# comprna/radian

Measured on AMD Instinct MI355X. Metric: signal samples/s basecalled (chunk=1024, beam=10), higher is better.
Workload: dtype f32

## Files before the change

include/radian_hip.h:

```cpp
#ifndef RADIAN_HIP_H
#define RADIAN_HIP_H

#include <stddef.h>
#include <stdint.h>

#ifdef __cplusplus
extern "C" {
#endif

#define RD_OK 0
#define RD_ERR_ARG (-1)
#define RD_ERR_HIP (-2)
#define RD_ERR_STATE (-3)
#define RD_ERR_NOMEM (-4)
#define RD_ERR_RCCL (-5)
#define RD_ERR_FORMAT (-6)
#define RD_ERR_IO (-7)
#define RD_LEN_MISSING_CONTEXT (-1)

typedef struct rd_ctx rd_ctx;

const char* rd_last_error(void);
int rd_version(void);
int rd_device_count(int* n);
int rd_decode_max_width(void);
int rd_decode_lane_width(void);

int rd_create(int device_id, rd_ctx** out);
int rd_destroy(rd_ctx* ctx);
int rd_sync(rd_ctx* ctx);
int rd_set_precision(rd_ctx* ctx, int mode);

typedef struct rd_weights_header {
    uint32_t magic;
    uint32_t version;
    uint32_t nb_filters;
    uint32_t kernel_size;
    uint32_t relu_units;
    uint32_t n_classes;
    uint32_t n_blocks;
    uint32_t dilations[16];
    uint32_t n_floats;
} rd_weights_header;
int rd_load_weights(rd_ctx* ctx, const void* blob, size_t nbytes);

int rd_load_lm(rd_ctx* ctx, const double* table, int k);
int rd_load_lm_absent(rd_ctx* ctx, int k);
int rd_load_lm_hashed(rd_ctx* ctx, const double* table, int table_order, int context_len);
int rd_set_logits(rd_ctx* ctx, int mode);
int rd_set_decode_partition(rd_ctx* ctx, int cus_per_xcd);
int rd_set_decode_math(rd_ctx* ctx, int mode);

int rd_forward(rd_ctx* ctx, const float* windows, int n_windows, int chunk_len, float* probs);

int rd_assemble(rd_ctx* ctx, const float* probs, int n_windows, int chunk_len, int pad, int step, double* out,
                int64_t out_cap, int64_t* n_rows, int* is_f64);

int rd_decode_batch(rd_ctx* ctx, const void* probs, int prob_is_f64, const int64_t* seq_off, const int32_t* seq_len,
                    int n_seq, int beam_width, int use_lm, double s_thr, double r_thr, uint8_t* labels_out,
                    const int64_t* label_off, int32_t* label_len, double* best_score);

int rd_basecall_chunk(rd_ctx* ctx, const float* windows, int n_windows, int chunk_len, const int32_t* valid_len,
                      int beam_width, uint8_t* labels_out, int32_t* label_len);

int rd_basecall_global(rd_ctx* ctx, const float* windows, int chunk_len, int step, const int32_t* read_win_off,
                       const int32_t* pad, int n_reads, int beam_width, int use_lm, double s_thr, double r_thr,
                       uint8_t* labels_out, const int64_t* label_off, int32_t* label_len);

int rd_count_windows(int64_t n_samples, int chunk_len, int step);
int rd_basecall_reads_chunk(rd_ctx* ctx, const float* signal, const int64_t* read_off, int n_reads, int chunk_len,
                            int step, int beam_width, uint8_t* labels_out, int32_t* label_len);
int rd_basecall_reads_global(rd_ctx* ctx, const float* signal, const int64_t* read_off, int n_reads, int chunk_len,
                             int step, int beam_width, int use_lm, double s_thr, double r_thr, uint8_t* labels_out,
                             const int64_t* label_off, int32_t* label_len);

int rd_normalise_reads(rd_ctx* ctx, const int16_t* raw, const int64_t* read_off, int n_reads, int outlier_clip,
                       float* norm_out , int32_t* status);
int rd_basecall_raw_chunk(rd_ctx* ctx, const int16_t* raw, const int64_t* read_off, int n_reads, int outlier_clip,
                          int chunk_len, int step, int beam_width, uint8_t* labels_out, int32_t* label_len, int32_t* status);
int rd_basecall_raw_global(rd_ctx* ctx, const int16_t* raw, const int64_t* read_off, int n_reads, int outlier_clip,
                           int chunk_len, int step, int beam_width, int use_lm, double s_thr, double r_thr,
                           uint8_t* labels_out, const int64_t* label_off, int32_t* label_len, int32_t* status);

int rd_dev_alloc(rd_ctx* ctx, size_t bytes, void** d_ptr);
int rd_dev_free(rd_ctx* ctx, void* d_ptr);
int rd_mem_info(rd_ctx* ctx, size_t* free_bytes, size_t* total_bytes);
int rd_memcpy_h2d(rd_ctx* ctx, void* d_dst, const void* src, size_t bytes);
int rd_memcpy_d2h(rd_ctx* ctx, void* dst, const void* d_src, size_t bytes);
int rd_forward_resident(rd_ctx* ctx, const float* d_windows, int n_windows, int chunk_len, float* d_probs);
int rd_forward_reads_resident(rd_ctx* ctx, const float* d_signal, const int64_t* read_off, int n_reads, int chunk_len,
                              int step, int decode_type, int lane, int64_t* total_rows);
int rd_forward_reads(rd_ctx* ctx, const float* signal, const int64_t* read_off, int n_reads, int chunk_len, int step,
                     float* probs_out, int64_t windows_cap, int64_t* n_windows);
int rd_basecall_chunk_resident(rd_ctx* ctx, const float* d_windows, int n_windows, int chunk_len,
                               const int32_t* valid_len, int beam_width, uint8_t* labels_out, int32_t* label_len);
int rd_decode_resident(rd_ctx* ctx, const float* d_probs, int n_windows, int chunk_len, const int32_t* valid_len,
                       int beam_width, uint8_t* labels_out, int32_t* label_len);

int rd_basecall_reads_chunk_resident(rd_ctx* ctx, const float* d_signal, const int64_t* read_off, int n_reads,
                                     int chunk_len, int step, int beam_width, uint8_t* labels_out, int32_t* label_len);
int rd_basecall_reads_global_resident(rd_ctx* ctx, const float* d_signal, const int64_t* read_off, int n_reads,
                                      int chunk_len, int step, int beam_width, int use_lm, double s_thr, double r_thr,
                                      uint8_t* labels_out, const int64_t* label_off, int32_t* label_len);

int rd_pipe_config(rd_ctx* ctx, int group_batches);
int rd_pipe_set_lanes(rd_ctx* ctx, int lanes);
int rd_pipe_submit(rd_ctx* ctx, const float* d_windows, int n_windows, int chunk_len, const int32_t* valid_len,
                   int beam_width, uint8_t* labels_out, int32_t* label_len);
int rd_pipe_submit_reads(rd_ctx* ctx, const float* d_signal, const int64_t* read_off, int n_reads, int chunk_len,
                         int step, int beam_width, uint8_t* labels_out, int32_t* label_len);
int rd_pipe_submit_reads_global(rd_ctx* ctx, const float* d_signal, const int64_t* read_off, int n_reads, int chunk_len,
                                int step, int beam_width, int use_lm, double s_thr, double r_thr, uint8_t* labels_out,
                                const int64_t* label_off, int32_t* label_len);
int rd_pipe_submit_raw_global(rd_ctx* ctx, const int16_t* raw, const int64_t* read_off, int n_reads, int outlier_clip,
                              int chunk_len, int step, int beam_width, int use_lm, double s_thr, double r_thr,
                              uint8_t* labels_out, const int64_t* label_off, int32_t* label_len, int32_t* status);
int rd_pipe_submit_raw_chunk(rd_ctx* ctx, const int16_t* raw, const int64_t* read_off, int n_reads, int outlier_clip,
                             int chunk_len, int step, int beam_width, uint8_t* labels_out, int32_t* label_len, int32_t* status);
int rd_pipe_progress(rd_ctx* ctx, int64_t wait_for, int64_t* delivered);
int rd_pipe_flush(rd_ctx* ctx);
int rd_pipe_submitted(rd_ctx* ctx, int64_t* submitted);

int rd_lm_json_probe(const char* buf, size_t n, int* k_out);
int rd_lm_json_fill(const char* buf, size_t n, int k, double* table, int64_t* n_entries, int64_t* n_contexts);
int rd_lm_json_write(const char* path, const double* table, int k, int64_t* n_rows, int64_t* n_bytes);

int rd_fasta_scan(const char* buf, size_t n, int field, const char* value, uint8_t* codes, int64_t* offsets, int64_t* counts);
int rd_lm_build(rd_ctx* ctx, const uint8_t* codes, const int64_t* offsets, int64_t n_records, int k, int as_written, int unseen, double alpha,
                double r_thr, int64_t cut, double* table_out, uint32_t* counts_out, int64_t* stats);
int rd_lm_score(rd_ctx* ctx, const uint8_t* codes, const int64_t* offsets, int64_t n_records, int as_written, double r_thr, int64_t cut,
                int64_t* stats, double* nll_sum);

typedef struct rd_fast5 rd_fast5;
int rd_fast5_open(const char* path, rd_fast5** out);
int rd_fast5_open_mem(const void* buf, size_t n, rd_fast5** out);
void rd_fast5_close(rd_fast5* f);
int rd_fast5_count(const rd_fast5* f, int64_t* n_reads);
int rd_fast5_lengths(rd_fast5* f, int64_t lo, int64_t hi, int64_t* n_samples);
int rd_fast5_read_batch(rd_fast5* f, int64_t lo, int64_t hi, int16_t* samples, int64_t cap, int64_t* offsets, char* ids, int id_stride);

int rd_stitch_chunk(const uint8_t* labels, const int32_t* label_len, int chunk_len, const int32_t* read_win_off, int n_reads,
                    uint8_t* seq_out, const int64_t* seq_off, int32_t* seq_len, int n_threads);

#define RD_ALIGN_OK 0
#define RD_ALIGN_CLIP_INDEX_ERROR 1
#define RD_ALIGN_EMPTY_AFTER_CLIP 2
#define RD_ALIGN_TOO_LARGE 3
int rd_align_batch(rd_ctx* ctx, const uint8_t* refs, const int64_t* ref_off, const uint8_t* reads, const int64_t* read_off, int n_pairs,
                   int match, int mismatch, int gap_open, int gap_extend, int64_t budget_bytes, int32_t* score, int32_t* counts,
                   int32_t* status, uint8_t* ops_out, const int64_t* ops_off, int32_t* ops_len);
int64_t rd_align_workspace_bytes(int64_t n, int64_t m);
int rd_align_clip_count(const uint8_t* ops, int64_t n_ops, const uint8_t* ref, const uint8_t* read, int32_t* counts, int32_t* status);

#define RD_CTCALIGN_OK 0
#define RD_CTCALIGN_NO_PATH 1
#define RD_CTCALIGN_TOO_LARGE 2
int rd_ctc_align_batch(rd_ctx* ctx, const void* probs, int prob_is_f64, const int64_t* seq_off, const int32_t* seq_len, int n_seq,
                       const uint8_t* labels, const int64_t* label_off, const int32_t* label_len, int64_t budget_bytes,
                       int32_t* first_step, int32_t* last_step, uint8_t* qual, double* score, int32_t* status);
int64_t rd_ctc_align_workspace_bytes(int64_t n_rows, int64_t n_labels);
int rd_basecall_raw_global_q(rd_ctx* ctx, const int16_t* raw, const int64_t* read_off, int n_reads, int outlier_clip, int chunk_len,
                             int step, int beam_width, int use_lm, double s_thr, double r_thr, uint8_t* labels_out,
                             const int64_t* label_off, int32_t* label_len, int32_t* status, int64_t budget_bytes, uint8_t* qual_out,
                             int32_t* first_step_out, int32_t* last_step_out, double* score_out, int32_t* align_status);

typedef struct rd_tfrecord rd_tfrecord;
int rd_tfrecord_open(const char* path, rd_tfrecord** out);
int rd_tfrecord_open_mem(const void* buf, size_t n, rd_tfrecord** out);
void rd_tfrecord_close(rd_tfrecord* f);
int rd_tfrecord_count(const rd_tfrecord* f, int64_t* n_records, int64_t* n_labels);
int rd_tfrecord_read(const rd_tfrecord* f, int64_t lo, int64_t hi, float* signals, int32_t* input_len, int64_t* label_off,
                     int32_t* label_len, uint8_t* labels, int64_t labels_cap);
uint32_t rd_crc32c(const void* buf, size_t n);
int rd_tfrecord_write(const char* path, const float* signals, const int32_t* input_len, const uint8_t* labels, const int64_t* label_off,
                      const int32_t* label_len, int64_t n, int append);

#define RD_FIT_OK 0
#define RD_FIT_EMPTY 1
#define RD_FIT_TOO_LARGE 2
int rd_fit_batch(rd_ctx* ctx, const uint8_t* refs, const int64_t* ref_off, int64_t n_refs, const uint8_t* queries, const int64_t* query_off,
                 const int32_t* query_ref, int64_t n_queries, int match, int mismatch, int gap_open, int gap_extend, int64_t budget_bytes,
                 int32_t* score, int32_t* ref_start, int32_t* ref_end, int32_t* counts, int32_t* status);

#define RD_MAP_HASH_C1 0x9E3779B1u
// ... 59 lines not shown
```

radian_amd/_lib.py:

```python
import ctypes
import os

HERE = os.path.dirname(os.path.abspath(__file__))
LIB_PATH = os.environ.get("RADIAN_HIP_LIB") or os.path.join(HERE, "libradian_hip.so")

c_i = ctypes.c_int
c_i32p = ctypes.POINTER(ctypes.c_int32)
c_i64 = ctypes.c_int64
c_i64p = ctypes.POINTER(ctypes.c_int64)
c_d = ctypes.c_double
c_dp = ctypes.POINTER(ctypes.c_double)
c_fp = ctypes.POINTER(ctypes.c_float)
c_u8p = ctypes.POINTER(ctypes.c_uint8)
c_vp = ctypes.c_void_p
c_sz = ctypes.c_size_t

SIGNATURES = {
    "rd_last_error": (ctypes.c_char_p, []),
    "rd_version": (c_i, []),
    "rd_device_count": (c_i, [ctypes.POINTER(c_i)]),
    "rd_decode_max_width": (c_i, []),
    "rd_decode_lane_width": (c_i, []),
    "rd_create": (c_i, [c_i, ctypes.POINTER(c_vp)]),
    "rd_destroy": (c_i, [c_vp]),
    "rd_sync": (c_i, [c_vp]),
    "rd_set_precision": (c_i, [c_vp, c_i]),
    "rd_load_weights": (c_i, [c_vp, c_vp, c_sz]),
    "rd_load_lm": (c_i, [c_vp, c_vp, c_i]),
    "rd_load_lm_absent": (c_i, [c_vp, c_i]),
    "rd_load_lm_hashed": (c_i, [c_vp, c_vp, c_i, c_i]),
    "rd_set_logits": (c_i, [c_vp, c_i]),
    "rd_set_decode_math": (c_i, [c_vp, c_i]),
    "rd_set_decode_partition": (c_i, [c_vp, c_i]),
    "rd_forward": (c_i, [c_vp, c_vp, c_i, c_i, c_vp]),
    "rd_assemble": (c_i, [c_vp, c_vp, c_i, c_i, c_i, c_i, c_vp, c_i64, c_i64p, ctypes.POINTER(c_i)]),
    "rd_decode_batch": (c_i, [c_vp, c_vp, c_i, c_vp, c_vp, c_i, c_i, c_i, c_d, c_d, c_vp, c_vp, c_vp, c_vp]),
    "rd_basecall_chunk": (c_i, [c_vp, c_vp, c_i, c_i, c_vp, c_i, c_vp, c_vp]),
    "rd_basecall_global": (c_i, [c_vp, c_vp, c_i, c_i, c_vp, c_vp, c_i, c_i, c_i, c_d, c_d, c_vp, c_vp, c_vp]),
    "rd_count_windows": (c_i, [c_i64, c_i, c_i]),
    "rd_basecall_reads_chunk": (c_i, [c_vp, c_vp, c_vp, c_i, c_i, c_i, c_i, c_vp, c_vp]),
    "rd_basecall_reads_global": (c_i, [c_vp, c_vp, c_vp, c_i, c_i, c_i, c_i, c_i, c_d, c_d, c_vp, c_vp, c_vp]),
    "rd_basecall_reads_chunk_resident": (c_i, [c_vp, c_vp, c_vp, c_i, c_i, c_i, c_i, c_vp, c_vp]),
    "rd_basecall_reads_global_resident": (c_i, [c_vp, c_vp, c_vp, c_i, c_i, c_i, c_i, c_i, c_d, c_d, c_vp, c_vp, c_vp]),
    "rd_pipe_submit_reads": (c_i, [c_vp, c_vp, c_vp, c_i, c_i, c_i, c_i, c_vp, c_vp]),
    "rd_pipe_submit_reads_global": (c_i, [c_vp, c_vp, c_vp, c_i, c_i, c_i, c_i, c_i, c_d, c_d, c_vp, c_vp, c_vp]),
    "rd_pipe_submit_raw_global": (c_i, [c_vp, c_vp, c_vp, c_i, c_i, c_i, c_i, c_i, c_i, c_d, c_d, c_vp, c_vp, c_vp, c_vp]),
    "rd_pipe_submit_raw_chunk": (c_i, [c_vp, c_vp, c_vp, c_i, c_i, c_i, c_i, c_i, c_vp, c_vp, c_vp]),
    "rd_pipe_progress": (c_i, [c_vp, c_i64, c_i64p]),
    "rd_pipe_submitted": (c_i, [c_vp, c_i64p]),
    "rd_normalise_reads": (c_i, [c_vp, c_vp, c_vp, c_i, c_i, c_vp, c_vp]),
    "rd_basecall_raw_chunk": (c_i, [c_vp, c_vp, c_vp, c_i, c_i, c_i, c_i, c_i, c_vp, c_vp, c_vp]),
    "rd_basecall_raw_global": (c_i, [c_vp, c_vp, c_vp, c_i, c_i, c_i, c_i, c_i, c_i, c_d, c_d, c_vp, c_vp, c_vp, c_vp]),
    "rd_stitch_chunk": (c_i, [c_vp, c_vp, c_i, c_vp, c_i, c_vp, c_vp, c_vp, c_i]),
    "rd_fast5_open": (c_i, [ctypes.c_char_p, ctypes.POINTER(c_vp)]),
    "rd_fast5_open_mem": (c_i, [c_vp, c_sz, ctypes.POINTER(c_vp)]),
    "rd_fast5_close": (None, [c_vp]),
    "rd_fast5_count": (c_i, [c_vp, c_i64p]),
    "rd_fast5_lengths": (c_i, [c_vp, c_i64, c_i64, c_vp]),
    "rd_fast5_read_batch": (c_i, [c_vp, c_i64, c_i64, c_vp, c_i64, c_vp, c_vp, c_i]),
    "rd_lm_json_probe": (c_i, [c_vp, ctypes.c_size_t, ctypes.POINTER(c_i)]),
    "rd_lm_json_fill": (c_i, [c_vp, ctypes.c_size_t, c_i, c_vp, ctypes.POINTER(ctypes.c_int64), ctypes.POINTER(ctypes.c_int64)]),
    "rd_lm_json_write": (c_i, [ctypes.c_char_p, c_vp, c_i, c_i64p, c_i64p]),
    "rd_fasta_scan": (c_i, [c_vp, c_sz, c_i, ctypes.c_char_p, c_vp, c_vp, c_vp]),
    "rd_lm_build": (c_i, [c_vp, c_vp, c_vp, c_i64, c_i, c_i, c_i, c_d, c_d, c_i64, c_vp, c_vp, c_vp]),
    "rd_lm_score": (c_i, [c_vp, c_vp, c_vp, c_i64, c_i, c_d, c_i64, c_vp, c_dp]),
    "rd_dev_alloc": (c_i, [c_vp, c_sz, ctypes.POINTER(c_vp)]),
    "rd_mem_info": (c_i, [c_vp, ctypes.POINTER(c_sz), ctypes.POINTER(c_sz)]),
    "rd_dev_free": (c_i, [c_vp, c_vp]),
    "rd_memcpy_h2d": (c_i, [c_vp, c_vp, c_vp, c_sz]),
    "rd_memcpy_d2h": (c_i, [c_vp, c_vp, c_vp, c_sz]),
    "rd_forward_resident": (c_i, [c_vp, c_vp, c_i, c_i, c_vp]),
    "rd_forward_reads_resident": (c_i, [c_vp, c_vp, c_vp, c_i, c_i, c_i, c_i, c_i, c_vp]),
    "rd_forward_reads": (c_i, [c_vp, c_vp, c_vp, c_i, c_i, c_i, c_vp, c_i64, c_vp]),
    "rd_basecall_chunk_resident": (c_i, [c_vp, c_vp, c_i, c_i, c_vp, c_i, c_vp, c_vp]),
    "rd_decode_resident": (c_i, [c_vp, c_vp, c_i, c_i, c_vp, c_i, c_vp, c_vp]),
    "rd_pipe_config": (c_i, [c_vp, c_i]),
    "rd_pipe_set_lanes": (c_i, [c_vp, c_i]),
    "rd_pipe_submit": (c_i, [c_vp, c_vp, c_i, c_i, c_vp, c_i, c_vp, c_vp]),
    "rd_pipe_flush": (c_i, [c_vp]),
    "rd_align_batch": (c_i, [c_vp, c_vp, c_vp, c_vp, c_vp, c_i, c_i, c_i, c_i, c_i, c_i64, c_vp, c_vp, c_vp, c_vp, c_vp, c_vp]),
    "rd_align_workspace_bytes": (c_i64, [c_i64, c_i64]),
    "rd_align_clip_count": (c_i, [c_vp, c_i64, c_vp, c_vp, c_vp, c_vp]),
    "rd_ctc_align_batch": (c_i, [c_vp, c_vp, c_i, c_vp, c_vp, c_i, c_vp, c_vp, c_vp, c_i64, c_vp, c_vp, c_vp, c_vp, c_vp]),
    "rd_ctc_align_workspace_bytes": (c_i64, [c_i64, c_i64]),
    "rd_basecall_raw_global_q": (c_i, [c_vp, c_vp, c_vp, c_i, c_i, c_i, c_i, c_i, c_i, c_d, c_d, c_vp, c_vp, c_vp, c_vp, c_i64, c_vp, c_vp, c_vp, c_vp, c_vp]),
    "rd_tfrecord_open": (c_i, [ctypes.c_char_p, ctypes.POINTER(c_vp)]),
    "rd_tfrecord_open_mem": (c_i, [c_vp, c_sz, ctypes.POINTER(c_vp)]),
    "rd_tfrecord_close": (None, [c_vp]),
    "rd_tfrecord_count": (c_i, [c_vp, c_i64p, c_i64p]),
    "rd_tfrecord_read": (c_i, [c_vp, c_i64, c_i64, c_vp, c_vp, c_vp, c_vp, c_vp, c_i64]),
    "rd_crc32c": (ctypes.c_uint32, [c_vp, c_sz]),
    "rd_tfrecord_write": (c_i, [ctypes.c_char_p, c_vp, c_vp, c_vp, c_vp, c_vp, c_i64, c_i]),
    "rd_fit_batch": (c_i, [c_vp, c_vp, c_vp, c_i64, c_vp, c_vp, c_vp, c_i64, c_i, c_i, c_i, c_i, c_i64, c_vp, c_vp, c_vp, c_vp, c_vp]),
    "rd_map_minimizers": (c_i, [c_vp, c_i64, c_i, c_i, c_vp, c_vp, c_i64, c_i64p]),
    "rd_map_index": (c_i, [c_vp, c_vp, c_vp, c_i64, c_i, c_i, c_i, c_vp]),
    "rd_map_batch": (c_i, [c_vp, c_vp, c_vp, c_i64, c_i, c_i, c_i, c_i, c_i64, c_vp, c_vp, c_vp]),
    "rd_ctc_eval": (c_i, [c_vp, c_vp, c_i, c_vp, c_vp, c_vp, c_vp, c_vp, c_vp, c_vp, c_vp, c_vp]),
    "rd_ctc_probs": (c_i, [c_vp, c_vp, c_i, c_vp, c_vp, c_vp, c_vp, c_vp, c_vp, c_vp, c_vp, c_vp]),
    "rd_ctc_probs_resident": (c_i, [c_vp, c_vp, c_i, c_vp, c_vp, c_vp, c_vp, c_vp, c_vp, c_vp, c_vp, c_vp]),
    "rd_train_grad": (c_i, [c_vp, c_vp, c_i, c_vp, c_vp, c_vp, c_vp, c_vp, c_vp, c_vp]),
    "rd_train_step": (c_i, [c_vp, c_vp, c_i, c_vp, c_vp, c_vp, c_vp, c_vp, c_vp, c_vp]),
    "rd_train_step_resident": (c_i, [c_vp, c_vp, c_i, c_vp, c_vp, c_vp, c_vp, c_vp, c_vp, c_vp]),
    "rd_train_reset": (c_i, [c_vp]),
    "rd_get_weights": (c_i, [c_vp, c_vp, c_sz]),
    "rd_model_params": (c_i, [c_vp, c_i64p]),
    "rd_train_ctc_grad": (c_i, [c_vp, c_vp, c_i, c_vp, c_vp, c_vp, c_vp, c_vp, c_vp, c_vp]),
    "rd_rccl_probe": (c_i, []),
    "rd_rccl_unique_id": (c_i, [c_vp]),
    "rd_rccl_init": (c_i, [c_vp, c_i, c_i, c_vp]),
    "rd_rccl_bcast_model": (c_i, [c_vp, c_i]),
    "rd_clone_artifacts": (c_i, [c_vp, c_vp]),
    "rd_rccl_allreduce_max": (c_i, [c_vp, c_vp, c_i]),
    "rd_rccl_barrier": (c_i, [c_vp]),
    "rd_rccl_comm_count": (c_i, [c_vp, ctypes.POINTER(c_i)]),
    "rd_rccl_finalize": (c_i, [c_vp]),
}

DIAG_SIGNATURES = {
    "rd_set_conv_fuse": (c_i, [c_vp, c_i]),
    "rd_set_conv_shape": (c_i, [c_vp, c_i]),
    "rd_split3": (c_i, [c_vp, c_vp, c_sz, c_vp]),
    "rd_set_decode_form": (c_i, [c_vp, c_i]),
    "rd_pipe_policy_read": (c_i, [c_vp, c_i, c_i, c_i, c_vp, c_vp, c_vp]),
    "rd_pipe_stats": (c_i, [c_vp, c_i64p, c_i]),
    "rd_set_trie_budget": (c_i, [c_vp, c_i64]),
    "rd_timer_enable": (c_i, [c_vp, c_i, c_i]),
    "rd_timer_read": (c_i, [c_vp, c_i, c_dp, ctypes.POINTER(c_i), c_dp, c_dp]),
    "rd_timer_read_launches": (c_i, [c_vp, c_i, c_i, c_vp, c_vp, c_vp, ctypes.POINTER(c_i)]),
}

_lib = None


def load():
    global _lib
    if _lib is not None:
        return _lib
    if not os.path.exists(LIB_PATH):
        raise RuntimeError(
            f"{LIB_PATH} is missing: build it with `python -m radian_amd.build` (hipcc --offload-arch=gfx950). "
            "radian_amd has no CPU fallback.")
    lib = ctypes.CDLL(LIB_PATH)
    for name, (res, args) in {**SIGNATURES, **DIAG_SIGNATURES}.items():
        fn = getattr(lib, name)
        fn.restype = res
        fn.argtypes = args
    _lib = lib
    return lib
```

radian_amd/backend.py:

```python
import ctypes

import numpy as np

from . import _lib
from .weights import pack_blob, DEFAULT_DILATIONS

RD_TIMER_CONV, RD_TIMER_DECODE, RD_TIMER_HEAD, RD_TIMER_IN = 0, 1, 2, 3


class RadianHipError(RuntimeError):
    pass


def lib_path():
    return _lib.LIB_PATH


def _p(a):
    return None if a is None else a.ctypes.data_as(ctypes.c_void_p)


MISSING_CONTEXT = -1


def _labels_of(labels, off, n):
    if n == MISSING_CONTEXT:
        return None
    return labels[off: off + n].copy()


def device_count():
    n = ctypes.c_int(0)
    L = _lib.load()
    if L.rd_device_count(ctypes.byref(n)) != 0:
        raise RadianHipError(L.rd_last_error().decode())
    return n.value


def device_for_rank(local_rank):
    n = device_count()
    if n < 1:
        raise RadianHipError("no HIP device is visible to this process")
    return local_rank if local_rank < n else local_rank % n


ALIGN_OK, ALIGN_CLIP_INDEX_ERROR, ALIGN_EMPTY_AFTER_CLIP, ALIGN_TOO_LARGE = 0, 1, 2, 3
ALIGN_SCORES = (2, -4, -4, -2)


CTCALIGN_OK, CTCALIGN_NO_PATH, CTCALIGN_TOO_LARGE = 0, 1, 2
CTCALIGN_STATUS_NAMES = ("ok", "no-path", "too-large")


def ctc_align_workspace_bytes(n_rows, n_labels):
    return int(_lib.load().rd_ctc_align_workspace_bytes(int(n_rows), int(n_labels)))


class CtcAlignResult:
    __slots__ = ("first_step", "last_step", "qual", "score", "status")

    def __init__(self, first_step, last_step, qual, score, status):
        self.first_step, self.last_step, self.qual, self.score, self.status = first_step, last_step, qual, score, status


FIT_OK, FIT_EMPTY, FIT_TOO_LARGE = 0, 1, 2


class FitResult:

    def __init__(self, score, ref_start, ref_end, counts, status):
        self.score, self.ref_start, self.ref_end, self.counts, self.status = score, ref_start, ref_end, counts, status


def _concat_codes(seqs):
    arrs = [np.ascontiguousarray(np.frombuffer(s, dtype=np.uint8) if isinstance(s, (bytes, bytearray)) else s, dtype=np.uint8).reshape(-1) for s in seqs]
    off = np.zeros(len(arrs) + 1, dtype=np.int64)
    np.cumsum([a.size for a in arrs], out=off[1:])
    buf = np.concatenate(arrs) if off[-1] else np.zeros(1, dtype=np.uint8)
    return np.ascontiguousarray(buf), off


MAP_OK, MAP_NO_SEED, MAP_NO_CHAIN, MAP_TOO_LARGE, MAP_EMPTY_SPAN = 0, 1, 2, 3, 4


class MapResult:

    FIELDS = ("t", "score", "score2", "n_anchors", "q0", "r0", "q1", "r1")

    def __init__(self, status, hits, stats=None):
        self.status, self.hits, self.stats = status, hits, stats
        for c, name in enumerate(self.FIELDS):
            setattr(self, name, hits[:, c])


def map_minimizers(codes, k, w):
    L = _lib.load()
    c = np.ascontiguousarray(codes, dtype=np.uint8).reshape(-1)
    n = c.size
    buf = c if n else np.zeros(1, dtype=np.uint8)
    pos = np.zeros(max(n, 1), dtype=np.int32)
    hs = np.zeros(max(n, 1), dtype=np.uint32)
    got = ctypes.c_int64(0)
    rc = L.rd_map_minimizers(_p(buf), n, int(k), int(w), _p(pos), _p(hs), pos.size, ctypes.byref(got))
    if rc != 0:
        raise RadianHipError(f"[rd error {rc}] " + L.rd_last_error().decode("utf-8", "replace"))
    return pos[: got.value].copy(), hs[: got.value].copy()


def tfrecord_write(path, signals, input_len, labels, label_len=None, append=False):
    L = _lib.load()
    sig = np.ascontiguousarray(signals, dtype=np.float32)
    n = len(input_len)
    if sig.size != n * CTC_T:
        raise ValueError(f"signals must be [{n}, {CTC_T}] float32")
    il = np.ascontiguousarray(input_len, dtype=np.int32).reshape(-1)
    buf, off, ll = _pack_labels(labels, label_len, n)
    rc = L.rd_tfrecord_write(str(path).encode(), _p(sig), _p(il), _p(buf), _p(off), _p(ll), n, 1 if append else 0)
    if rc == -7:
        raise OSError(L.rd_last_error().decode("utf-8", "replace"))
    if rc != 0:
        raise RadianHipError(f"[rd error {rc}] " + L.rd_last_error().decode("utf-8", "replace"))


def _as_bytes(s):
    return s.encode("latin-1") if isinstance(s, str) else bytes(s)


def _concat(seqs):
    bs = [_as_bytes(s) for s in seqs]
    off = np.zeros(len(bs) + 1, dtype=np.int64)
    np.cumsum([len(b) for b in bs], out=off[1:])
    buf = np.frombuffer(b"".join(bs), dtype=np.uint8) if off[-1] else np.zeros(1, dtype=np.uint8)
    return np.ascontiguousarray(buf), off


def align_workspace_bytes(n, m):
    return int(_lib.load().rd_align_workspace_bytes(int(n), int(m)))


def align_clip_count(ops, ref, read):
    L = _lib.load()
    o, r, q = (np.frombuffer(_as_bytes(x), dtype=np.uint8) if len(x) else np.zeros(1, dtype=np.uint8) for x in (ops, ref, read))
    cnt = np.zeros(4, dtype=np.int32)
    st = np.zeros(1, dtype=np.int32)
    rc = L.rd_align_clip_count(_p(o), len(ops), _p(r), _p(q), _p(cnt), _p(st))
    if rc != 0:
        raise RadianHipError(f"[rd error {rc}] " + L.rd_last_error().decode("utf-8", "replace"))
    return tuple(int(c) for c in cnt), int(st[0])


class AlignResult:

    def __init__(self, score, counts, status, ops):
        self.score, self.counts, self.status, self.ops = score, counts, status, ops


CTC_OK, CTC_INFEASIBLE = 0, 1
CTC_T, CTC_MAX_LABEL = 1024, 255


def _pack_labels(labels, label_len, n):
    if label_len is None:
        label_len = [len(l) for l in labels]
    ll = np.ascontiguousarray(label_len, dtype=np.int32).reshape(-1)
    if len(labels) != n or ll.size != n:
        raise ValueError(f"{len(labels)} label rows and {ll.size} lengths for {n} windows")
    rows = []
    for i in range(n):
        row = np.asarray(labels[i]).reshape(-1)
        if ll[i] < 0 or ll[i] > row.size:
            raise ValueError(f"window {i}: label_length {int(ll[i])} outside 0..{row.size}")
        r = row[: ll[i]]
        if r.size and (np.any(r != np.round(r)) or r.min() < 0 or r.max() > 3):
            raise ValueError(f"window {i}: labels must be 0..3")
        rows.append(r.astype(np.uint8))
    off = np.zeros(n + 1, dtype=np.int64)
    np.cumsum(ll, out=off[1:])
    buf = np.concatenate(rows) if off[-1] else np.zeros(1, dtype=np.uint8)
    return np.ascontiguousarray(buf), np.ascontiguousarray(off[:-1]), ll


class CtcResult:

    def __init__(self, loss, status, greedy_len, edit_distance, greedy):
        self.loss, self.status, self.greedy_len, self.edit_distance, self.greedy = loss, status, greedy_len, edit_distance, greedy


class PipeTicket:

    def __init__(self, be, decode_type, off, n):
        self.be, self.decode_type, self.off, self.n = be, decode_type, off, n
        self.status = np.zeros(n, dtype=np.int32)
        self.labels = self.lens = self.label_off = self.nw = None
        self.seq = 0

    def done(self):
        return self.be.pipe_progress(0) >= self.seq

    def wait(self):
        if self.be.pipe_progress(self.seq) < self.seq:
            raise RadianHipError("pipeline did not deliver the awaited batch")

    def result_raw(self):
        self.wait()
        return self.labels, self.lens, self.nw, self.status

    def result(self):
        self.wait()
        if self.decode_type == "global":
            return [_labels_of(self.labels, self.off[r], self.lens[r]) for r in range(self.n)], self.status
        out, w = [], 0
        for n in self.nw:
            out.append([self.labels[w + i, : self.lens[w + i]].copy() for i in range(n)])
            w += n
        return out, self.status


class Backend:

    def __init__(self, device_id=0):
        self._L = _lib.load()
        h = ctypes.c_void_p()
        self._h = None
        self._check(self._L.rd_create(int(device_id), ctypes.byref(h)))
        self._h = h
        self.device_id = device_id
        self.lm_k = None
        self._tickets = {}

    def _check(self, rc):
        if rc != 0:
            raise RadianHipError(f"[rd error {rc}] " + self._L.rd_last_error().decode("utf-8", "replace"))

    def close(self):
        if self._h is not None:
            self._L.rd_destroy(self._h)
            self._h = None
        self._tickets.clear()

    def __del__(self):
        try:
            self.close()
        except Exception:
            pass

    def __enter__(self):
        return self

    def __exit__(self, *exc):
        self.close()

    def sync(self):
        self._check(self._L.rd_sync(self._h))

    def set_precision(self, mode):
        code = {"fp32": 0, "f16x3": 1, "bf16x3": 2}[mode] if isinstance(mode, str) else int(mode)
        self._check(self._L.rd_set_precision(self._h, code))

    def set_conv_shape(self, shape):
        self._check(self._L.rd_set_conv_shape(self._h, int(shape)))

    def split3(self, values):
        v = np.ascontiguousarray(values, dtype=np.float32).ravel()
        out = np.zeros((3, v.size), dtype=np.uint16)
        self._check(self._L.rd_split3(self._h, _p(v), v.size, _p(out)))
        return out

    @property
    def max_beam_width(self):
        return self._L.rd_decode_max_width()

    def load_weights(self, flat, dilations=DEFAULT_DILATIONS):
        blob = pack_blob(flat, dilations)
        self.load_weights_blob(blob)

    def load_weights_blob(self, blob):
        buf = ctypes.create_string_buffer(blob, len(blob))
        self._check(self._L.rd_load_weights(self._h, ctypes.cast(buf, ctypes.c_void_p), len(blob)))

    def load_lm(self, table, k):
        if table is None:
            self._check(self._L.rd_load_lm(self._h, None, 0))
            self.lm_k = None
            return
        table = np.ascontiguousarray(table, dtype=np.float64)
        if table.shape != (4 ** k, 4):
            raise ValueError(f"LM table must be [4^{k},4], got {table.shape}")
        self._check(self._L.rd_load_lm(self._h, _p(table), int(k)))
        self.lm_k = k

    UNSEEN = {"backoff": 0, "uniform": 1, "absent": 2}

    @staticmethod
    def _records(codes, offsets):
        codes = np.ascontiguousarray(codes, dtype=np.uint8)
        offsets = np.ascontiguousarray(offsets, dtype=np.int64)
        if offsets.ndim != 1 or len(offsets) < 1 or codes.ndim != 1 or int(offsets[-1]) != len(codes):
            raise ValueError("offsets must be [records + 1] and end at len(codes)")
        return (codes if len(codes) else np.zeros(1, dtype=np.uint8)), offsets

    def build_lm(self, codes, offsets, k, as_written=False, unseen="backoff", pseudocount=0.0, r_threshold=0.5, cut=0,
                 want_table=True, want_counts=False):
        codes, offsets = self._records(codes, offsets)
        if unseen not in self.UNSEEN:
            raise ValueError(f"unseen must be one of {sorted(self.UNSEEN)}")
        big = 1 <= k <= 13
        table = np.empty((4 ** k, 4), dtype=np.float64) if want_table and big else None
        counts = np.empty((4 ** k, 4), dtype=np.uint32) if want_counts and big else None
        st = np.zeros(32, dtype=np.int64)
        self._check(self._L.rd_lm_build(self._h, _p(codes), _p(offsets), len(offsets) - 1, int(k), 1 if as_written else 0, self.UNSEEN[unseen],
                                        float(pseudocount), float(r_threshold), int(cut), _p(table), _p(counts), _p(st)))
        self.lm_k = k
        stats = {"windows": int(st[0]), "contexts": 4 ** k, "contexts_seen": int(st[1]), "gate_contexts": int(st[2]), "gate_windows": int(st[3]),
                 "absent_rows": int(st[4]), "uniform_rows": int(st[5]), "launches": int(st[6]),
                 "stage_us": {name: int(st[24 + i]) for i, name in enumerate(("staging", "upload", "count", "table", "download"))},
                 "rows_per_order": {j: int(st[8 + j]) for j in range(k, -1, -1) if st[8 + j]}}
        if counts is not None:
            stats["counts"] = counts
        return table, stats

    def score_lm(self, codes, offsets, as_written=False, r_threshold=0.5, cut=0):
        codes, offsets = self._records(codes, offsets)
        st = np.zeros(8, dtype=np.int64)
        total = ctypes.c_double(0.0)
        self._check(self._L.rd_lm_score(self._h, _p(codes), _p(offsets), len(offsets) - 1, 1 if as_written else 0, float(r_threshold), int(cut),
                                        _p(st), ctypes.byref(total)))
        n = int(st[1])
        return {"windows": int(st[0]), "scored": n, "zero": int(st[2]), "absent": int(st[3]), "gate_windows": int(st[4]),
                "nll_sum": total.value, "mean_nll": total.value / n if n else float("nan")}

    def load_lm_absent(self, k):
        self._check(self._L.rd_load_lm_absent(self._h, int(k)))
        self.lm_k = k

    def load_lm_hashed(self, table, table_order, context_len):
        table = np.ascontiguousarray(table, dtype=np.float64)
        if table.shape != (4 ** table_order, 4):
            raise ValueError(f"LM table must be [4^{table_order},4], got {table.shape}")
        self._check(self._L.rd_load_lm_hashed(self._h, _p(table), int(table_order), int(context_len)))
        self.lm_k = context_len

    def set_logits(self, mode):
        self._check(self._L.rd_set_logits(self._h, {"f32": 0, "f16": 1}[mode] if isinstance(mode, str) else int(mode)))

    def set_trie_budget(self, nbytes):
        self._check(self._L.rd_set_trie_budget(self._h, int(nbytes)))

    def set_conv_fuse(self, on):
        self._check(self._L.rd_set_conv_fuse(self._h, 1 if on else 0))

    def set_decode_form(self, form):
        self._check(self._L.rd_set_decode_form(self._h, {"auto": 0, "waves": 1, "lanes": 2, "two": 3, "one": 4, "queue": 5}[form] if isinstance(form, str) else int(form)))

    def set_decode_partition(self, cus_per_xcd):
        self._check(self._L.rd_set_decode_partition(self._h, int(cus_per_xcd)))

    def set_decode_math(self, mode):
        self._check(self._L.rd_set_decode_math(self._h, {"fast": 0, "glibc": 1}[mode] if isinstance(mode, str) else int(mode)))

    def forward(self, windows):
        windows = np.ascontiguousarray(windows, dtype=np.float32)
        if windows.ndim != 2:
            raise ValueError("windows must be [n_windows, chunk_len]")
        n, T = windows.shape
        probs = np.empty((n, T, 5), dtype=np.float32)
        self._check(self._L.rd_forward(self._h, _p(windows), n, T, _p(probs)))
        return probs

    def assemble(self, probs, pad, step):
        probs = np.ascontiguousarray(probs, dtype=np.float32)
        nW, T, _ = probs.shape
        cap = (nW - 1) * step + T
        out = np.empty((max(cap, 1), 5), dtype=np.float64)
        n_rows = ctypes.c_int64(0)
        is64 = ctypes.c_int(0)
        self._check(self._L.rd_assemble(self._h, _p(probs), nW, T, int(pad), int(step), _p(out), out.shape[0],
                                        ctypes.byref(n_rows), ctypes.byref(is64)))
        out = out[: n_rows.value]
        return out if is64.value else out.astype(np.float32)

    def forward_reads(self, signals, chunk_len, step):
        sigs = [np.ascontiguousarray(s_, dtype=np.float32) for s_ in signals]
        off = np.zeros(len(sigs) + 1, dtype=np.int64)
        off[1:] = np.cumsum([s_.shape[0] for s_ in sigs])
        nws = [self.count_windows(int(s_.shape[0]), chunk_len, step) for s_ in sigs]
        tot = int(sum(nws))
        flat = np.concatenate(sigs) if sigs else np.zeros(0, dtype=np.float32)
        out = np.zeros((tot, chunk_len, 5), dtype=np.float32)
        n = ctypes.c_int64(0)
        self._check(self._L.rd_forward_reads(self._h, _p(flat), _p(off), len(sigs), int(chunk_len), int(step), _p(out), tot, ctypes.byref(n)))
        assert n.value == tot
        res, w = [], 0
        for k in nws:
            res.append(out[w:w + k])
            w += k
        return res

    def decode_batch(self, mats, seq_off, seq_len, beam_width, use_lm=False, s_threshold=0.0, r_threshold=0.0,
                     with_scores=False):
        mats = np.ascontiguousarray(mats)
        if mats.dtype not in (np.float32, np.float64):
            raise TypeError("probabilities must be float32 or float64")
        seq_off = np.ascontiguousarray(seq_off, dtype=np.int64)
        seq_len = np.ascontiguousarray(seq_len, dtype=np.int32)
        n = int(seq_len.shape[0])
        label_off = np.zeros(n, dtype=np.int64)
        if n:
            label_off[1:] = np.cumsum(seq_len[:-1].astype(np.int64))
        labels = np.zeros(int(seq_len.astype(np.int64).sum()) + 1, dtype=np.uint8)
        lens = np.zeros(n, dtype=np.int32)
# ... 528 lines not shown
```

radian_amd/csrc/api.hip:

```cpp
#include "common.h"
#include "plan.h"
#include "../../include/radian_hip.h"

#include <math.h>
#include <string.h>

using namespace rdi;

namespace {

struct SeqMeta {
    int64_t *d_seq_off, *d_seq_off2, *d_node_off, *d_label_off;
    int32_t *d_seq_len, *d_split, *d_label_len;
    double* d_score;
    int64_t total_labels;
    std::vector<TrieRun> runs;
};

int prepare_seq_meta(rd_ctx* ctx, const int64_t* seq_off, const int64_t* seq_off2, const int32_t* split, const int32_t* seq_len,
                     int n_seq, int W, SeqMeta& sm, std::vector<int64_t>& label_off_used)
{
    std::vector<int64_t> node_off(n_seq), lab_off(n_seq);
    int64_t labs = 0;
    for (int i = 0; i < n_seq; i++) {
// ... 194 lines not shown
    }
    return decode_and_fetch(ctx, d_probs, 0, seq_off.data(), valid_len, n_windows, beam_width, 0, 0.0, 0.0, labels_out, lab_off.data(),
                            label_len, nullptr);
}

extern "C" int rd_basecall_chunk_resident(rd_ctx* ctx, const float* d_windows, int n_windows, int chunk_len,
                                          const int32_t* valid_len, int beam_width, uint8_t* labels_out, int32_t* label_len)
{
    RD_REQUIRE(ctx && d_windows && valid_len && labels_out && label_len, "rd_basecall_chunk_resident: null argument");
    RD_REQUIRE(n_windows >= 1 && chunk_len >= 1, "rd_basecall_chunk_resident: bad shape");
    RD_REQUIRE(beam_width >= 1 && beam_width <= rd_decode_max_width(), "beam_width %d out of range", beam_width);
    RD_HIP(hipSetDevice(ctx->device));
    const size_t n = (size_t)n_windows * chunk_len;
    if (ctx->ws_probs.reserve(n * 20)) return RD_ERR_NOMEM;
    int rc = rd_forward_dev(ctx, d_windows, n_windows, chunk_len, ctx->ws_probs.as<float>());
    if (rc) return rc;
    return chunk_decode_from_probs(ctx, ctx->ws_probs.as<float>(), n_windows, chunk_len, valid_len, beam_width, labels_out, label_len);
}

extern "C" int rd_basecall_chunk(rd_ctx* ctx, const float* windows, int n_windows, int chunk_len, const int32_t* valid_len,
                                 int beam_width, uint8_t* labels_out, int32_t* label_len)
{
    RD_REQUIRE(ctx && windows, "rd_basecall_chunk: null argument");
    RD_REQUIRE(n_windows >= 1 && chunk_len >= 1, "rd_basecall_chunk: bad shape");
    RD_HIP(hipSetDevice(ctx->device));
    const size_t n = (size_t)n_windows * chunk_len;
    if (ctx->ws_in.reserve(n * 4)) return RD_ERR_NOMEM;
    RD_HIP(hipMemcpyAsync(ctx->ws_in.p, windows, n * 4, hipMemcpyHostToDevice, ctx->stream));
    return rd_basecall_chunk_resident(ctx, ctx->ws_in.as<float>(), n_windows, chunk_len, valid_len, beam_width, labels_out, label_len);
}

extern "C" int rd_decode_resident(rd_ctx* ctx, const float* d_probs, int n_windows, int chunk_len, const int32_t* valid_len,
                                  int beam_width, uint8_t* labels_out, int32_t* label_len)
{
    RD_REQUIRE(ctx && d_probs && valid_len && labels_out && label_len, "rd_decode_resident: null argument");
    RD_REQUIRE(beam_width >= 1 && beam_width <= rd_decode_max_width(), "beam_width %d out of range", beam_width);
    RD_HIP(hipSetDevice(ctx->device));
    return chunk_decode_from_probs(ctx, d_probs, n_windows, chunk_len, valid_len, beam_width, labels_out, label_len);
}

extern "C" int rd_forward_resident(rd_ctx* ctx, const float* d_windows, int n_windows, int chunk_len, float* d_probs)
{
    RD_REQUIRE(ctx && d_windows, "rd_forward_resident: null argument");
    RD_HIP(hipSetDevice(ctx->device));
    if (!d_probs) {
        if (ctx->ws_probs.reserve((size_t)n_windows * chunk_len * 20)) return RD_ERR_NOMEM;
        d_probs = ctx->ws_probs.as<float>();
    }
    return rd_forward_dev(ctx, d_windows, n_windows, chunk_len, d_probs);
}

static int global_finish(rd_ctx* ctx, const void* d_probs, int f16, bool streamed, const int32_t* win_off, const int32_t* pad, const int64_t* src_row,
                         const int64_t* read_off, int n_reads, int chunk_len, int step, int beam_width, int use_lm, double s_thr, double r_thr,
                         uint8_t* labels_out, const int64_t* label_off, int32_t* label_len, AlignOut* ao = nullptr )
{
    std::vector<ReadRows> rr;
    const int64_t rows64 = classify_reads(win_off, pad, n_reads, chunk_len, step, 0, rr);
    for (int r = 0; read_off && r < n_reads; r++)
        RD_REQUIRE(rr[r].N == read_off[r + 1] - read_off[r], "internal: assembled length mismatch for read %d", r);
    if (ctx->ws_mat.reserve((size_t)(rows64 + 1) * 40)) return RD_ERR_NOMEM;
    int rc;
    for (int r = 0; r < n_reads; r++) {
        if (!rr[r].is64) continue;
        rc = rd_assemble_dev(ctx, (const char*)d_probs + (size_t)src_row[r] * 5 * (f16 ? 2 : 4), win_off[r + 1] - win_off[r], chunk_len, pad[r], step,
                             ctx->ws_mat.as<double>() + rr[r].row64 * 5, rr[r].N, streamed ? 1 : 0, f16);
        if (rc) return rc;
    }
    for (int pass = 0; pass < 2; pass++) {
        std::vector<int64_t> so, lo;
        std::vector<int32_t> sl;
        std::vector<int> idx;
        for (int r = 0; r < n_reads; r++)
            if (rr[r].is64 == (pass == 0)) {
                so.push_back(pass == 0 ? rr[r].row64 : src_row[r]);
                sl.push_back((int32_t)rr[r].N);
                lo.push_back(label_off[r]);
                idx.push_back(r);
            }
        if (idx.empty()) continue;
        std::vector<int32_t> ll(idx.size()), ast(idx.size());
        std::vector<double> asc(idx.size());
        AlignOut pa;
        if (ao) {
            pa = *ao;
            pa.score = asc.data();
            pa.status = ast.data();
        }
        rc = decode_and_fetch(ctx, pass == 0 ? (const void*)ctx->ws_mat.p : d_probs, pass == 0 ? 1 : (f16 ? 2 : 0), so.data(), sl.data(),
                              (int)idx.size(), beam_width, use_lm, s_thr, r_thr, labels_out, lo.data(), ll.data(), nullptr, nullptr, nullptr,
                              ao ? &pa : nullptr);
        if (rc) return rc;
        for (size_t i = 0; i < idx.size(); i++) {
            label_len[idx[i]] = ll[i];
            if (ao) {
                ao->score[idx[i]] = asc[i];
                ao->status[idx[i]] = ast[i];
                ao->too_large |= pa.too_large;
            }
        }
    }
    return RD_OK;
}

extern "C" int rd_basecall_global(rd_ctx* ctx, const float* windows, int chunk_len, int step, const int32_t* read_win_off,
                                  const int32_t* pad, int n_reads, int beam_width, int use_lm, double s_thr, double r_thr,
                                  uint8_t* labels_out, const int64_t* label_off, int32_t* label_len)
{
    RD_REQUIRE(ctx && windows && read_win_off && pad && labels_out && label_off && label_len, "rd_basecall_global: null argument");
    RD_REQUIRE(n_reads >= 1 && chunk_len >= 1, "rd_basecall_global: bad shape");
    RD_REQUIRE(step >= 1 && step <= chunk_len, "rd_basecall_global: step %d must be in [1, chunk_len]", step);
    RD_REQUIRE(beam_width >= 1 && beam_width <= rd_decode_max_width(), "beam_width %d out of range", beam_width);
    RD_REQUIRE_WIDTH_LM(ctx, beam_width, use_lm);
    RD_HIP(hipSetDevice(ctx->device));
    const int nW = read_win_off[n_reads];
    RD_REQUIRE(nW >= n_reads, "rd_basecall_global: every read needs at least one window");
    const size_t n = (size_t)nW * chunk_len;
    if (ctx->ws_in.reserve(n * 4) || ctx->ws_probs.reserve(n * 20)) return RD_ERR_NOMEM;
    RD_HIP(hipMemcpyAsync(ctx->ws_in.p, windows, n * 4, hipMemcpyHostToDevice, ctx->stream));
    int rc = rd_forward_dev(ctx, ctx->ws_in.as<float>(), nW, chunk_len, ctx->ws_probs.as<float>());
    if (rc) return rc;
    std::vector<int64_t> src_row(n_reads);
    for (int r = 0; r < n_reads; r++) {
        RD_REQUIRE(read_win_off[r + 1] > read_win_off[r], "rd_basecall_global: read %d has no windows", r);
        RD_REQUIRE(pad[r] >= 0 && pad[r] <= chunk_len, "rd_basecall_global: pad[%d] out of range", r);
        src_row[r] = (int64_t)read_win_off[r] * chunk_len;
    }
    return global_finish(ctx, ctx->ws_probs.p, 0, false, read_win_off, pad, src_row.data(), nullptr, n_reads, chunk_len, step, beam_width, use_lm,
                         s_thr, r_thr, labels_out, label_off, label_len);
}

extern "C" int rd_count_windows(int64_t n_samples, int chunk_len, int step)
{
    if (n_samples < 0 || chunk_len < 1 || step < 1 || step > chunk_len) return -1;
    return count_windows(n_samples, chunk_len, step);
}

namespace {
struct PlanCache {
    PlanKey key;
    ReadsPlan plan;
    bool streamed = false;
    DevBuf d_tiles;
    TileLists lists;
};

int get_plan(rd_ctx* ctx, const int64_t* read_off, int n_reads, int chunk, int step, int mode, const ReadsPlan** out,
             const TileLists** lists, bool* streamed)
{
    PlanCache* pc = (PlanCache*)ctx->plan_cache[mode];
    if (!pc) {
        pc = new PlanCache();
        ctx->plan_cache[mode] = pc;
    }
    const int halo = rd_model_halo(ctx);
    if (!(pc->d_tiles.p && pc->key.matches(ctx->model, read_off, n_reads, chunk, step, mode, halo))) {
        RD_REQUIRE(read_off[0] == 0, "read_off[0] must be 0");
        size_t total = 0;
        int rc = pc->key.rebuild(ctx->model, read_off, n_reads, chunk, step, mode, halo, pc->plan, &pc->streamed, &total);
        if (rc) return rc;
        if (pc->d_tiles.reserve(total * sizeof(TileDesc) + 16)) return RD_ERR_NOMEM;
        if ((rc = rd_sync_lanes(ctx))) return rc;
        std::vector<TileDesc> host(total);
        plan_fill_lists(pc->plan, pc->d_tiles.as<TileDesc>(), host.data(), pc->lists);
        if (total) RD_HIP(hipMemcpy(pc->d_tiles.p, host.data(), total * sizeof(TileDesc), hipMemcpyHostToDevice));
        pc->key.valid = true;
    }
    *out = &pc->plan;
    *lists = &pc->lists;
    if (streamed) *streamed = pc->streamed;
    return RD_OK;
}

}

int rdi::rd_check_reads_args(rd_ctx* ctx, const void* signal, const int64_t* read_off, int n_reads, int chunk_len, int step, int W)
{
    RD_REQUIRE(ctx && signal && read_off, "null argument");
    RD_REQUIRE(n_reads >= 1 && chunk_len >= 1, "bad shape");
    RD_REQUIRE(step >= 1 && step <= chunk_len, "step %d must be in [1, chunk_len]", step);
    RD_REQUIRE(W >= 1 && W <= rd_decode_max_width(), "beam_width %d out of range", W);
    if (!ctx->model.loaded) {
        rd_set_error("no weights loaded (rd_load_weights)");
        return RD_ERR_STATE;
    }
    return RD_OK;
}

void rd_plan_cache_destroy_internal(rd_ctx* ctx)
{
    for (int m = 0; m < 2; m++) {
        PlanCache* pc = (PlanCache*)ctx->plan_cache[m];
        if (pc) {
            pc->d_tiles.release();
            delete pc;
        }
        ctx->plan_cache[m] = nullptr;
    }
}

extern "C" int rd_basecall_reads_chunk_resident(rd_ctx* ctx, const float* d_signal, const int64_t* read_off, int n_reads,
                                                int chunk_len, int step, int beam_width, uint8_t* labels_out,
                                                int32_t* label_len)
{
    int rc = rd_check_reads_args(ctx, d_signal, read_off, n_reads, chunk_len, step, beam_width);
    if (rc) return rc;
    RD_REQUIRE(labels_out && label_len, "rd_basecall_reads_chunk: null output");
    RD_HIP(hipSetDevice(ctx->device));
    const ReadsPlan* P = nullptr;
    const TileLists* tl = nullptr;
    if ((rc = get_plan(ctx, read_off, n_reads, chunk_len, step, 0, &P, &tl, nullptr))) return rc;
    if (ctx->ws_probs.reserve((size_t)P->total_rows * 20)) return RD_ERR_NOMEM;
    const int f16 = ctx->logits_f16;
    rc = rd_forward_tiles_dev(ctx, d_signal, *tl, P->total_rows, ctx->ws_probs.p, 0, f16);
    if (rc) return rc;
    std::vector<int64_t> lab_off(P->n_windows);
    for (int w = 0; w < P->n_windows; w++) lab_off[w] = (int64_t)w * chunk_len;
    return decode_and_fetch(ctx, ctx->ws_probs.p, f16 ? 2 : 0, P->off1.data(), P->valid.data(), P->n_windows, beam_width, 0, 0.0, 0.0,
                            labels_out, lab_off.data(), label_len, nullptr, P->off2.data(), P->split.data());
}

extern "C" int rd_forward_reads_resident(rd_ctx* ctx, const float* d_signal, const int64_t* read_off, int n_reads, int chunk_len,
                                         int step, int decode_type, int lane, int64_t* total_rows)
{
    int rc = rd_check_reads_args(ctx, d_signal, read_off, n_reads, chunk_len, step, 1);
    if (rc) return rc;
    RD_REQUIRE(decode_type == 0 || decode_type == 1, "rd_forward_reads_resident: decode_type %d (0 = chunk plan, 1 = global plan)", decode_type);
    RD_REQUIRE(lane >= 0 && lane < RD_MAX_LANES, "rd_forward_reads_resident: lane %d out of range [0,%d)", lane, RD_MAX_LANES);
    RD_HIP(hipSetDevice(ctx->device));
    const ReadsPlan* P = nullptr;
    const TileLists* tl = nullptr;
    if ((rc = get_plan(ctx, read_off, n_reads, chunk_len, step, decode_type, &P, &tl, nullptr))) return rc;
    if (ctx->ws_probs.reserve((size_t)P->total_rows * 20)) return RD_ERR_NOMEM;
    if (total_rows) *total_rows = P->total_rows;
    return rd_forward_tiles_dev(ctx, d_signal, *tl, P->total_rows, ctx->ws_probs.p, lane, ctx->logits_f16);
}

extern "C" int rd_forward_reads(rd_ctx* ctx, const float* signal, const int64_t* read_off, int n_reads, int chunk_len, int step,
                                float* probs_out, int64_t windows_cap, int64_t* n_windows)
{
    int rc = rd_check_reads_args(ctx, signal, read_off, n_reads, chunk_len, step, 1);
    if (rc) return rc;
    RD_REQUIRE(probs_out && n_windows, "rd_forward_reads: null output");
    RD_REQUIRE(!ctx->logits_f16, "rd_forward_reads: float32 rows only (rd_set_logits 0)");
    RD_HIP(hipSetDevice(ctx->device));
    const size_t n = (size_t)read_off[n_reads];
    if (ctx->ws_in.reserve(n * 4 + 16)) return RD_ERR_NOMEM;
    RD_HIP(hipMemcpyAsync(ctx->ws_in.p, signal, n * 4, hipMemcpyHostToDevice, ctx->stream));
    const ReadsPlan* P = nullptr;
    const TileLists* tl = nullptr;
    if ((rc = get_plan(ctx, read_off, n_reads, chunk_len, step, 0, &P, &tl, nullptr))) return rc;
    *n_windows = P->n_windows;
    RD_REQUIRE(P->n_windows <= windows_cap, "rd_forward_reads: %d windows, room for %lld", P->n_windows, (long long)windows_cap);
    if (ctx->ws_probs.reserve((size_t)P->total_rows * 20)) return RD_ERR_NOMEM;
    if ((rc = rd_forward_tiles_dev(ctx, ctx->ws_in.as<float>(), *tl, P->total_rows, ctx->ws_probs.p, 0, 0))) return rc;
    const size_t nw = (size_t)P->n_windows, a8 = align_up(nw * 8, 256), a4 = align_up(nw * 4, 256);
    const size_t out_bytes = nw * chunk_len * 20;
    if (ctx->ws_misc.reserve(2 * a8 + 2 * a4) || ctx->ws_mat.reserve(out_bytes + 16)) return RD_ERR_NOMEM;
    char* dm = (char*)ctx->ws_misc.p;
    RD_HIP(hipMemcpyAsync(dm, P->off1.data(), nw * 8, hipMemcpyHostToDevice, ctx->stream));
    RD_HIP(hipMemcpyAsync(dm + a8, P->off2.data(), nw * 8, hipMemcpyHostToDevice, ctx->stream));
    RD_HIP(hipMemcpyAsync(dm + 2 * a8, P->split.data(), nw * 4, hipMemcpyHostToDevice, ctx->stream));
    RD_HIP(hipMemcpyAsync(dm + 2 * a8 + a4, P->valid.data(), nw * 4, hipMemcpyHostToDevice, ctx->stream));
    if ((rc = rd_gather_windows_dev(ctx->stream, ctx->ws_probs.as<float>(), (const int64_t*)dm, (const int64_t*)(dm + a8), (const int32_t*)(dm + 2 * a8),
                                    (const int32_t*)(dm + 2 * a8 + a4), P->n_windows, chunk_len, (float*)ctx->ws_mat.p)))
        return rc;
    RD_HIP(hipMemcpyAsync(probs_out, ctx->ws_mat.p, out_bytes, hipMemcpyDeviceToHost, ctx->stream));
    RD_HIP(hipStreamSynchronize(ctx->stream));
    return RD_OK;
}

extern "C" int rd_basecall_reads_chunk(rd_ctx* ctx, const float* signal, const int64_t* read_off, int n_reads, int chunk_len,
                                       int step, int beam_width, uint8_t* labels_out, int32_t* label_len)
{
    int rc = rd_check_reads_args(ctx, signal, read_off, n_reads, chunk_len, step, beam_width);
    if (rc) return rc;
    RD_HIP(hipSetDevice(ctx->device));
    const size_t n = (size_t)read_off[n_reads];
    if (ctx->ws_in.reserve(n * 4 + 16)) return RD_ERR_NOMEM;
    RD_HIP(hipMemcpyAsync(ctx->ws_in.p, signal, n * 4, hipMemcpyHostToDevice, ctx->stream));
    return rd_basecall_reads_chunk_resident(ctx, ctx->ws_in.as<float>(), read_off, n_reads, chunk_len, step, beam_width, labels_out,
                                            label_len);
}

static int reads_global_resident(rd_ctx* ctx, const float* d_signal, const int64_t* read_off, int n_reads, int chunk_len, int step, int beam_width,
                                 int use_lm, double s_thr, double r_thr, uint8_t* labels_out, const int64_t* label_off, int32_t* label_len,
                                 AlignOut* ao)
{
    int rc = rd_check_reads_args(ctx, d_signal, read_off, n_reads, chunk_len, step, beam_width);
    if (rc) return rc;
    RD_REQUIRE(labels_out && label_off && label_len, "rd_basecall_reads_global: null output");
    RD_REQUIRE_WIDTH_LM(ctx, beam_width, use_lm);
    RD_HIP(hipSetDevice(ctx->device));
    const ReadsPlan* P = nullptr;
    const TileLists* tl = nullptr;
    bool streamed = false;
    if ((rc = get_plan(ctx, read_off, n_reads, chunk_len, step, 1, &P, &tl, &streamed))) return rc;
    if (ctx->ws_probs.reserve((size_t)P->total_rows * 20)) return RD_ERR_NOMEM;
    const int f16 = ctx->logits_f16;
    rc = rd_forward_tiles_dev(ctx, d_signal, *tl, P->total_rows, ctx->ws_probs.p, 0, f16);
    if (rc) return rc;
    return global_finish(ctx, ctx->ws_probs.p, f16, streamed, P->read_win_off.data(), P->valid.data(), P->read_row.data(), read_off, n_reads, chunk_len,
                         step, beam_width, use_lm, s_thr, r_thr, labels_out, label_off, label_len, ao);
}

extern "C" int rd_basecall_reads_global_resident(rd_ctx* ctx, const float* d_signal, const int64_t* read_off, int n_reads,
                                                 int chunk_len, int step, int beam_width, int use_lm, double s_thr, double r_thr,
                                                 uint8_t* labels_out, const int64_t* label_off, int32_t* label_len)
{
    return reads_global_resident(ctx, d_signal, read_off, n_reads, chunk_len, step, beam_width, use_lm, s_thr, r_thr, labels_out, label_off, label_len,
                                 nullptr);
}
// ... 94 lines not shown
```

radian_amd/csrc/common.h:

```cpp
#pragma once
#include <hip/hip_runtime.h>
#include <stdint.h>
#include <stddef.h>
#include <string>
#include <vector>

#define RD_OK 0
#define RD_ERR_ARG (-1)
#define RD_ERR_HIP (-2)
#define RD_ERR_STATE (-3)
#define RD_ERR_NOMEM (-4)
#define RD_ERR_RCCL (-5)

void rd_set_error(const char* fmt, ...);

#define RD_HIP(expr)                                                                                   \
    do {                                                                                               \
        hipError_t _e = (expr);                                                                        \
        if (_e != hipSuccess) {                                                                        \
            rd_set_error("%s:%d: %s failed: %s", __FILE__, __LINE__, #expr, hipGetErrorString(_e));   \
            return RD_ERR_HIP;                                                                         \
        }                                                                                              \
    } while (0)

#define RD_REQUIRE(cond, ...)                                                                          \
    do {                                                                                               \
        if (!(cond)) {                                                                                 \
            rd_set_error(__VA_ARGS__);                                                                 \
            return RD_ERR_ARG;                                                                         \
        }                                                                                              \
    } while (0)

struct DevBuf {
    void* p = nullptr;
    size_t cap = 0;
    int reserve(size_t bytes);
    void release();
    template <typename T> T* as() const { return (T*)p; }
};

constexpr int RD_C = 256;
constexpr int RD_K = 3;
constexpr int RD_H = 128;
constexpr int RD_NCLS = 5;
constexpr int RD_MAX_BLOCKS = 16;

struct Model {
    bool loaded = false;
    int nblocks = 0;
    int dil[RD_MAX_BLOCKS] = {0};
    float* sink = nullptr;
    float* w_in = nullptr;
    float* b_in = nullptr;
    float* w_match = nullptr;
    float* b_match = nullptr;
    float* w_conv[2 * RD_MAX_BLOCKS] = {nullptr};
    float* b_conv[2 * RD_MAX_BLOCKS] = {nullptr};
    float* w_d1 = nullptr;
    float* b_d1 = nullptr;
    void* ws_conv[2 * RD_MAX_BLOCKS] = {nullptr};
    float inv_scale[2 * RD_MAX_BLOCKS] = {0};
    void* ws_d1 = nullptr;
    float inv_scale_d1 = 0.f;
    void* w3_conv[2 * RD_MAX_BLOCKS] = {nullptr};
    void* w3_d1 = nullptr;
    float* w_d2 = nullptr;
    float* b_d2 = nullptr;
    DevBuf storage;
    bool split_stale = false;
};

struct LM {
    bool loaded = false;
    int k = 0;
    int table_order = 0;
    int hashed = 0;
    double* table = nullptr;
    double* d_entropy = nullptr;
    int sparse = 0;
    uint32_t* d_missing = nullptr;
    uint32_t* gate_bits = nullptr;
    double gate_r_thr = 0.0;
    bool gate_valid = false;
    DevBuf storage, gate_storage;
};

struct TileDesc {
    int64_t seg_row;
    int64_t src_row;
    int64_t alt_row;
    int32_t t0;
    int32_t seg_len;
    int32_t in_len;
    int32_t alt_in;
    int32_t alt_res;
    int32_t pad_;
};

constexpr int RD_MAX_LAYERS = 2 * 16 + 1;
struct TileLists {
    const TileDesc* d[RD_MAX_LAYERS];
    int n[RD_MAX_LAYERS];
    int64_t rows[RD_MAX_LAYERS];
};

struct KernelTimer {
    bool enabled = false;
    std::vector<hipEvent_t> starts, stops;
    size_t used = 0;
    double flops = 0.0;
    double bytes = 0.0;
    std::vector<double> each_flops;
    std::vector<int> each_tag;
};

constexpr int RD_MAX_LANES = 4;
struct FwdLane {
    hipStream_t st = nullptr;
    DevBuf act[3];
    hipEvent_t done = nullptr;
};

struct rd_ctx {
    int device = 0;
    int n_cu = 256;
    int precision = 0;
    int decode_form = 0;
    int decode_math = 1;
    int conv_fuse = 1;
    int conv_shape = 0;
    int logits_f16 = 0;
    hipStream_t stream = nullptr;
    hipStream_t stream_hi = nullptr;
    hipEvent_t ev_chain = nullptr;
    Model model;
    LM lm;
    DevBuf ws_tiles, ws_raw;
    int tiles_nW = -1, tiles_T = -1;
    FwdLane lanes[2 * RD_MAX_LANES];
    int part_mode = -1;
    int part_cus = 0;
    DevBuf ws_in, ws_probs, ws_mat, ws_seq, ws_nodes_child, ws_nodes_back, ws_labels, ws_misc;
    DevBuf ws_queue;
    DevBuf ws_wide, ws_wide_slot;
    DevBuf ws_align;
    DevBuf ws_ctc;
    DevBuf ws_calign;
    int64_t trie_budget = (int64_t)24 << 30;
    void* h_stage = nullptr;
    size_t h_stage_cap = 0;
    bool h_stage_busy = false;
    KernelTimer timer_conv, timer_decode, timer_head, timer_in;
    void* rccl = nullptr;
    void* rpipe = nullptr;
    int pipe_group = 4;
    int pipe_lanes = 2;
    void* plan_cache[2] = {nullptr, nullptr};
    void* train = nullptr;
    void* map = nullptr;
};

size_t rd_model_image_floats(int nblocks);
void rd_model_bind(Model& m);
int rd_model_refresh_split(rd_ctx* ctx);
int rd_model_halo(const rd_ctx* ctx);
size_t rd_lm_image_doubles(int table_order);
void rd_lm_bind(LM& lm);
int rd_lm_finish_device(rd_ctx* ctx, int table_order, int context_len, int hashed);
int rd_forward_dev(rd_ctx* ctx, const float* d_windows, int nW, int T, float* d_probs, int lane = 0);
int rd_forward_tiles_dev(rd_ctx* ctx, const float* d_signal, const TileLists& tiles, int64_t total_rows, void* d_probs, int lane = 0,
                         int probs_f16 = 0 );
int rd_lane_get(rd_ctx* ctx, int lane, FwdLane** out);
constexpr int RD_XCDS = 8;
int rd_part_set(rd_ctx* ctx, int cus_per_xcd);
int rd_masked_stream_acquire(int device, int cus_per_xcd, bool complement, hipStream_t* out);
void rd_masked_stream_release(hipStream_t st);
int rd_sync_lanes(rd_ctx* ctx);
int rd_split3_dev(rd_ctx* ctx, const float* d_in, size_t n, uint16_t* d_out);
int rd_decode_dev(rd_ctx* ctx, const void* d_probs, int ptype , const int64_t* d_seq_off, const int32_t* d_seq_len,
                  const int64_t* d_node_off, const int64_t* d_label_off, int n_seq, int64_t total_nodes, int W, int use_lm,
                  double s_thr, double r_thr, uint8_t* d_labels, int32_t* d_label_len, double* d_best_score,
                  hipStream_t stream = nullptr , const int64_t* d_seq_off2 = nullptr,
                  const int32_t* d_seq_split = nullptr, int n_cu_avail = 0 ,
                  int queue_wave_slots = 0 );
int rd_normalise_dev(rd_ctx* ctx, const int16_t* d_raw, const int64_t* d_read_off, int n_reads, int clip, float* d_out,
                     int32_t* d_status, hipStream_t stream = nullptr );
struct AsmRead {
    int64_t src_row, out_row;
    int32_t N, nW, pad, pad_;
};
int rd_assemble_batch_dev(hipStream_t st, const void* d_probs, const AsmRead* d_reads, int n_reads, int64_t max_n, int T, int step,
                          double* d_out, int streamed, int in_f16);
int rd_gather_windows_dev(hipStream_t st, const float* d_rows, const int64_t* d_off1, const int64_t* d_off2, const int32_t* d_split,
                          const int32_t* d_valid, int n_windows, int T, float* d_out);
int rd_assemble_dev(rd_ctx* ctx, const void* d_probs, int nW, int T, int pad, int step, double* d_out, int64_t N,
                    int streamed = 0 ,
                    int in_f16 = 0 );

int rd_ctc_align_dev(rd_ctx* ctx, hipStream_t st, const void* d_probs, int ptype, const int64_t* seq_off, const int32_t* seq_len, int n_seq,
                     const uint8_t* d_labels, const int64_t* dlab_off, const int32_t* label_len, int64_t budget_bytes, int32_t* first_step,
                     int32_t* last_step, uint8_t* qual, const int64_t* out_off, double* score, int32_t* status);
void rd_train_invalidate(rd_ctx* ctx);
void rd_train_destroy(rd_ctx* ctx);
int rd_train_weights_host(rd_ctx* ctx, std::vector<float>& flat);
void rd_map_destroy(rd_ctx* ctx);
void rd_plan_cache_destroy_internal(rd_ctx* ctx);

bool rd_rpipe_idle(const rd_ctx* ctx);
int rd_rpipe_drain_decode(rd_ctx* ctx);
void rd_rpipe_destroy(rd_ctx* ctx);

inline bool rd_decode_len_ok(int W, int64_t rows) { return 1 + (int64_t)W * rows < ((int64_t)1 << 29); }

extern "C" int rd_decode_max_width(void);
constexpr int RD_LANE_MAX_W = 256;
constexpr int RD_HASHED_MAX_W = 64;
constexpr int RD_WIDE_MAX_W = 1024;
int rd_decode_wide_launch(rd_ctx* ctx, hipStream_t st, const void* decode_args, int ptype, int n_seq, int64_t total_nodes, bool lm);

static inline size_t align_up(size_t x, size_t a) { return (x + a - 1) / a * a; }

inline size_t rd_wide_scratch_bytes(int W)
{
    const size_t b = (size_t)2 * W * 48 + (size_t)3 * 5 * W * 8 + (size_t)2 * 5 * W * 4 + (size_t)W * 4;
    return (b + 255) & ~(size_t)255;
}

struct TrieRun {
    int k0, k1;
    int64_t nodes;
};
template <typename LenOf>
inline void rd_plan_trie_runs(const rd_ctx* ctx, int W, int k_begin, int k_end, LenOf len_of, int64_t* node_off, std::vector<TrieRun>& runs)
{
    const int64_t per_node = W > RD_LANE_MAX_W ? 24 : 20;
    const int64_t per_seq = W > RD_LANE_MAX_W ? (int64_t)rd_wide_scratch_bytes(W) : 0;
    int64_t nodes = 0, bytes = 0;
    int k0 = k_begin;
    for (int k = k_begin; k < k_end; k++) {
        const int64_t nk = 1 + (int64_t)W * len_of(k), bk = nk * per_node + per_seq;
        if (k > k0 && bytes + bk > ctx->trie_budget) {
            runs.push_back({k0, k, nodes});
            k0 = k;
            nodes = bytes = 0;
        }
        node_off[k] = nodes;
        nodes += nk;
        bytes += bk;
    }
    if (k_end > k0) runs.push_back({k0, k_end, nodes});
}

#define RD_REQUIRE_WIDTH_LM(ctx, W, use_lm)                                                                                     \
    RD_REQUIRE(!((use_lm) && (ctx)->lm.loaded && (ctx)->lm.hashed && (W) > RD_HASHED_MAX_W),                                     \
               "beam width %d with a hashed long-context RNA model (rd_load_lm_hashed): hashed contexts exist for widths up to 64", (W))
```

radian_amd/csrc/context.hip:

```cpp
#include "common.h"
#include "../../include/radian_hip.h"
#include "../../include/radian_hip_diag.h"

#include <algorithm>
#include <stdarg.h>
#include <stdio.h>
#include <string.h>

static thread_local char g_err[1024] = "";

void rd_set_error(const char* fmt, ...)
{
    va_list ap;
    va_start(ap, fmt);
    vsnprintf(g_err, sizeof(g_err), fmt, ap);
    va_end(ap);
}

extern "C" const char* rd_last_error(void) { return g_err; }
extern "C" int rd_version(void) { return 1; }

int DevBuf::reserve(size_t bytes)
{
    if (bytes <= cap) return 0;
// ... 41 lines not shown
        return RD_ERR_HIP;
    }
    *n = c;
    return RD_OK;
}


extern "C" int rd_create(int device_id, rd_ctx** out)
{
    RD_REQUIRE(out != nullptr, "rd_create: null out pointer");
    *out = nullptr;
    int n = 0;
    hipError_t e = hipGetDeviceCount(&n);
    if (e != hipSuccess || n <= 0) {
        rd_set_error("rd_create: no HIP device available (%s); this backend has no CPU fallback",
                     e != hipSuccess ? hipGetErrorString(e) : "device count is 0");
        return RD_ERR_HIP;
    }
    RD_REQUIRE(device_id >= 0 && device_id < n, "rd_create: device_id %d out of range [0,%d)", device_id, n);
    RD_HIP(hipSetDevice(device_id));
    hipDeviceProp_t prop;
    RD_HIP(hipGetDeviceProperties(&prop, device_id));
    if (strncmp(prop.gcnArchName, "gfx950", 6) != 0) {
        rd_set_error("rd_create: device %d is %s; libradian_hip is built for gfx950 (MI355X) only", device_id, prop.gcnArchName);
        return RD_ERR_HIP;
    }
    rd_ctx* ctx = new rd_ctx();
    ctx->device = device_id;
    ctx->n_cu = prop.multiProcessorCount > 0 ? prop.multiProcessorCount : 256;
    e = hipStreamCreateWithFlags(&ctx->stream, hipStreamNonBlocking);
    if (e == hipSuccess) {
        int lo = 0, hi = 0;
        e = hipDeviceGetStreamPriorityRange(&lo, &hi);
        if (e == hipSuccess) e = hipStreamCreateWithPriority(&ctx->stream_hi, hipStreamNonBlocking, hi);
        if (e == hipSuccess) e = hipEventCreateWithFlags(&ctx->ev_chain, hipEventDisableTiming);
    }
    if (e != hipSuccess) {
        rd_set_error("hipStreamCreate failed: %s", hipGetErrorString(e));
        if (ctx->stream) (void)hipStreamDestroy(ctx->stream);
        if (ctx->stream_hi) (void)hipStreamDestroy(ctx->stream_hi);
        delete ctx;
        return RD_ERR_HIP;
    }
    *out = ctx;
    return RD_OK;
}

static void timer_free(KernelTimer& t)
{
    for (auto ev : t.starts) (void)hipEventDestroy(ev);
    for (auto ev : t.stops) (void)hipEventDestroy(ev);
    t.starts.clear();
    t.stops.clear();
    t.each_flops.clear();
    t.each_tag.clear();
    t.used = 0;
    t.enabled = false;
}

extern "C" int rd_destroy(rd_ctx* ctx)
{
    if (!ctx) return RD_OK;
    (void)hipSetDevice(ctx->device);
    if (ctx->stream) (void)hipStreamSynchronize(ctx->stream);
    rd_rccl_finalize(ctx);
    rd_rpipe_destroy(ctx);
    rd_plan_cache_destroy_internal(ctx);
    rd_train_destroy(ctx);
    rd_map_destroy(ctx);
    timer_free(ctx->timer_conv);
    timer_free(ctx->timer_decode);
    timer_free(ctx->timer_head);
    timer_free(ctx->timer_in);
    for (int i = 0; i < 2 * RD_MAX_LANES; i++) {
        FwdLane& L = ctx->lanes[i];
        if (i > 0 && L.st) {
            (void)hipStreamSynchronize(L.st);
            if (i >= RD_MAX_LANES) rd_masked_stream_release(L.st);
            else (void)hipStreamDestroy(L.st);
        }
        if (L.done) (void)hipEventDestroy(L.done);
        for (DevBuf& b : L.act) b.release();
    }
    DevBuf* bufs[] = {&ctx->ws_tiles, &ctx->ws_raw, &ctx->ws_in, &ctx->ws_probs, &ctx->ws_mat, &ctx->ws_seq,
                      &ctx->ws_nodes_child, &ctx->ws_nodes_back, &ctx->ws_wide, &ctx->ws_wide_slot, &ctx->ws_align, &ctx->ws_ctc, &ctx->ws_calign, &ctx->ws_queue, &ctx->ws_labels, &ctx->ws_misc, &ctx->model.storage,
                      &ctx->lm.storage, &ctx->lm.gate_storage};
    for (DevBuf* b : bufs) b->release();
    if (ctx->h_stage) (void)hipHostFree(ctx->h_stage);
    if (ctx->stream_hi) {
        (void)hipStreamSynchronize(ctx->stream_hi);
        (void)hipStreamDestroy(ctx->stream_hi);
    }
    if (ctx->ev_chain) (void)hipEventDestroy(ctx->ev_chain);
    if (ctx->stream) (void)hipStreamDestroy(ctx->stream);
    delete ctx;
    return RD_OK;
}

extern "C" int rd_set_precision(rd_ctx* ctx, int mode)
{
    RD_REQUIRE(ctx, "rd_set_precision: null context");
    RD_REQUIRE(mode >= 0 && mode <= 2, "rd_set_precision: mode %d (0 = fp32 MFMA, 1 = split-f16 f16x3, 2 = three-term bf16x3)", mode);
    ctx->precision = mode;
    return RD_OK;
}

extern "C" int rd_sync(rd_ctx* ctx)
{
    RD_REQUIRE(ctx, "rd_sync: null context");
    return rd_sync_lanes(ctx);
}

extern "C" int rd_set_logits(rd_ctx* ctx, int mode)
{
    RD_REQUIRE(ctx, "rd_set_logits: null context");
    RD_REQUIRE(mode == 0 || mode == 1, "rd_set_logits: mode %d (0 = float32 rows, 1 = float16 rows)", mode);
    ctx->logits_f16 = mode;
    return RD_OK;
}

extern "C" int rd_set_decode_form(rd_ctx* ctx, int form)
{
    RD_REQUIRE(ctx, "rd_set_decode_form: null context");
    RD_REQUIRE(form >= 0 && form <= 5, "rd_set_decode_form: form %d (0 = per launch, 1 = waves per sequence, 2 = candidates per lane, 3 = W <= 12: two sequences per "
               "wave, 4 = one, 5 = work queue)", form);
    ctx->decode_form = form;
    return RD_OK;
}

extern "C" int rd_set_trie_budget(rd_ctx* ctx, int64_t bytes)
{
    RD_REQUIRE(ctx, "rd_set_trie_budget: null context");
    RD_REQUIRE(bytes >= 0, "rd_set_trie_budget: negative budget");
    ctx->trie_budget = bytes ? bytes : (int64_t)24 << 30;
    return RD_OK;
}

extern "C" int rd_set_conv_shape(rd_ctx* ctx, int shape)
{
    RD_REQUIRE(ctx, "rd_set_conv_shape: null context");
    RD_REQUIRE(shape == 0 || shape == 1, "rd_set_conv_shape: shape %d (0 = 128-row tiles, two workgroups per CU; 1 = 256-row tiles, one workgroup per CU)", shape);
    ctx->conv_shape = shape;
    return RD_OK;
}

extern "C" int rd_set_conv_fuse(rd_ctx* ctx, int on)
{
    RD_REQUIRE(ctx, "rd_set_conv_fuse: null context");
    RD_REQUIRE(on == 0 || on == 1, "rd_set_conv_fuse: %d (1 = block 0's first conv inside its second, 0 = its own kernel)", on);
    ctx->conv_fuse = on;
    return RD_OK;
}

extern "C" int rd_set_decode_partition(rd_ctx* ctx, int cus_per_xcd)
{
    RD_REQUIRE(ctx, "rd_set_decode_partition: null context");
    RD_REQUIRE(cus_per_xcd >= -1 && cus_per_xcd <= 16, "rd_set_decode_partition: %d CUs per XCD (-1 = by beam width, 0 = off, 1..16)", cus_per_xcd);
    RD_REQUIRE(rd_rpipe_idle(ctx), "rd_set_decode_partition: pipeline not empty (call rd_pipe_flush first)");
    ctx->part_mode = cus_per_xcd;
    return RD_OK;
}

extern "C" int rd_set_decode_math(rd_ctx* ctx, int mode)
{
    RD_REQUIRE(ctx, "rd_set_decode_math: null context");
    RD_REQUIRE(mode == 0 || mode == 1, "rd_set_decode_math: mode %d (0 = library routines, 1 = glibc's operation sequence)", mode);
    ctx->decode_math = mode;
    return RD_OK;
}

extern "C" int rd_dev_alloc(rd_ctx* ctx, size_t bytes, void** d_ptr)
{
    RD_REQUIRE(ctx && d_ptr, "rd_dev_alloc: null argument");
    RD_HIP(hipSetDevice(ctx->device));
    RD_HIP(hipMalloc(d_ptr, bytes ? bytes : 1));
    return RD_OK;
}
extern "C" int rd_mem_info(rd_ctx* ctx, size_t* free_bytes, size_t* total_bytes)
{
    RD_REQUIRE(ctx && free_bytes && total_bytes, "rd_mem_info: null argument");
    RD_HIP(hipSetDevice(ctx->device));
    RD_HIP(hipMemGetInfo(free_bytes, total_bytes));
    return RD_OK;
}
extern "C" int rd_dev_free(rd_ctx* ctx, void* d_ptr)
{
    RD_REQUIRE(ctx, "rd_dev_free: null context");
    if (d_ptr) RD_HIP(hipFree(d_ptr));
    return RD_OK;
}
extern "C" int rd_memcpy_h2d(rd_ctx* ctx, void* d_dst, const void* src, size_t bytes)
{
    RD_REQUIRE(ctx && d_dst && src, "rd_memcpy_h2d: null argument");
    RD_HIP(hipMemcpyAsync(d_dst, src, bytes, hipMemcpyHostToDevice, ctx->stream));
    RD_HIP(hipStreamSynchronize(ctx->stream));
    return RD_OK;
}
extern "C" int rd_memcpy_d2h(rd_ctx* ctx, void* dst, const void* d_src, size_t bytes)
{
    RD_REQUIRE(ctx && dst && d_src, "rd_memcpy_d2h: null argument");
    RD_HIP(hipMemcpyAsync(dst, d_src, bytes, hipMemcpyDeviceToHost, ctx->stream));
    RD_HIP(hipStreamSynchronize(ctx->stream));
    return RD_OK;
}

extern "C" int rd_split3(rd_ctx* ctx, const float* values, size_t n, uint16_t* terms_out)
{
    RD_REQUIRE(ctx && values && terms_out, "rd_split3: null argument");
    RD_HIP(hipSetDevice(ctx->device));
    if (n == 0) return RD_OK;
    if (ctx->ws_in.reserve(n * 4) || ctx->ws_misc.reserve(n * 6)) return RD_ERR_NOMEM;
    RD_HIP(hipMemcpyAsync(ctx->ws_in.p, values, n * 4, hipMemcpyHostToDevice, ctx->stream));
    int rc = rd_split3_dev(ctx, ctx->ws_in.as<float>(), n, ctx->ws_misc.as<uint16_t>());
    if (rc) return rc;
    RD_HIP(hipMemcpyAsync(terms_out, ctx->ws_misc.p, n * 6, hipMemcpyDeviceToHost, ctx->stream));
    RD_HIP(hipStreamSynchronize(ctx->stream));
    return RD_OK;
}

static KernelTimer* timer_of(rd_ctx* ctx, int which)
{
    switch (which) {
        case RD_TIMER_CONV: return &ctx->timer_conv;
        case RD_TIMER_DECODE: return &ctx->timer_decode;
        case RD_TIMER_HEAD: return &ctx->timer_head;
        case RD_TIMER_IN: return &ctx->timer_in;
    }
    return nullptr;
}

extern "C" int rd_timer_enable(rd_ctx* ctx, int which, int max_launches)
{
    RD_REQUIRE(ctx, "rd_timer_enable: null context");
    KernelTimer* t = timer_of(ctx, which);
    RD_REQUIRE(t, "rd_timer_enable: unknown timer %d", which);
    RD_HIP(hipSetDevice(ctx->device));
    RD_HIP(hipStreamSynchronize(ctx->stream));
    timer_free(*t);
    t->flops = t->bytes = 0.0;
    if (max_launches <= 0) return RD_OK;
    t->starts.resize(max_launches);
    t->stops.resize(max_launches);
    for (int i = 0; i < max_launches; i++) {
        RD_HIP(hipEventCreate(&t->starts[i]));
        RD_HIP(hipEventCreate(&t->stops[i]));
    }
    t->enabled = true;
    return RD_OK;
}

extern "C" int rd_timer_read(rd_ctx* ctx, int which, double* total_ms, int* launches, double* flops, double* bytes)
{
    RD_REQUIRE(ctx, "rd_timer_read: null context");
    KernelTimer* t = timer_of(ctx, which);
    RD_REQUIRE(t, "rd_timer_read: unknown timer %d", which);
    RD_HIP(hipStreamSynchronize(ctx->stream));
    double ms = 0.0;
    for (size_t i = 0; i < t->used; i++) {
        float f = 0.f;
        RD_HIP(hipEventElapsedTime(&f, t->starts[i], t->stops[i]));
        ms += f;
    }
    if (total_ms) *total_ms = ms;
    if (launches) *launches = (int)t->used;
    if (flops) *flops = t->flops;
    if (bytes) *bytes = t->bytes;
    return RD_OK;
}

extern "C" int rd_timer_read_launches(rd_ctx* ctx, int which, int cap, float* ms_out, double* flops_out, int32_t* tag_out, int* n_out)
{
    RD_REQUIRE(ctx && n_out, "rd_timer_read_launches: null argument");
    KernelTimer* t = timer_of(ctx, which);
    RD_REQUIRE(t, "rd_timer_read_launches: unknown timer %d", which);
    RD_HIP(hipStreamSynchronize(ctx->stream));
    const size_t n = std::min(t->used, (size_t)std::max(0, cap));
    for (size_t i = 0; i < n; i++) {
        float f = 0.f;
        RD_HIP(hipEventElapsedTime(&f, t->starts[i], t->stops[i]));
        if (ms_out) ms_out[i] = f;
        if (flops_out) flops_out[i] = i < t->each_flops.size() ? t->each_flops[i] : 0.0;
        if (tag_out) tag_out[i] = i < t->each_tag.size() ? t->each_tag[i] : 0;
    }
    *n_out = (int)n;
    return RD_OK;
}
```

radian_amd/csrc/forward.hip:

```cpp
#include "common.h"

#include <algorithm>
#include <vector>
#include <mutex>

#include <stdint.h>
#include <stdlib.h>
#include <type_traits>

namespace {

typedef float f32x16 __attribute__((ext_vector_type(16)));

constexpr int BM = 128;
constexpr int BK = 16;

enum { EPI_RELU = 0, EPI_RES_IDENT = 1, EPI_RES_MATCH = 2, EPI_HEAD = 3 };

struct ZeroRows {
    uint4* row[3];
    int n16;
};
__device__ __forceinline__ void clear_zero_rows(const ZeroRows& z)
{
    if (blockIdx.x != 0) return;
    for (int r = 0; r < 3; r++)
        for (int i = threadIdx.x; i < z.n16; i += blockDim.x) z.row[r][i] = make_uint4(0u, 0u, 0u, 0u);
}

struct ConvArgs {
    const float* in;
    float* out;
    const float* wpk;
    const float* bias;
    const float* resid;
    const float* x;
    const float* wmatch;
    const float* bmatch;
    const float* w2;
    const float* b2;
    float* probs;
    int probs_f16;
    int zero_row;
    float* sink;
    const TileDesc* tiles;
    int dil;
    const float* w_in;
    const float* b_in;
    ZeroRows zr;
};

__device__ __forceinline__ float conv_in_value(float b, float w0, float w1, float w2, float x0, float x1, float x2)
{
    const float v = __builtin_fmaf(x2, w2, __builtin_fmaf(x1, w1, __builtin_fmaf(x0, w0, b)));
    return v > 0.f ? v : 0.f;
}

__device__ __forceinline__ void glds16_uncounted(const float* src, float* lds_dst)
{
    unsigned keep;
    const unsigned dst = (unsigned)(uintptr_t)(__attribute__((address_space(3))) void*)lds_dst;
    asm volatile("s_mov_b32 %0, m0\n\ts_mov_b32 m0, %2\n\ts_nop 0\n\tglobal_load_lds_dwordx4 %1, off\n\ts_mov_b32 m0, %0"
                 : "=&s"(keep)
                 : "v"(src), "s"(dst)
                 : "memory");
}
template <int OFFSET>
__device__ __forceinline__ void glds16_uncounted_saddr(unsigned lane_off, const void* sbase, float* lds_dst)
{
    unsigned keep;
    const unsigned dst = (unsigned)(uintptr_t)(__attribute__((address_space(3))) void*)lds_dst;
    asm volatile("s_mov_b32 %0, m0\n\ts_mov_b32 m0, %3\n\ts_nop 0\n\tglobal_load_lds_dwordx4 %1, %2 offset:%4\n\ts_mov_b32 m0, %0"
                 : "=&s"(keep)
                 : "v"(lane_off), "s"(sbase), "s"(dst), "n"(OFFSET)
                 : "memory");
}
template <int LEAVE, bool LGKM = false>
__device__ __forceinline__ void wait_dma_and_barrier()
{
    if constexpr (LGKM) asm volatile("s_waitcnt vmcnt(%0) lgkmcnt(0)\n\ts_barrier" ::"n"(LEAVE) : "memory");
    else asm volatile("s_waitcnt vmcnt(%0)\n\ts_barrier" ::"n"(LEAVE) : "memory");
}

__device__ __forceinline__ float relu_raw(float v)
{
    float r;
    asm("v_max_f32 %0, 0, %1" : "=v"(r) : "v"(v));
    return r;
}

typedef float f32x4 __attribute__((ext_vector_type(4)));
__device__ __forceinline__ __attribute__((address_space(1))) char* sgpr_base(const void* p)
{
    const uint32_t lo = __builtin_amdgcn_readfirstlane((uint32_t)(uint64_t)p), hi = __builtin_amdgcn_readfirstlane((uint32_t)((uint64_t)p >> 32));
    uint64_t u = (uint64_t)hi << 32 | lo;
    asm("" : "+s"(u));
    return (__attribute__((address_space(1))) char*)u;
}
__device__ __forceinline__ float4 gload16(const void* sbase, unsigned byte_off)
{
    asm("" : "+v"(byte_off));
    const f32x4 v = *(const __attribute__((address_space(1))) f32x4*)(sgpr_base(sbase) + byte_off);
    return make_float4(v.x, v.y, v.z, v.w);
}
__device__ __forceinline__ void gstore16(void* sbase, unsigned byte_off, float4 v)
{
    asm("" : "+v"(byte_off));
    *(__attribute__((address_space(1))) f32x4*)(sgpr_base(sbase) + byte_off) = f32x4{v.x, v.y, v.z, v.w};
}

template <int ROWS, typename Args>
__device__ __forceinline__ void head_dense5_softmax(const float* hs, const float* w2s, float* part, const TileDesc* __restrict__ tds,
                                                    const Args& a, int tid)
{
    constexpr int LDH = RD_H + 1;
    const int hrow = tid < ROWS ? tid : tid - ROWS;
    const int j0 = tid < ROWS ? 0 : RD_H / 2;
    float lg[5];
#pragma unroll
    for (int o = 0; o < 5; o++) lg[o] = tid < ROWS ? w2s[RD_H * 5 + o] : 0.f;
    for (int j = j0; j < j0 + RD_H / 2; j++) {
        const float h = hs[hrow * LDH + j];
#pragma unroll
        for (int o = 0; o < 5; o++) lg[o] += h * w2s[j * 5 + o];
    }
    if (tid >= ROWS) {
#pragma unroll
        for (int o = 0; o < 5; o++) part[hrow * 5 + o] = lg[o];
    }
    __syncthreads();
    if (tid < ROWS) {
        const TileDesc sd = tds[tid >> 5];
        const int t = sd.t0 + (tid & 31);
        const int64_t seg_row = sd.seg_row;
        if (t < sd.seg_len) {
#pragma unroll
            for (int o = 0; o < 5; o++) lg[o] += part[tid * 5 + o];
            float mx = lg[0];
#pragma unroll
            for (int o = 1; o < 5; o++) mx = lg[o] > mx ? lg[o] : mx;
            float e[5], sum = 0.f;
#pragma unroll
            for (int o = 0; o < 5; o++) {
                e[o] = expf(lg[o] - mx);
                sum += e[o];
            }
            if (a.probs_f16) {
                _Float16* pr = (_Float16*)a.probs + ((size_t)seg_row + t) * 5;
#pragma unroll
                for (int o = 0; o < 5; o++) pr[o] = (_Float16)(e[o] / sum);
            } else {
                float* pr = a.probs + ((size_t)seg_row + t) * 5;
#pragma unroll
                for (int o = 0; o < 5; o++) pr[o] = e[o] / sum;
            }
        }
    }
}

constexpr int FIN_DMAX = 2;
template <int NT, int TAPS, int EPI, int WM = 2, bool FIN = false>
__global__ __launch_bounds__(128 * WM, WM == 2 ? 2 : 1) void tcn_gemm_kernel(ConvArgs a)
{
    static_assert(!FIN || (EPI == EPI_RES_MATCH && WM == 2 && TAPS == 3 && NT == 4), "FIN: block 0's second conv, product shape");
    constexpr int BM = 64 * WM;
    constexpr int NWAVE = 2 * WM;
    constexpr int BN = 2 * NT * 32;
    constexpr int NCHUNK = TAPS * (RD_C / BK);
    constexpr int A_FLOATS = FIN ? 0 : BM * BK;
    constexpr int STAGE_FLOATS = A_FLOATS + BN * BK;
    constexpr int HEAD_FLOATS = BM * (RD_H + 1) + RD_H * 5 + 8 + BM * 5;
    constexpr int NSTAGE = 3;
    constexpr int MIDROWS = 4 * (32 + 2 * FIN_DMAX);
    constexpr int FIN_FLOATS = FIN ? 2 * MIDROWS * BK + 4 * RD_C : 0;
    constexpr int SMEM_FLOATS = (EPI == EPI_HEAD && HEAD_FLOATS > NSTAGE * STAGE_FLOATS) ? HEAD_FLOATS : NSTAGE * STAGE_FLOATS + FIN_FLOATS;

    __shared__ __attribute__((aligned(1024))) float smem[SMEM_FLOATS];

    if constexpr (FIN) clear_zero_rows(a.zr);
    const int tid = threadIdx.x;
    const int lane = tid & 63;
    const int wave = __builtin_amdgcn_readfirstlane(tid >> 6);
    const int wm = wave >> 1;
    const int wn = wave & 1;
    const TileDesc* __restrict__ tds = a.tiles + (size_t)blockIdx.x * NWAVE;
    const TileDesc sdm[2] = {tds[wm * 2], tds[wm * 2 + 1]};
    const bool mval[2] = {sdm[0].seg_len > sdm[0].t0, sdm[1].seg_len > sdm[1].t0};

    const int dma_r = lane >> 2;
    const int dma_ps = lane & 3;
    const TileDesc sst = tds[wave];
    const int64_t d_seg = sst.seg_row, d_alt = sst.alt_row;
    const int d_t0 = sst.t0, d_ain = sst.alt_in;
    const int d_len = sst.seg_len > sst.t0 ? sst.in_len : 0;
    const int lane_slot = (dma_ps ^ ((dma_r >> 2) & 3)) * 4;
    int arow[TAPS][2];
#pragma unroll
    for (int tap = 0; tap < TAPS; tap++)
#pragma unroll
        for (int pc = 0; pc < 2; pc++) {
            const int t = d_t0 + pc * 16 + dma_r - (TAPS - 1 - tap) * a.dil;
            arow[tap][pc] = (t >= 0 && t < d_len) ? (int)((t < d_ain ? d_seg : d_alt) + t) : a.zero_row;
        }
    const char* lanebase = (const char*)(a.in + lane_slot);
    const unsigned lane_off = lane * 16;

    constexpr int PB = BN / (16 * NWAVE);
    constexpr int NA = FIN ? 0 : 2;
    constexpr int NPIECE = NA + PB;
    auto stage_piece = [&](int chunk, int tap, float* st, int pc) {
        if (pc < NA) {
            const int cc = chunk / TAPS;
            const char* src = lanebase + (size_t)cc * (BK * 4) + (uint64_t)(unsigned)arow[tap][pc] * (RD_C * 4);
            glds16_uncounted((const float*)src, st + (wave * 2 + pc) * 256);
        } else {
            const float* wb = a.wpk + (size_t)chunk * BN * BK + wave * PB * 256;
            float* dst = st + A_FLOATS + wave * PB * 256;
            const int pb = pc - NA;
            if (pb == 0) glds16_uncounted_saddr<0>(lane_off, wb, dst);
            else if (pb == 1) glds16_uncounted_saddr<1024>(lane_off, wb, dst);
            else if (pb == 2) glds16_uncounted_saddr<2048>(lane_off, wb, dst);
            else glds16_uncounted_saddr<3072>(lane_off, wb, dst);
        }
    };
    auto stage = [&](int chunk, int tap, float* st) {
#pragma unroll
        for (int pc = 0; pc < NPIECE; pc++) stage_piece(chunk, tap, st, pc);
    };

    float* const midb = smem + NSTAGE * STAGE_FLOATS;
    float* const wins = midb + 2 * MIDROWS * BK;
    const int RS = 32 + 2 * a.dil;
    float xs[3][3] = {{0.f, 0.f, 0.f}, {0.f, 0.f, 0.f}, {0.f, 0.f, 0.f}};
    bool rowv[3] = {false, false, false};
    if constexpr (FIN) {
        *(float4*)(wins + tid * 4) = tid < 192 ? *(const float4*)(a.w_in + tid * 4) : *(const float4*)(a.b_in + (tid - 192) * 4);
        const float* __restrict__ xw = a.x + sst.src_row;
#pragma unroll
        for (int p = 0; p < 3; p++) {
            const int i = dma_r + 16 * p;
            const int t = d_t0 - 2 * a.dil + i;
            rowv[p] = i < RS && t >= 0 && t < d_len;
#pragma unroll
            for (int j = 0; j < 3; j++) {
                const int u = t - (2 - j) * a.dil;
                xs[p][j] = (rowv[p] && u >= 0) ? xw[u] : 0.f;
            }
        }
        __syncthreads();
    }
    auto fin_pass = [&](int cc, int p) {
        const int i = dma_r + 16 * p;
        if (i < RS) {
            const int c0 = cc * BK + dma_ps * 4;
            const float4 w0 = *(const float4*)(wins + c0), w1 = *(const float4*)(wins + RD_C + c0), w2 = *(const float4*)(wins + 2 * RD_C + c0),
                         bb = *(const float4*)(wins + 3 * RD_C + c0);
            float4 v = make_float4(0.f, 0.f, 0.f, 0.f);
            if (rowv[p]) {
                v.x = conv_in_value(bb.x, w0.x, w1.x, w2.x, xs[p][0], xs[p][1], xs[p][2]);
                v.y = conv_in_value(bb.y, w0.y, w1.y, w2.y, xs[p][0], xs[p][1], xs[p][2]);
                v.z = conv_in_value(bb.z, w0.z, w1.z, w2.z, xs[p][0], xs[p][1], xs[p][2]);
                v.w = conv_in_value(bb.w, w0.w, w1.w, w2.w, xs[p][0], xs[p][1], xs[p][2]);
            }
            const int rho = wave * RS + i;
            *(float4*)(midb + (cc & 1) * (MIDROWS * BK) + rho * BK + ((dma_ps ^ ((rho >> 2) & 3)) * 4)) = v;
        }
    };
    if constexpr (FIN) {
#pragma unroll
        for (int p = 0; p < 3; p++) fin_pass(0, p);
    }

    const int fr = lane & 31;
    const int fh = lane >> 5;
    f32x16 acc[2][NT];
#pragma unroll
    for (int n = 0; n < NT; n++) {
        const float bias = a.bias[wn * NT * 32 + n * 32 + fr];
#pragma unroll
        for (int m = 0; m < 2; m++)
#pragma unroll
            for (int e = 0; e < 16; e++) acc[m][n][e] = bias;
    }

    const int swz = (fr >> 2) & 3;
    int koff[BK / 8];
#pragma unroll
    for (int g = 0; g < BK / 8; g++) koff[g] = ((2 * g + fh) ^ swz) * 4;
    const int a_off = (wm * 64 + fr) * BK;
    const int b_off = A_FLOATS + (wn * NT * 32 + fr) * BK;

    const bool work = mval[0] || mval[1];
    int frow[3][2] = {{0, 0}, {0, 0}, {0, 0}}, fswz[3][2] = {{0, 0}, {0, 0}, {0, 0}};
    if constexpr (FIN) {
#pragma unroll
        for (int tap = 0; tap < 3; tap++)
#pragma unroll
            for (int m = 0; m < 2; m++) {
                const int rho = (wm * 2 + m) * RS + fr + tap * a.dil;
                frow[tap][m] = rho * BK;
                fswz[tap][m] = (rho >> 2) & 3;
            }
    }
    auto chunk_step = [&](const float* st, int cur, int cur_tap, int next, int next_tap, float* nst) {
        const float* Ab = st + a_off;
        const float* Bb = st + b_off;
        const float* Mb = midb + ((cur / TAPS) & 1) * (MIDROWS * BK);
        constexpr int NSTEP = (BK / 8) * NT;
        float4 af[2][2], bq[2];
        auto rdA = [&](int g) {
#pragma unroll
            for (int m = 0; m < 2; m++) {
                if constexpr (FIN) af[g & 1][m] = *(const float4*)(Mb + frow[cur_tap][m] + (((2 * g + fh) ^ fswz[cur_tap][m]) * 4));
                else af[g & 1][m] = *(const float4*)(Ab + m * 32 * BK + koff[g]);
            }
        };
        auto rdB = [&](int sidx) { bq[sidx & 1] = *(const float4*)(Bb + (sidx % NT) * 32 * BK + koff[sidx / NT]); };
        const bool st_ok = next < NCHUNK;
        if (work) {
            rdA(0);
            rdB(0);
        }
#pragma unroll
        for (int sidx = 0; sidx < NSTEP; sidx++) {
            const int g = sidx / NT, n = sidx % NT;
            if (work) {
                if (sidx + 1 < NSTEP) rdB(sidx + 1);
                if (n == NT - 1 && g + 1 < BK / 8) rdA(g + 1);
#pragma unroll
                for (int kr = 0; kr < 4; kr++) {
                    const float bv = kr == 0 ? bq[sidx & 1].x : kr == 1 ? bq[sidx & 1].y : kr == 2 ? bq[sidx & 1].z : bq[sidx & 1].w;
#pragma unroll
                    for (int m = 0; m < 2; m++) {
                        const float4 aq = af[g & 1][m];
                        const float av = kr == 0 ? aq.x : kr == 1 ? aq.y : kr == 2 ? aq.z : aq.w;
                        acc[m][n] = __builtin_amdgcn_mfma_f32_32x32x2f32(av, bv, acc[m][n], 0, 0, 0);
                    }
                }
                __builtin_amdgcn_sched_group_barrier(0x100, 3, 0);
                __builtin_amdgcn_sched_group_barrier(0x008, 8, 0);
            }
            __builtin_amdgcn_sched_barrier(0);
            if (st_ok && sidx < NPIECE) stage_piece(next, next_tap, nst, sidx);
            if constexpr (FIN) {
                if (sidx == NPIECE && cur / TAPS + 1 < RD_C / BK) fin_pass(cur / TAPS + 1, cur_tap);
            }
            __builtin_amdgcn_sched_barrier(0);
        }
    };

    static_assert(NPIECE <= (BK / 8) * NT, "one DMA piece per MFMA step");
    float* st0 = smem;
    float* st1 = smem + STAGE_FLOATS;
    float* st2 = smem + 2 * STAGE_FLOATS;
    constexpr bool T3 = TAPS == 3;
    static_assert(TAPS == 3 || TAPS == 1, "tap of a chunk is a literal in the unrolled loop");
    stage(0, 0, st0);
    stage(1, T3 ? 1 : 0, st1);
    auto step = [&](int c, int tap, const float* st, int tap2, float* nst) {
        if (c + 1 < NCHUNK) wait_dma_and_barrier<NPIECE, FIN>(); else wait_dma_and_barrier<0, FIN>();
        chunk_step(st, c, tap, c + 2, tap2, nst);
    };
    for (int chunk = 0; chunk < NCHUNK; chunk += 3) {
        step(chunk, 0, st0, T3 ? 2 : 0, st2);
        if (chunk + 1 < NCHUNK) step(chunk + 1, T3 ? 1 : 0, st1, 0, st0);
        if (chunk + 2 < NCHUNK) step(chunk + 2, T3 ? 2 : 0, st2, T3 ? 1 : 0, st1);
    }
    __syncthreads();

    if constexpr (EPI != EPI_HEAD) {
        constexpr int TSTR = 64;
        float* ts = smem + wave * (32 * TSTR);
        float4* sink4 = (float4*)a.sink + (threadIdx.x & 255);
        const int rrow = lane >> 4;
        const int c4 = (lane & 15) * 4;
#pragma unroll
        for (int m = 0; m < 2; m++) {
            if (!mval[m]) continue;
            const TileDesc sd = sdm[m];
            const int T = sd.seg_len;
            float* __restrict__ outw = a.out + (size_t)sd.seg_row * RD_C;
            const float* __restrict__ resw = a.resid + (size_t)sd.seg_row * RD_C;
            const float* __restrict__ resalt = a.resid + (size_t)sd.alt_row * RD_C;
            const bool interior = sd.t0 + 32 <= T;
            auto to_patch = [&](int np) {
#pragma unroll
                for (int j = 0; j < 2; j++) {
                    const int n = 2 * np + j;
#pragma unroll
                    for (int e = 0; e < 16; e++) {
                        const int rl = (e & 3) + 8 * (e >> 2) + 4 * fh;
                        ts[rl * TSTR + j * 32 + fr] = relu_raw(acc[m][n][e]);
                    }
                }
                __builtin_amdgcn_fence(__ATOMIC_RELEASE, "wavefront");
                __builtin_amdgcn_wave_barrier();
            };
            const bool res_one = EPI != EPI_RES_IDENT || sd.t0 + 32 <= sd.alt_res || sd.t0 >= sd.alt_res;
            if (EPI != EPI_RES_MATCH && interior && res_one) {
                const unsigned lbyte = (rrow * RD_C + c4) * 4;
                float* __restrict__ ob = outw + (size_t)sd.t0 * RD_C + wn * (NT * 32);
                const float* __restrict__ rb = (sd.t0 < sd.alt_res ? resw : resalt) + (size_t)sd.t0 * RD_C + wn * (NT * 32);
#pragma unroll
                for (int np = 0; np < NT / 2; np++) {
                    to_patch(np);
#pragma unroll
                    for (int ih = 0; ih < 8; ih += 4) {
                        float4 rv[4];
                        if constexpr (EPI == EPI_RES_IDENT) {
#pragma unroll
                            for (int i = 0; i < 4; i++) rv[i] = gload16(rb + np * 64 + (ih + i) * 4 * RD_C, lbyte);
                        }
#pragma unroll
                        for (int i = 0; i < 4; i++) {
                            float4 v = *(const float4*)(ts + ((ih + i) * 4 + rrow) * TSTR + c4);
                            if constexpr (EPI == EPI_RES_IDENT) {
                                v.x += rv[i].x; v.y += rv[i].y; v.z += rv[i].z; v.w += rv[i].w;
                            }
                            gstore16(ob + np * 64 + (ih + i) * 4 * RD_C, lbyte, v);
                        }
                    }
                    __builtin_amdgcn_fence(__ATOMIC_RELEASE, "wavefront");
                    __builtin_amdgcn_wave_barrier();
                }
                continue;
            }
#pragma unroll
            for (int np = 0; np < NT / 2; np++) {
                to_patch(np);
                const int ch = wn * NT * 32 + np * 64 + c4;
                float4 wm4 = make_float4(0.f, 0.f, 0.f, 0.f), bm4 = wm4;
                if constexpr (EPI == EPI_RES_MATCH) {
                    wm4 = *(const float4*)(a.wmatch + ch);
                    bm4 = *(const float4*)(a.bmatch + ch);
                }
#pragma unroll
                for (int ih = 0; ih < 8; ih += 4) {
                    float4 rv[4];
                    int tt[4];
#pragma unroll
                    for (int i = 0; i < 4; i++) {
                        const int t = sd.t0 + (ih + i) * 4 + rrow;
                        tt[i] = t;
                        if constexpr (EPI == EPI_RES_IDENT) {
                            const int tc = (interior || t < T) ? t : T - 1;
                            rv[i] = *(const float4*)((tc < sd.alt_res ? resw : resalt) + (size_t)tc * RD_C + ch);
                        }
                    }
#pragma unroll
                    for (int i = 0; i < 4; i++) {
                        float4 v = *(const float4*)(ts + ((ih + i) * 4 + rrow) * TSTR + c4);
                        const int t = tt[i];
                        const bool inb = interior || t < T;
                        if constexpr (EPI == EPI_RES_IDENT) {
                            v.x += rv[i].x; v.y += rv[i].y; v.z += rv[i].z; v.w += rv[i].w;
                        } else if constexpr (EPI == EPI_RES_MATCH) {
                            const float xv = a.x[(size_t)sd.src_row + (inb ? t : T - 1)];
                            v.x = (bm4.x + xv * wm4.x) + v.x; v.y = (bm4.y + xv * wm4.y) + v.y;
                            v.z = (bm4.z + xv * wm4.z) + v.z; v.w = (bm4.w + xv * wm4.w) + v.w;
                            v.x = v.x > 0.f ? v.x : 0.f; v.y = v.y > 0.f ? v.y : 0.f;
                            v.z = v.z > 0.f ? v.z : 0.f; v.w = v.w > 0.f ? v.w : 0.f;
                        }
                        float4* dst = inb ? (float4*)(outw + (size_t)t * RD_C + ch) : sink4;
                        *dst = v;
                    }
                }
                __builtin_amdgcn_fence(__ATOMIC_RELEASE, "wavefront");
                __builtin_amdgcn_wave_barrier();
            }
        }
    } else {
        constexpr int LDH = RD_H + 1;
        float* hs = smem;
#pragma unroll
        for (int n = 0; n < NT; n++) {
            const int hcol = wn * NT * 32 + n * 32 + fr;
#pragma unroll
            for (int m = 0; m < 2; m++)
#pragma unroll
                for (int e = 0; e < 16; e++) {
                    const int row = wm * 64 + m * 32 + (e & 3) + 8 * (e >> 2) + 4 * fh;
                    const float v = acc[m][n][e];
                    hs[row * LDH + hcol] = v > 0.f ? v : 0.f;
                }
        }
        float* w2s = smem + BM * LDH;
        for (int i = tid; i < RD_H * 5; i += 64 * NWAVE) w2s[i] = a.w2[i];
        if (tid < 5) w2s[RD_H * 5 + tid] = a.b2[tid];
        __syncthreads();
        static_assert(64 * NWAVE == 2 * BM, "head epilogue: two threads per row");
        head_dense5_softmax<BM>(hs, w2s, w2s + RD_H * 5 + 8, tds, a, tid);
    }
}

__global__ __launch_bounds__(256) void tcn_in_kernel(const float* __restrict__ x, const float* __restrict__ w ,
                                                      const float* __restrict__ b, float* __restrict__ out,
                                                      const TileDesc* __restrict__ tiles, int dil, ZeroRows zr)
{
    clear_zero_rows(zr);
    const TileDesc td = tiles[(size_t)blockIdx.x * 4 + (threadIdx.x >> 6)];
    const int c4 = (threadIdx.x & 63) * 4;
    const float4 w0 = *(const float4*)(w + c4), w1 = *(const float4*)(w + 256 + c4), w2 = *(const float4*)(w + 512 + c4);
    const float4 bb = *(const float4*)(b + c4);
    const float* xw = x + td.src_row;
    float* ow = out + (size_t)td.seg_row * RD_C;
    const int tend = td.t0 + 32 < td.seg_len ? td.t0 + 32 : td.seg_len;
    for (int t = td.t0; t < tend; t++) {
        const float x2 = xw[t];
        const float x1 = t - dil >= 0 ? xw[t - dil] : 0.f;
        const float x0 = t - 2 * dil >= 0 ? xw[t - 2 * dil] : 0.f;
        float4 v;
        v.x = conv_in_value(bb.x, w0.x, w1.x, w2.x, x0, x1, x2);
        v.y = conv_in_value(bb.y, w0.y, w1.y, w2.y, x0, x1, x2);
        v.z = conv_in_value(bb.z, w0.z, w1.z, w2.z, x0, x1, x2);
        v.w = conv_in_value(bb.w, w0.w, w1.w, w2.w, x0, x1, x2);
        *(float4*)(ow + (size_t)t * RD_C + c4) = v;
    }
}

typedef _Float16 f16x8 __attribute__((ext_vector_type(8)));
typedef _Float16 f16x4 __attribute__((ext_vector_type(4)));
constexpr int ROWH = 2 * RD_C;

struct SplitArgs {
    const _Float16* in;
    _Float16* out;
    const _Float16* wpk;
    const float* bias;
    float inv_scale;
    const _Float16* resid;
    const float* x;
    const float* wmatch;
    const float* bmatch;
    const float* w2;
    const float* b2;
    float* probs;
    int probs_f16;
    int zero_row;
    float* sink;
    const TileDesc* tiles;
    int dil;
};

template <int NT, int TAPS, int EPI>
__global__ __launch_bounds__(256, 2) void tcn_gemm_split_kernel(SplitArgs a)
{
    constexpr int BN = 2 * NT * 32;
    constexpr int BKC = 16;
    constexpr int NCHUNK = TAPS * (RD_C / BKC);
    constexpr int STAGE_FLOATS = (BM + BN) * 16;
    constexpr int NSTAGE = 3;
    constexpr int HEAD_FLOATS = BM * (RD_H + 1) + RD_H * 5 + 8 + BM * 5;
    constexpr int SMEM_FLOATS = (EPI == EPI_HEAD && HEAD_FLOATS > NSTAGE * STAGE_FLOATS) ? HEAD_FLOATS : NSTAGE * STAGE_FLOATS;

    __shared__ __attribute__((aligned(1024))) float smem[SMEM_FLOATS];

    const int tid = threadIdx.x;
    const int lane = tid & 63;
    const int wave = __builtin_amdgcn_readfirstlane(tid >> 6);
    const int wm = wave >> 1;
    const int wn = wave & 1;
    const TileDesc* __restrict__ tds = a.tiles + (size_t)blockIdx.x * 4;
    const TileDesc sdm[2] = {tds[wm * 2], tds[wm * 2 + 1]};
    const bool mval[2] = {sdm[0].seg_len > sdm[0].t0, sdm[1].seg_len > sdm[1].t0};

    const int dma_r = lane >> 2;
    const int dma_ps = lane & 3;
    const TileDesc sst = tds[wave];
    const int64_t d_seg = sst.seg_row, d_alt = sst.alt_row;
    const int d_t0 = sst.t0, d_ain = sst.alt_in;
    const int d_len = sst.seg_len > sst.t0 ? sst.in_len : 0;
    const int lslot = dma_ps ^ ((dma_r >> 2) & 3);
    const int lane_half = (lslot & 1) * 8 + (lslot >> 1) * 32;
    int arow[TAPS][2];
#pragma unroll
    for (int tap = 0; tap < TAPS; tap++)
#pragma unroll
        for (int pc = 0; pc < 2; pc++) {
            const int t = d_t0 + pc * 16 + dma_r - (TAPS - 1 - tap) * a.dil;
            arow[tap][pc] = (t >= 0 && t < d_len) ? (int)((t < d_ain ? d_seg : d_alt) + t) : a.zero_row;
        }
    const char* lanebase = (const char*)(a.in + lane_half);
    const unsigned lane_off = lane * 16;

    constexpr int PB = BN / 64;
    constexpr int NPIECE = 2 + PB;
    auto stage_piece = [&](int chunk, int tap, float* st, int pc) {
        if (pc < 2) {
            const int cc = chunk / TAPS;
            const char* src = lanebase + (size_t)((cc >> 1) * 128 + (cc & 1) * 32) + (uint64_t)(unsigned)arow[tap][pc] * (ROWH * 2);
            glds16_uncounted((const float*)src, st + (wave * 2 + pc) * 256);
        } else {
            const float* wb = (const float*)(a.wpk + (size_t)chunk * BN * 32) + wave * PB * 256;
            float* dst = st + BM * 16 + wave * PB * 256;
            if (pc == 2) glds16_uncounted_saddr<0>(lane_off, wb, dst);
            else if (pc == 3) glds16_uncounted_saddr<1024>(lane_off, wb, dst);
            else if (pc == 4) glds16_uncounted_saddr<2048>(lane_off, wb, dst);
            else glds16_uncounted_saddr<3072>(lane_off, wb, dst);
        }
    };
    auto stage = [&](int chunk, int tap, float* st) {
#pragma unroll
        for (int pc = 0; pc < NPIECE; pc++) stage_piece(chunk, tap, st, pc);
    };

    const int fr = lane & 31;
    const int fh = lane >> 5;
    f32x16 acc[2][NT];
#pragma unroll
    for (int n = 0; n < NT; n++) {
// ... 445 lines not shown
                }
                bf16x4 r3[8][3];
                int tt[8];
#pragma unroll
                for (int i = 0; i < 8; i++) {
                    const int t = sd.t0 + i * 4 + rrow;
                    tt[i] = t;
                    if constexpr (EPI == EPI_RES_IDENT) {
                        const int tc = (interior || t < T) ? t : T - 1;
                        const __bf16* rb = (tc < sd.alt_res ? resw : resalt) + (size_t)tc * ROW3 + hoff;
#pragma unroll
                        for (int q = 0; q < 3; q++) r3[i][q] = *(const bf16x4*)(rb + 16 * q);
                    }
                }
#pragma unroll
                for (int i = 0; i < 8; i++) {
                    const float4 p = *(const float4*)(ts + (i * 4 + rrow) * TSTR + c4);
                    float v[4] = {p.x, p.y, p.z, p.w};
                    const int t = tt[i];
                    const bool inb = interior || t < T;
                    if constexpr (EPI == EPI_RES_IDENT) {
#pragma unroll
                        for (int q = 0; q < 4; q++) {
                            v[q] += (float)r3[i][0][q] + ((float)r3[i][1][q] + (float)r3[i][2][q]);
                            v[q] = v[q] > 0.f ? v[q] : 0.f;
                        }
                    } else if constexpr (EPI == EPI_RES_MATCH) {
                        const float xv = a.x[(size_t)sd.src_row + (inb ? t : T - 1)];
                        const float wq[4] = {wm4.x, wm4.y, wm4.z, wm4.w}, bq[4] = {bm4.x, bm4.y, bm4.z, bm4.w};
#pragma unroll
                        for (int q = 0; q < 4; q++) {
                            v[q] = (bq[q] + xv * wq[q]) + v[q];
                            v[q] = v[q] > 0.f ? v[q] : 0.f;
                        }
                    }
                    bf16x4 o3[3];
#pragma unroll
                    for (int q = 0; q < 4; q++) {
                        __bf16 h, md, l;
                        split3(v[q], h, md, l);
                        o3[0][q] = h;
                        o3[1][q] = md;
                        o3[2][q] = l;
                    }
                    __bf16* ob = outw + (size_t)t * ROW3 + hoff;
#pragma unroll
                    for (int q = 0; q < 3; q++) {
                        bf16x4* d = inb ? (bf16x4*)(ob + 16 * q) : sinkh;
                        *d = o3[q];
                    }
                }
                __builtin_amdgcn_fence(__ATOMIC_RELEASE, "wavefront");
                __builtin_amdgcn_wave_barrier();
            }
        }
    } else {
        constexpr int LDH = RD_H + 1;
        float* hs = smem;
#pragma unroll
        for (int n = 0; n < NT; n++) {
            const int hcol = wn * NT * 32 + n * 32 + fr;
#pragma unroll
            for (int m = 0; m < 2; m++)
#pragma unroll
                for (int e = 0; e < 16; e++) {
                    const int row = wm * 64 + m * 32 + (e & 3) + 8 * (e >> 2) + 4 * fh;
                    const float v = acc[m][n][e];
                    hs[row * LDH + hcol] = v > 0.f ? v : 0.f;
                }
        }
        float* w2s = smem + BM3 * LDH;
        for (int i = tid; i < RD_H * 5; i += 512) w2s[i] = a.w2[i];
        if (tid < 5) w2s[RD_H * 5 + tid] = a.b2[tid];
        __syncthreads();
        head_dense5_softmax<BM3>(hs, w2s, w2s + RD_H * 5 + 8, tds, a, tid);
    }
}

__global__ __launch_bounds__(256) void tcn_in_bf3_kernel(const float* __restrict__ x, const float* __restrict__ w, const float* __restrict__ b,
                                                          __bf16* __restrict__ out, const TileDesc* __restrict__ tiles, int dil, ZeroRows zr)
{
    clear_zero_rows(zr);
    const TileDesc td = tiles[(size_t)blockIdx.x * 4 + (threadIdx.x >> 6)];
    const int c4 = (threadIdx.x & 63) * 4;
    const float4 w0 = *(const float4*)(w + c4), w1 = *(const float4*)(w + 256 + c4), w2 = *(const float4*)(w + 512 + c4);
    const float4 bb = *(const float4*)(b + c4);
    const float* xw = x + td.src_row;
    __bf16* ow = out + (size_t)td.seg_row * ROW3;
    const int hoff = (c4 >> 4) * 48 + (c4 & 15);
    const int tend = td.t0 + 32 < td.seg_len ? td.t0 + 32 : td.seg_len;
    for (int t = td.t0; t < tend; t++) {
        const float x2 = xw[t];
        const float x1 = t - dil >= 0 ? xw[t - dil] : 0.f;
        const float x0 = t - 2 * dil >= 0 ? xw[t - 2 * dil] : 0.f;
        float v[4];
        v[0] = bb.x + x0 * w0.x + x1 * w1.x + x2 * w2.x;
        v[1] = bb.y + x0 * w0.y + x1 * w1.y + x2 * w2.y;
        v[2] = bb.z + x0 * w0.z + x1 * w1.z + x2 * w2.z;
        v[3] = bb.w + x0 * w0.w + x1 * w1.w + x2 * w2.w;
        bf16x4 o3[3];
#pragma unroll
        for (int q = 0; q < 4; q++) {
            const float r = v[q] > 0.f ? v[q] : 0.f;
            __bf16 h, md, l;
            split3(r, h, md, l);
            o3[0][q] = h;
            o3[1][q] = md;
            o3[2][q] = l;
        }
#pragma unroll
        for (int q = 0; q < 3; q++) *(bf16x4*)(ow + (size_t)t * ROW3 + hoff + 16 * q) = o3[q];
    }
}

__global__ void split3_kernel(const float* __restrict__ v, uint16_t* __restrict__ out, size_t n)
{
    const size_t i = (size_t)blockIdx.x * blockDim.x + threadIdx.x;
    if (i >= n) return;
    __bf16 h, m, l;
    split3(v[i], h, m, l);
    out[i] = *(const uint16_t*)&h;
    out[n + i] = *(const uint16_t*)&m;
    out[2 * n + i] = *(const uint16_t*)&l;
}

int timer_begin(hipStream_t st, KernelTimer& tm)
{
    if (tm.enabled && tm.used < tm.starts.size()) RD_HIP(hipEventRecord(tm.starts[tm.used], st));
    return RD_OK;
}
int timer_end(hipStream_t st, KernelTimer& tm, double flops, double bytes, int tag = 0)
{
    if (tm.enabled && tm.used < tm.starts.size()) {
        RD_HIP(hipEventRecord(tm.stops[tm.used], st));
        tm.used++;
        tm.flops += flops;
        tm.bytes += bytes;
        tm.each_flops.push_back(flops);
        tm.each_tag.push_back(tag);
    }
    return RD_OK;
}

}

namespace {

bool fuse_first_conv(const rd_ctx* ctx)
{
    return ctx->conv_fuse && ctx->precision == 0 && ctx->conv_shape == 0 && ctx->model.nblocks >= 1 && ctx->model.dil[0] >= 1 &&
           ctx->model.dil[0] <= FIN_DMAX;
}

int launch_layer(rd_ctx* ctx, hipStream_t st, int b, int kind , const TileDesc* tiles, int n,
                double rows, int zero_row, const float* d_signal, float* Xin, float* Xout, float* MID, float* d_probs, int probs_f16)
{
    if (n <= 0) return RD_OK;
    Model& m = ctx->model;
    const bool split = ctx->precision == 1;
    const bool bf3 = ctx->precision == 2;
    if (kind != 0 && (bf3 || (!split && ctx->conv_shape == 1)))
        RD_REQUIRE(n % 2 == 0, "internal: %d tiles in a layer of 256-row workgroups (lists are padded to pairs)", n);
    int rc;
    ZeroRows zr = {};
    const bool fin = kind == 2 && b == 0 && fuse_first_conv(ctx);
    if (kind == 0 || fin) {
        const size_t row_bytes = (size_t)RD_C * (bf3 ? 6 : 4);
        zr.n16 = (int)(row_bytes / 16);
        zr.row[0] = (uint4*)((char*)Xin + (size_t)zero_row * row_bytes);
        zr.row[1] = (uint4*)((char*)Xout + (size_t)zero_row * row_bytes);
        zr.row[2] = (uint4*)((char*)MID + (size_t)zero_row * row_bytes);
    }
    if (kind == 0 && fuse_first_conv(ctx)) return RD_OK;
    if (bf3) {
        Bf3Args h = {};
        h.zero_row = zero_row;
        h.sink = m.sink;
        h.tiles = tiles;
        if (kind == 0) {
            if ((rc = timer_begin(st, ctx->timer_in))) return rc;
            hipLaunchKernelGGL(tcn_in_bf3_kernel, dim3(n), dim3(256), 0, st, d_signal, m.w_in, m.b_in, (__bf16*)MID, tiles, m.dil[0], zr);
            RD_HIP(hipGetLastError());
            return timer_end(st, ctx->timer_in, 2.0 * rows * RD_C * RD_K, rows * (RD_C * 6.0 + 4.0));
        }
        if (kind == 3) {
            if ((rc = timer_begin(st, ctx->timer_head))) return rc;
            h.in = (const __bf16*)Xin;
            h.wpk = (const __bf16*)m.w3_d1;
            h.bias = m.b_d1;
            h.w2 = m.w_d2;
            h.b2 = m.b_d2;
            h.probs = d_probs;
            h.probs_f16 = probs_f16;
            hipLaunchKernelGGL((tcn_gemm_bf3_kernel<2, 1, EPI_HEAD>), dim3(n / 2), dim3(512), 0, st, h);
            RD_HIP(hipGetLastError());
            return timer_end(st, ctx->timer_head, 2.0 * rows * (RD_C * RD_H + RD_H * 5), rows * (RD_C * 6.0 + 20.0));
        }
        const int wi = 2 * b + (kind == 2 ? 1 : 0);
        h.dil = m.dil[b];
        h.wpk = (const __bf16*)m.w3_conv[wi];
        h.bias = m.b_conv[wi];
        if (kind == 1) {
            h.in = (const __bf16*)Xin;
            h.out = (__bf16*)MID;
        } else {
            h.in = (const __bf16*)MID;
            h.out = (__bf16*)Xout;
            h.resid = (const __bf16*)Xin;
            h.x = d_signal;
            h.wmatch = m.w_match;
            h.bmatch = m.b_match;
        }
        if ((rc = timer_begin(st, ctx->timer_conv))) return rc;
        if (kind == 1) hipLaunchKernelGGL((tcn_gemm_bf3_kernel<4, 3, EPI_RELU>), dim3(n / 2), dim3(512), 0, st, h);
        else if (b == 0) hipLaunchKernelGGL((tcn_gemm_bf3_kernel<4, 3, EPI_RES_MATCH>), dim3(n / 2), dim3(512), 0, st, h);
        else hipLaunchKernelGGL((tcn_gemm_bf3_kernel<4, 3, EPI_RES_IDENT>), dim3(n / 2), dim3(512), 0, st, h);
        RD_HIP(hipGetLastError());
        return timer_end(st, ctx->timer_conv, 2.0 * rows * RD_C * RD_C * RD_K, (kind == 2 && b > 0 ? 3.0 : 2.0) * rows * RD_C * 6.0, kind == 1 ? 0 : b == 0 ? 2 : 1);
    }
    if (kind == 0) {
        if ((rc = timer_begin(st, ctx->timer_in))) return rc;
        if (split)
            hipLaunchKernelGGL(tcn_in_split_kernel, dim3(n), dim3(256), 0, st, d_signal, m.w_in, m.b_in, (_Float16*)MID, tiles, m.dil[0], zr);
        else
            hipLaunchKernelGGL(tcn_in_kernel, dim3(n), dim3(256), 0, st, d_signal, m.w_in, m.b_in, MID, tiles, m.dil[0], zr);
        RD_HIP(hipGetLastError());
        return timer_end(st, ctx->timer_in, 2.0 * rows * RD_C * RD_K, rows * (RD_C * 4.0 + 4.0));
    }
    if (kind == 3) {
        if ((rc = timer_begin(st, ctx->timer_head))) return rc;
        if (split) {
            SplitArgs h = {};
            h.zero_row = zero_row;
            h.sink = m.sink;
            h.tiles = tiles;
            h.in = (const _Float16*)Xin;
            h.wpk = (const _Float16*)m.ws_d1;
            h.inv_scale = m.inv_scale_d1;
            h.bias = m.b_d1;
            h.w2 = m.w_d2;
            h.b2 = m.b_d2;
            h.probs = d_probs;
            h.probs_f16 = probs_f16;
            hipLaunchKernelGGL((tcn_gemm_split_kernel<2, 1, EPI_HEAD>), dim3(n), dim3(256), 0, st, h);
        } else {
            ConvArgs h = {};
            h.zero_row = zero_row;
            h.sink = m.sink;
            h.tiles = tiles;
            h.in = Xin;
            h.wpk = m.w_d1;
            h.bias = m.b_d1;
            h.w2 = m.w_d2;
            h.b2 = m.b_d2;
            h.probs = d_probs;
            h.probs_f16 = probs_f16;
            if (ctx->conv_shape == 1) hipLaunchKernelGGL((tcn_gemm_kernel<2, 1, EPI_HEAD, 4>), dim3(n / 2), dim3(512), 0, st, h);
            else hipLaunchKernelGGL((tcn_gemm_kernel<2, 1, EPI_HEAD>), dim3(n), dim3(256), 0, st, h);
        }
        RD_HIP(hipGetLastError());
        return timer_end(st, ctx->timer_head, 2.0 * rows * (RD_C * RD_H + RD_H * 5), rows * (RD_C * 4.0 + 20.0));
    }
    const int wi = 2 * b + (kind == 2 ? 1 : 0);
    ConvArgs a = {};
    a.zero_row = zero_row;
    a.sink = m.sink;
    a.dil = m.dil[b];
    a.tiles = tiles;
    a.wpk = m.w_conv[wi];
    a.bias = m.b_conv[wi];
    SplitArgs sa = {};
    sa.zero_row = zero_row;
    sa.sink = m.sink;
    sa.dil = m.dil[b];
    sa.tiles = tiles;
    sa.wpk = (const _Float16*)m.ws_conv[wi];
    sa.inv_scale = m.inv_scale[wi];
    sa.bias = m.b_conv[wi];
    if (kind == 1) {
        a.in = Xin;
        a.out = MID;
        sa.in = (const _Float16*)Xin;
        sa.out = (_Float16*)MID;
    } else {
        a.in = MID;
        a.out = Xout;
        a.resid = Xin;
        a.x = d_signal;
        a.wmatch = m.w_match;
        a.bmatch = m.b_match;
        sa.in = (const _Float16*)MID;
        sa.out = (_Float16*)Xout;
        sa.resid = (const _Float16*)Xin;
        sa.x = d_signal;
        sa.wmatch = m.w_match;
        sa.bmatch = m.b_match;
    }
    if ((rc = timer_begin(st, ctx->timer_conv))) return rc;
    if (kind == 1) {
        if (split) hipLaunchKernelGGL((tcn_gemm_split_kernel<4, 3, EPI_RELU>), dim3(n), dim3(256), 0, st, sa);
        else if (ctx->conv_shape == 1) hipLaunchKernelGGL((tcn_gemm_kernel<4, 3, EPI_RELU, 4>), dim3(n / 2), dim3(512), 0, st, a);
        else hipLaunchKernelGGL((tcn_gemm_kernel<4, 3, EPI_RELU>), dim3(n), dim3(256), 0, st, a);
    } else if (b == 0) {
        if (fin) {
            a.w_in = m.w_in;
            a.b_in = m.b_in;
            a.zr = zr;
            a.in = nullptr;
        }
        if (split) hipLaunchKernelGGL((tcn_gemm_split_kernel<4, 3, EPI_RES_MATCH>), dim3(n), dim3(256), 0, st, sa);
        else if (ctx->conv_shape == 1) hipLaunchKernelGGL((tcn_gemm_kernel<4, 3, EPI_RES_MATCH, 4>), dim3(n / 2), dim3(512), 0, st, a);
        else if (fin) hipLaunchKernelGGL((tcn_gemm_kernel<4, 3, EPI_RES_MATCH, 2, true>), dim3(n), dim3(256), 0, st, a);
        else hipLaunchKernelGGL((tcn_gemm_kernel<4, 3, EPI_RES_MATCH>), dim3(n), dim3(256), 0, st, a);
    } else {
        if (split) hipLaunchKernelGGL((tcn_gemm_split_kernel<4, 3, EPI_RES_IDENT>), dim3(n), dim3(256), 0, st, sa);
        else if (ctx->conv_shape == 1) hipLaunchKernelGGL((tcn_gemm_kernel<4, 3, EPI_RES_IDENT, 4>), dim3(n / 2), dim3(512), 0, st, a);
        else hipLaunchKernelGGL((tcn_gemm_kernel<4, 3, EPI_RES_IDENT>), dim3(n), dim3(256), 0, st, a);
    }
    RD_HIP(hipGetLastError());
    return timer_end(st, ctx->timer_conv, 2.0 * rows * RD_C * RD_C * RD_K, (kind == 2 && b > 0 ? 3.0 : 2.0) * rows * RD_C * 4.0, kind == 1 ? 0 : b == 0 ? 2 : 1);
}

}

int rd_split3_dev(rd_ctx* ctx, const float* d_in, size_t n, uint16_t* d_out)
{
    if (n == 0) return RD_OK;
    hipLaunchKernelGGL(split3_kernel, dim3((unsigned)((n + 255) / 256)), dim3(256), 0, ctx->stream, d_in, d_out, n);
    RD_HIP(hipGetLastError());
    return RD_OK;
}

namespace {
struct MaskedStream {
    int device, cus;
    bool complement, in_use;
    hipStream_t st;
};
std::vector<MaskedStream> g_masked;
std::mutex g_masked_mu;
}

int rd_masked_stream_acquire(int device, int cus_per_xcd, bool complement, hipStream_t* out)
{
    std::lock_guard<std::mutex> lk(g_masked_mu);
    for (MaskedStream& m : g_masked)
        if (!m.in_use && m.device == device && m.cus == cus_per_xcd && m.complement == complement) {
            m.in_use = true;
            *out = m.st;
            return RD_OK;
        }
    uint32_t mask[RD_XCDS] = {0};
    const int nbits = RD_XCDS * 32, k = RD_XCDS * cus_per_xcd;
    for (int i = 0; i < nbits; i++)
        if ((i < k) != complement) mask[i / 32] |= 1u << (i % 32);
    hipStream_t st = nullptr;
    RD_HIP(hipExtStreamCreateWithCUMask(&st, RD_XCDS, mask));
    g_masked.push_back({device, cus_per_xcd, complement, true, st});
    *out = st;
    return RD_OK;
}

void rd_masked_stream_release(hipStream_t st)
{
    if (!st) return;
    (void)hipStreamSynchronize(st);
    std::lock_guard<std::mutex> lk(g_masked_mu);
    for (MaskedStream& m : g_masked)
        if (m.st == st) m.in_use = false;
}

int rd_lane_get(rd_ctx* ctx, int lane, FwdLane** out)
{
    if (lane < 0 || lane >= 2 * RD_MAX_LANES) {
        rd_set_error("forward lane %d out of range", lane);
        return RD_ERR_ARG;
    }
    FwdLane& L = ctx->lanes[lane];
    if (!L.st) {
        if (lane == 0) L.st = ctx->stream;
        else if (lane < RD_MAX_LANES) {
            RD_HIP(hipStreamCreateWithFlags(&L.st, hipStreamNonBlocking));
        }
        else {
            if (ctx->part_cus < 1 || ctx->part_cus > 31) {
                rd_set_error("internal: partitioned lane %d without a decode partition", lane);
                return RD_ERR_STATE;
            }
            int rc = rd_masked_stream_acquire(ctx->device, ctx->part_cus, true, &L.st);
            if (rc) return rc;
        }
    }
    if (!L.done) RD_HIP(hipEventCreateWithFlags(&L.done, hipEventDisableTiming));
    *out = &L;
    return RD_OK;
}

int rd_part_set(rd_ctx* ctx, int cus_per_xcd)
{
    if (ctx->part_cus == cus_per_xcd) return RD_OK;
    for (int i = RD_MAX_LANES; i < 2 * RD_MAX_LANES; i++) {
        FwdLane& L = ctx->lanes[i];
        if (L.st) {
            rd_masked_stream_release(L.st);
            L.st = nullptr;
        }
    }
    ctx->part_cus = cus_per_xcd;
    return RD_OK;
}

int rd_sync_lanes(rd_ctx* ctx)
{
    RD_HIP(hipStreamSynchronize(ctx->stream));
    for (int i = 1; i < 2 * RD_MAX_LANES; i++)
        if (ctx->lanes[i].st) RD_HIP(hipStreamSynchronize(ctx->lanes[i].st));
    return RD_OK;
}

int rd_forward_tiles_dev(rd_ctx* ctx, const float* d_signal, const TileLists& tl, int64_t total_rows, void* d_probs, int lane, int probs_f16)
{
    Model& m = ctx->model;
    if (!m.loaded) {
        rd_set_error("rd_forward: no weights loaded (rd_load_weights)");
        return RD_ERR_STATE;
    }
    if (total_rows == 0) return RD_OK;
    int rc = RD_OK;
    if (m.split_stale && ctx->precision != 0 && (rc = rd_model_refresh_split(ctx))) return rc;
    FwdLane* L = nullptr;
    if ((rc = rd_lane_get(ctx, lane, &L))) return rc;
    if (total_rows >= INT32_MAX) {
        rd_set_error("rd_forward: %lld rows in one batch (the kernels index rows with 32 bits)", (long long)total_rows);
        return RD_ERR_ARG;
    }
    const size_t row_bytes = (size_t)RD_C * (ctx->precision == 2 ? 6 : 4);
    const size_t act_bytes = (size_t)(total_rows + 1) * row_bytes;
    if (L->act[0].reserve(act_bytes) || L->act[1].reserve(act_bytes) || L->act[2].reserve(act_bytes)) return RD_ERR_NOMEM;
    float* Xin = L->act[0].as<float>();
    float* Xout = L->act[1].as<float>();
    float* MID = L->act[2].as<float>();
    const int zero_row = (int)total_rows;
    const int nl = 2 * m.nblocks + 1;
    for (int li = 0; li < nl; li++) {
        const int b = li == nl - 1 ? m.nblocks : li / 2;
        const int kind = li == nl - 1 ? 3 : (li == 0 ? 0 : (li & 1 ? 2 : 1));
        if ((rc = launch_layer(ctx, L->st, b, kind, tl.d[li], tl.n[li], (double)tl.rows[li], zero_row, d_signal, Xin, Xout, MID, (float*)d_probs, probs_f16))) return rc;
        if (kind == 2) {
            float* t = Xin;
            Xin = Xout;
            Xout = t;
        }
    }
    RD_HIP(hipEventRecord(L->done, L->st));
    return RD_OK;
}

int rd_uniform_tiles(rd_ctx* ctx, int nW, int T, TileLists* out)
{
    const int subs = (T + 31) / 32;
    const size_t nsub = (size_t)nW * subs;
    const size_t n = (nsub + 7) / 8 * 2;
    if (ctx->tiles_nW != nW || ctx->tiles_T != T) {
        std::vector<TileDesc> h(n * 4);
        for (size_t i = 0; i < n * 4; i++) {
            TileDesc& td = h[i];
            const size_t w = i / subs;
            const int k = (int)(i % subs);
            const bool real = i < nsub;
            td.seg_row = real ? (int64_t)w * T : 0;
            td.src_row = td.seg_row;
            td.alt_row = td.seg_row;
            td.t0 = real ? k * 32 : 0;
            td.seg_len = real ? T : 0;
            td.in_len = td.seg_len;
            td.alt_in = INT32_MAX;
            td.alt_res = INT32_MAX;
            td.pad_ = 0;
        }
        if (ctx->ws_tiles.reserve(h.size() * sizeof(TileDesc))) return RD_ERR_NOMEM;
        if (int rcs = rd_sync_lanes(ctx)) return rcs;
        RD_HIP(hipMemcpy(ctx->ws_tiles.p, h.data(), h.size() * sizeof(TileDesc), hipMemcpyHostToDevice));
        ctx->tiles_nW = nW;
        ctx->tiles_T = T;
    }
    const int nl = 2 * ctx->model.nblocks + 1;
    for (int li = 0; li < RD_MAX_LAYERS; li++) {
        out->d[li] = li < nl ? ctx->ws_tiles.as<TileDesc>() : nullptr;
        out->n[li] = li < nl ? (int)n : 0;
        out->rows[li] = li < nl ? (int64_t)nW * T : 0;
    }
    return RD_OK;
}

int rd_forward_dev(rd_ctx* ctx, const float* d_windows, int nW, int T, float* d_probs, int lane)
{
    RD_REQUIRE(nW >= 0 && T >= 1, "rd_forward: bad shape nW=%d T=%d", nW, T);
    if (nW == 0) return RD_OK;
    if (!ctx->model.loaded) {
        rd_set_error("rd_forward: no weights loaded (rd_load_weights)");
        return RD_ERR_STATE;
    }
    TileLists tl;
    int rc = rd_uniform_tiles(ctx, nW, T, &tl);
    if (rc) return rc;
    return rd_forward_tiles_dev(ctx, d_windows, tl, (int64_t)nW * T, d_probs, lane);
}
```

radian_amd/csrc/pipe_reads.hip:

```cpp
#include "common.h"
#include "plan.h"
#include "../../include/radian_hip.h"
#include "../../include/radian_hip_diag.h"

#include <stdio.h>
#include <time.h>
#include <stdlib.h>
#include <string.h>

using namespace rdi;

namespace {

__global__ void copy_bytes_kernel(char* __restrict__ dst, const char* __restrict__ src, size_t n)
{
    const size_t i0 = ((size_t)blockIdx.x * blockDim.x + threadIdx.x) * 16;
    const size_t stride = (size_t)gridDim.x * blockDim.x * 16;
    if ((((uintptr_t)dst | (uintptr_t)src) & 15) == 0) {
        for (size_t i = i0; i + 16 <= n; i += stride) *(uint4*)(dst + i) = *(const uint4*)(src + i);
        const size_t tail = n & ~(size_t)15;
        if (blockIdx.x == 0 && threadIdx.x < (n & 15)) dst[tail + threadIdx.x] = src[tail + threadIdx.x];
    } else {
        for (size_t i = i0; i < n; i += stride)
            for (size_t k = i; k < n && k < i + 16; k++) dst[k] = src[k];
// ... 309 lines not shown
    p->delivered += (int64_t)s.subs.size();
    slot_reset(s);
    return rc;
}

int slot_launch_decode(rd_ctx* ctx, ReadsPipe* p, RSlot& s)
{
    if (s.seqs.empty() || s.busy) return RD_OK;
    int rc;
    const size_t n = s.seqs.size();
    s.order.clear();
    for (size_t i = 0; i < n; i++)
        if (s.seqs[i].is64) s.order.push_back((int)i);
    s.n64 = (int)s.order.size();
    for (size_t i = 0; i < n; i++)
        if (!s.seqs[i].is64) s.order.push_back((int)i);
    auto by_len = [&](int x, int y) { return s.seqs[x].len != s.seqs[y].len ? s.seqs[x].len > s.seqs[y].len : x < y; };
    std::sort(s.order.begin(), s.order.begin() + s.n64, by_len);
    std::sort(s.order.begin() + s.n64, s.order.end(), by_len);
    const size_t a8 = align_up(n * 8, 256), a4 = align_up(n * 4, 256);
    const size_t o_off2 = a8, o_node = 2 * a8, o_lab = 3 * a8, o_len = 4 * a8, o_split = o_len + a4, o_llen = o_split + a4;
    const size_t meta_bytes = o_llen + a4;
    if ((rc = pinned_reserve(&s.h_meta, &s.h_meta_cap, meta_bytes))) return rc;
    if (s.meta.reserve(meta_bytes)) return RD_ERR_NOMEM;
    char* hm = (char*)s.h_meta;
    int64_t *h1 = (int64_t*)hm, *h2 = (int64_t*)(hm + o_off2), *hn = (int64_t*)(hm + o_node), *hl = (int64_t*)(hm + o_lab);
    int32_t *hlen = (int32_t*)(hm + o_len), *hsp = (int32_t*)(hm + o_split);
    for (size_t k = 0; k < n; k++) {
        const RSeq& q = s.seqs[s.order[k]];
        h1[k] = q.off1;
        h2[k] = q.off2;
        hsp[k] = q.split;
        hlen[k] = q.len;
        hl[k] = q.label_off;
    }
    std::vector<TrieRun> runs[2];
    rd_plan_trie_runs(ctx, s.W, 0, s.n64, [&](int k) { return (int64_t)hlen[k]; }, hn, runs[0]);
    rd_plan_trie_runs(ctx, s.W, s.n64, (int)n, [&](int k) { return (int64_t)hlen[k]; }, hn, runs[1]);
    if (s.labels.reserve((size_t)s.labels_total + 16)) return RD_ERR_NOMEM;
    const size_t ho_len = align_up((size_t)s.labels_total + 16, 256);
    s.status_off = ho_len + align_up(n * 4, 256);
    if ((rc = pinned_reserve(&s.h_out, &s.h_out_cap, s.status_off + (size_t)s.n_reads * 4 + 16))) return rc;
    const bool on_part = s.part && ((int)n <= part_seq_limit(s.part, s.W) || s.oversub);
    hipStream_t ds = on_part ? p->s_part : p->s_dec;
    if (p->last_dec && p->last_dec != ds) {
        RD_HIP(hipEventRecord(p->ev_switch, p->last_dec));
        RD_HIP(hipStreamWaitEvent(ds, p->ev_switch, 0));
    }
    p->last_dec = ds;
    s.dec_stream = ds;
    for (int l = 0; l < 2 * RD_MAX_LANES; l++)
        if (s.lane_mask & (1u << l)) RD_HIP(hipStreamWaitEvent(ds, ctx->lanes[l].done, 0));
    const bool kc = s.mode == 1;
    if ((rc = copy_on_stream(s.meta.p, s.h_meta, o_llen, ds, kc))) return rc;
    char* dm = (char*)s.meta.p;
    Calib::Dec* cd = nullptr;
    const bool q_launch = on_part && (int)n > part_seq_limit(s.part, s.W);
    if (s.mode == 1 && s.longest > 0 && (!q_launch || s.steps_total / queue_resident_seqs(s.part, s.W) <= s.longest * 4 / 5)) {
        calib_harvest(p->calib);
        Calib::Dec& d = p->calib.d[p->calib.d_next % Calib::ND];
        if (!d.pending) {
            cd = &d;
            p->calib.d_next++;
            d.longest = s.longest;
            d.key = Calib::key_of(s.W, on_part ? std::min(3, part_waves_per_simd(s.part, s.W, (int64_t)n)) : 0, ctx->decode_math, ctx->precision, s.use_lm);
            RD_HIP(hipEventRecord(d.e0, ds));
        }
    }
    for (int pass = 0; pass < 2; pass++)
    for (const TrieRun& run : runs[pass]) {
        const int k0 = run.k0, k1 = run.k1;
        const bool chunk = s.mode == 0;
        const void* src = pass == 0 ? s.mat.p : s.probs.p;
        const int ptype = pass == 0 ? 1 : (s.f16 ? 2 : 0);
        rc = rd_decode_dev(ctx, src, ptype, (const int64_t*)dm + k0, (const int32_t*)(dm + o_len) + k0, (const int64_t*)(dm + o_node) + k0,
                           (const int64_t*)(dm + o_lab) + k0, k1 - k0, run.nodes, s.W, s.use_lm, s.s_thr, s.r_thr, s.labels.as<uint8_t>(),
                           (int32_t*)(dm + o_llen) + k0, nullptr, ds, chunk ? (const int64_t*)(dm + o_off2) + k0 : nullptr,
                           chunk ? (const int32_t*)(dm + o_split) + k0 : nullptr, on_part ? RD_XCDS * s.part : 0,
                           on_part && (int)n > part_seq_limit(s.part, s.W) ? RD_XCDS * s.part * 4 * 3 : 0);
        if (rc) return rc;
    }
    if (cd) {
        RD_HIP(hipEventRecord(cd->e1, ds));
        cd->pending = true;
    }
    if ((rc = copy_on_stream(s.h_out, s.labels.p, (size_t)s.labels_total, ds, kc))) return rc;
    if ((rc = copy_on_stream((char*)s.h_out + ho_len, dm + o_llen, n * 4, ds, kc))) return rc;
    if (s.n_reads && s.status.p)
        if ((rc = copy_on_stream((char*)s.h_out + s.status_off, s.status.p, (size_t)s.n_reads * 4, ds, kc))) return rc;
    RD_HIP(hipEventRecord(s.dec_done, ds));
    s.busy = true;
    s.launch_seq = ++p->launches;
    if (s.mode == 1 && s.part && s.oversub && (int)s.seqs.size() > part_seq_limit(s.part, s.W)) p->queue_launches++;
    return RD_OK;
}

int close_group(rd_ctx* ctx, ReadsPipe* p)
{
    int rc = slot_launch_decode(ctx, p, p->slot[p->cur]);
    if (rc) return rc;
    p->cur = (p->cur + 1) % ReadsPipe::NSLOT;
    return RD_OK;
}

int flush_groups(rd_ctx* ctx, ReadsPipe* p)
{
    int rc;
    if ((rc = slot_launch_decode(ctx, p, p->slot[p->cur]))) return rc;
    for (;;) {
        RSlot* first = nullptr;
        for (RSlot& s : p->slot)
            if (s.busy && (!first || s.launch_seq < first->launch_seq)) first = &s;
        if (!first) return RD_OK;
        if ((rc = slot_collect(p, *first))) return rc;
    }
}

int open_slot(rd_ctx* ctx, ReadsPipe* p, int mode, int W, int f16, int use_lm, double s_thr, double r_thr, int part, int64_t rows,
              int64_t expect_rows, RSlot** out)
{
    int rc;
    RSlot* s = &p->slot[p->cur];
    if (s->busy && (rc = slot_collect(p, *s))) return rc;
    const bool same = s->mode == mode && s->W == W && s->f16 == f16 && s->use_lm == use_lm && s->s_thr == s_thr && s->r_thr == r_thr && s->part == part;
    if (!s->seqs.empty() && (!same || s->rows + rows > s->cap_rows)) {
        if (same) s->grow_hint = 2 * (s->rows + rows);
        if ((rc = close_group(ctx, p))) return rc;
        s = &p->slot[p->cur];
    }
    if (s->busy && (rc = slot_collect(p, *s))) return rc;
    if (s->seqs.empty()) {
        int64_t want = rows > s->grow_hint ? rows : s->grow_hint;
        if (expect_rows > want) want = expect_rows;
        if (want > s->cap_rows) {
            const int64_t cap = want + want / 4;
            if (s->probs.reserve((size_t)cap * 20)) return RD_ERR_NOMEM;
            s->cap_rows = cap;
        }
        if (mode == 1 && s->mat.reserve((size_t)(s->cap_rows + 1) * 40)) return RD_ERR_NOMEM;
    }
    s->mode = mode;
    s->part = part;
    s->W = W;
    s->f16 = f16;
    s->use_lm = use_lm;
    s->s_thr = s_thr;
    s->r_thr = r_thr;
    *out = s;
    return RD_OK;
}

int lane_plan_build(rd_ctx* ctx, RLane& R, const int64_t* read_off, int n_reads, int chunk, int step, int mode, bool* miss, size_t* n_desc)
{
    const int halo = rd_model_halo(ctx);
    *miss = !R.key.matches(ctx->model, read_off, n_reads, chunk, step, mode, halo);
    int rc = *miss ? R.key.rebuild(ctx->model, read_off, n_reads, chunk, step, mode, halo, R.plan, &R.streamed, &R.n_desc) : RD_OK;
    *n_desc = R.n_desc;
    return rc;
}

int lane_plan_upload(FwdLane* L, RLane& R, char* hs)
{
    ReadsPlan& P = R.plan;
    const size_t off = plan_fill_lists(P, R.tiles.as<TileDesc>(), (TileDesc*)hs, R.lists);
    if (off) {
        int rc_ = copy_on_stream(R.tiles.p, hs, off * sizeof(TileDesc), L->st);
        if (rc_) return rc_;
    }
    for (int li = 0; li < RD_MAX_LAYERS; li++) std::vector<TileDesc>().swap(P.tiles[li]);
    R.key.valid = true;
    return RD_OK;
}

int check_args(rd_ctx* ctx, const void* signal, const int64_t* read_off, int n_reads, int chunk_len, int step, int W, bool window_bound = false)
{
    const int rc = rd_check_reads_args(ctx, signal, read_off, n_reads, chunk_len, step, W);
    if (rc == RD_ERR_ARG) return rc;
    RD_REQUIRE(!window_bound || rd_decode_len_ok(W, chunk_len), "chunk_len %d too long for beam width %d (1 + W * rows < 2^29)", chunk_len, W);
    RD_REQUIRE(read_off[0] == 0, "read_off[0] must be 0");
    for (int r = 0; r < n_reads; r++) {
        RD_REQUIRE(read_off[r + 1] > read_off[r], "read %d is empty (the caller skips empty reads, basecall.py:77-82)", r);
        RD_REQUIRE(window_bound || rd_decode_len_ok(W, read_off[r + 1] - read_off[r]), "read %d has %lld samples; beam width %d supports at most %lld (1 + W * rows < 2^29)", r,
                   (long long)(read_off[r + 1] - read_off[r]), W, (long long)((((int64_t)1 << 29) - 2) / W));
    }
    return rc;
}

int join_group(rd_ctx* ctx, ReadsPipe* p, RSlot* s, RSub&& sb, const std::vector<RSeq>& seqs, int64_t rows, int64_t rows64, int64_t labels_total,
               int64_t longest, int64_t steps, int plane)
{
    s->seqs.insert(s->seqs.end(), seqs.begin(), seqs.end());
    s->rows64 = rows64;
    s->labels_total = labels_total;
    s->lane_mask |= 1u << plane;
    s->n_reads += sb.n_reads;
    s->rows += rows;
    if (longest > s->longest) s->longest = longest;
    s->steps_total += steps;
    s->subs.push_back(std::move(sb));
    p->next_lane = (plane % RD_MAX_LANES + 1) % ctx->pipe_lanes;
    p->submitted++;
    const int W = s->W, part = s->part, use_lm = s->use_lm;
    bool close;
    if (s->mode == 1) {
        const int limit = part ? part_seq_limit(part, W) : 0;
        const bool few = part && ((int)s->seqs.size() <= limit || s->oversub);
        const int m = few ? std::min(3, part_waves_per_simd(part, W, (int64_t)s->seqs.size())) : 0;
        int64_t need = chain_rows(ctx, p->calib, W, m, use_lm) * s->longest;
        const int resident = part ? queue_resident_seqs(part, W) : 1;
        const int64_t need_chain = need;
        if (s->oversub) need = std::max(need, chain_rows(ctx, p->calib, W, 3, use_lm) * 5 / 6 * s->steps_total / resident);
        close = s->rows >= need || s->rows >= kGroupRowsCap || (s->oversub && s->rows >= need_chain && (int)s->seqs.size() >= 3 * resident);
        close = close || p->launches == 0;
    } else {
        close = (int)s->subs.size() >= ctx->pipe_group;
    }
    if (close) return close_group(ctx, p);
    return RD_OK;
}

int submit(rd_ctx* ctx, int mode, const float* d_signal, const int16_t* raw, int clip, const int64_t* read_off, int n_reads, int chunk_len,
           int step, int W, int use_lm, double s_thr, double r_thr, uint8_t* labels_out, const int64_t* label_off, int32_t* label_len,
           int32_t* status)
{
    int rc;
    RD_REQUIRE_WIDTH_LM(ctx, W, use_lm && mode == 1);
    RD_HIP(hipSetDevice(ctx->device));
    ReadsPipe* p = nullptr;
    if ((rc = rpipe_get(ctx, &p))) return rc;
    const int part_cus = mode == 1 && ctx->n_cu == RD_XCDS * 32 ? (ctx->part_mode < 0 ? auto_part_cus(W) : ctx->part_mode) : 0;
    const int part = part_cus && n_reads <= part_seq_limit(part_cus, W) / 2 ? part_cus : 0;
    if (part && part != p->part_cus) {
        if ((rc = flush_groups(ctx, p))) return rc;
        if (p->s_part) {
            rd_masked_stream_release(p->s_part);
            p->s_part = nullptr;
            if (p->last_dec != p->s_dec) p->last_dec = nullptr;
        }
        if ((rc = rd_part_set(ctx, part))) return rc;
        if ((rc = rd_masked_stream_acquire(ctx->device, part, false, &p->s_part))) return rc;
        p->part_cus = part;
    }
    const int lane = p->next_lane % ctx->pipe_lanes;
    const int plane = lane + (part ? RD_MAX_LANES : 0);
    FwdLane* L = nullptr;
    if ((rc = rd_lane_get(ctx, plane, &L))) return rc;
    RLane& R = p->lane[plane];
    const size_t n_samples = (size_t)read_off[n_reads];
    const int f16 = ctx->logits_f16;

    if (!R.staged) RD_HIP(hipEventCreateWithFlags(&R.staged, hipEventDisableTiming));
    bool miss = false;
    size_t n_desc = 0;
    if ((rc = lane_plan_build(ctx, R, read_off, n_reads, chunk_len, step, mode, &miss, &n_desc))) return rc;
    const ReadsPlan& P = R.plan;
    const bool stages = raw || miss || mode == 1;
    const size_t st_off = align_up((size_t)(n_reads + 1) * 8, 256);
    const size_t st_raw = raw ? align_up(n_samples * 2 + 16, 256) : 0;
    const size_t st_desc = miss ? align_up(n_desc * sizeof(TileDesc), 256) : 0;
    const size_t st_asm = mode == 1 ? align_up((size_t)n_reads * sizeof(AsmRead), 256) : 0;
    const size_t o_raw = st_off, o_desc = raw ? st_off + st_raw : 0, o_asm = o_desc + st_desc;
    if (stages && R.staged_pending) {
        RD_HIP(hipEventSynchronize(R.staged));
        R.staged_pending = false;
    }
    if (stages && (rc = pinned_reserve(&R.h_stage, &R.h_stage_cap, o_asm + st_asm + 256))) return rc;
    char* hs = (char*)R.h_stage;
    const size_t d_asm = align_up(n_desc * sizeof(TileDesc), 256);
    if (d_asm + st_asm + 256 > R.tiles.cap) {
        RD_HIP(hipStreamSynchronize(L->st));
        if (!miss) {
            rd_set_error("internal: descriptor buffer too small on a plan hit");
            return RD_ERR_STATE;
        }
        if (R.tiles.reserve(d_asm + st_asm + (d_asm + st_asm) / 4 + 256)) {
            R.key.invalidate();
            return RD_ERR_NOMEM;
        }
    }
    const size_t d_st = st_off, d_raw = st_off + align_up((size_t)n_reads * 4, 256);
    if (raw && (d_raw + st_raw > R.raw.cap || n_samples * 4 + 16 > R.sig.cap)) {
        RD_HIP(hipStreamSynchronize(L->st));
        if (R.raw.reserve(d_raw + st_raw + (d_raw + st_raw) / 4) || R.sig.reserve(n_samples * 4 + n_samples + 16)) return RD_ERR_NOMEM;
    }

    RSlot* s = nullptr;
    int64_t expect_rows = ctx->pipe_group * P.total_rows;
    int64_t longest_b = 0;
    if (mode == 1) {
        for (int r = 0; r < n_reads; r++) longest_b = std::max<int64_t>(longest_b, read_off[r + 1] - read_off[r]);
        calib_harvest(p->calib);
        expect_rows = std::min<int64_t>(kGroupRowsCap, chain_rows(ctx, p->calib, W, part ? 2 : 0, use_lm) * longest_b + 2 * P.total_rows);
    }
    if (mode == 1 && part) {
        RSlot& g = p->slot[p->cur];
        const int limit = part_seq_limit(part, W);
        if (!g.busy && !g.seqs.empty() && g.mode == 1 && g.part == part && g.W == W && !g.oversub && (int)g.seqs.size() <= limit &&
            (int)g.seqs.size() + n_reads > limit) {
            const double ns = p->calib.ns_row[ctx->precision] > 0.0 ? p->calib.ns_row[ctx->precision] : kDefaultNsPerRow;
            const double* us3 = p->calib.find(Calib::key_of(W, 3, ctx->decode_math, ctx->precision, use_lm));
            const double pace3 = us3 ? *us3 : (double)chain_rows_default(W, true) * kDefaultNsPerRow * 1e-3;
            const double work_ms = (double)(g.steps_total + (int64_t)n_samples) * pace3 * 1e-3 / (double)queue_resident_seqs(part, W);
            const double fwd_ms = (double)(g.rows + P.total_rows) * ns * 1e-6;
            const int64_t chain_need = chain_rows(ctx, p->calib, W, 3, use_lm) * std::max<int64_t>(g.longest, longest_b);
            const bool uncovered = g.rows + P.total_rows < chain_need;
            if ((work_ms <= 1.25 * fwd_ms || uncovered) && W <= RD_LANE_MAX_W  && !(use_lm && ctx->lm.hashed)) g.oversub = true;
            else {
                p->limit_closes++;
                if ((rc = close_group(ctx, p))) return rc;
            }
        }
    }
    if ((rc = open_slot(ctx, p, mode, W, f16, use_lm, s_thr, r_thr, part, P.total_rows, expect_rows, &s))) return rc;

    RSub sb;
    sb.seq0 = (int)s->seqs.size();
    sb.read0 = s->n_reads;
    sb.n_reads = n_reads;
    sb.user_labels = labels_out;
    sb.user_lens = label_len;
    sb.user_status = raw ? status : nullptr;
    std::vector<RSeq> seqs;
// ... 355 lines not shown
```

radian_amd/csrc/plan.h:

```cpp
#pragma once
#include "common.h"

namespace rdi {

int64_t assembled_rows(int nW, int T, int pad, int step);
int assembled_is_f64(int nW, int T, int pad, int step);

struct ReadRows {
    int64_t N, row64;
    int is64;
};
int64_t classify_reads(const int32_t* win_off, const int32_t* pad, int n_reads, int T, int step, int64_t rows64, std::vector<ReadRows>& out);

inline int count_windows(int64_t N, int chunk, int step) { return (N < chunk ? 0 : (int)((N - chunk) / step) + 1) + 1; }

struct WindowGeom {
    int nW, pad;
};
inline WindowGeom window_geom(int64_t N, int chunk, int step)
{
    WindowGeom g;
    g.nW = count_windows(N, chunk, step);
    const int64_t last_start = (int64_t)(g.nW - 1) * step;
    g.pad = (int)(chunk - (N - last_start));
    return g;
}

struct ReadsPlan {
    int n_layers = 0;
    bool per_layer = false;
    std::vector<TileDesc> tiles[RD_MAX_LAYERS];
    int64_t rows[RD_MAX_LAYERS] = {0};
    std::vector<int64_t> off1, off2;
    std::vector<int32_t> split, valid;
    std::vector<int32_t> read_win_off;
    std::vector<int64_t> read_row;
    int64_t total_rows = 0;
    int n_windows = 0;
};

int plan_reads_chunk(const Model& m, const int64_t* read_off, int n_reads, int chunk, int step, int halo, ReadsPlan& P);
int plan_reads_global(const Model& m, const int64_t* read_off, int n_reads, int chunk, int step, int halo, ReadsPlan& P, bool* streamed);
size_t plan_pad_tiles(ReadsPlan& P);

struct PlanKey {
    bool valid = false;
    int chunk = -1, step = -1, mode = -1, halo = -1, nblocks = -1;
    int dil[RD_MAX_BLOCKS] = {0};
    std::vector<int64_t> lens;
    bool matches(const Model& m, const int64_t* read_off, int n_reads, int chunk_, int step_, int mode_, int halo_) const;
    void invalidate() { valid = false; }
    int rebuild(const Model& m, const int64_t* read_off, int n_reads, int chunk_, int step_, int mode_, int halo_, ReadsPlan& P, bool* streamed,
                size_t* n_desc);
};
size_t plan_fill_lists(const ReadsPlan& P, const TileDesc* d_base, TileDesc* h_dst, TileLists& lists);

int rd_check_reads_args(rd_ctx* ctx, const void* signal, const int64_t* read_off, int n_reads, int chunk_len, int step, int W);

int pinned_reserve(void** p, size_t* cap, size_t bytes);

}
```

radian_amd/csrc/plan.hip:

```cpp
#include "plan.h"

#include <string.h>

namespace rdi {

int64_t assembled_rows(int nW, int T, int pad, int step)
{
    int64_t N = 0;
    for (int i = 0; i < nW; i++) {
        int rows = (i == nW - 1) ? T - pad : T;
        int64_t end = (int64_t)i * step + rows;
        if (rows > 0 && end > N) N = end;
    }
    return N;
}

int assembled_is_f64(int nW, int T, int pad, int step)
{
    if (step >= T) return 0;
    if (nW >= 3) return 1;
    if (nW == 2 && T - pad > 0) return 1;
    return 0;
}

int64_t classify_reads(const int32_t* win_off, const int32_t* pad, int n_reads, int T, int step, int64_t rows64, std::vector<ReadRows>& out)
{
    out.resize(n_reads);
    for (int r = 0; r < n_reads; r++) {
        const int nW = win_off[r + 1] - win_off[r];
        out[r].N = assembled_rows(nW, T, pad[r], step);
        out[r].is64 = assembled_is_f64(nW, T, pad[r], step);
        out[r].row64 = rows64;
        if (out[r].is64) rows64 += out[r].N;
    }
    return rows64;
}

void add_segment(std::vector<TileDesc>& list, int64_t& rows, int64_t seg_row, int64_t src_row, int len, int in_len,
                 int64_t alt_row = 0, int alt_in = INT32_MAX, int alt_res = INT32_MAX)
{
    for (int t0 = 0; t0 < len; t0 += 32) {
        TileDesc td;
        td.seg_row = seg_row;
        td.src_row = src_row;
        td.alt_row = alt_row;
        td.t0 = t0;
        td.seg_len = len;
        td.in_len = in_len;
        td.alt_in = alt_in;
        td.alt_res = alt_res;
        td.pad_ = 0;
        list.push_back(td);
    }
    rows += len;
}

struct LayerHalo {
    int h_in, h_res, h_out;
};
void layer_halos(const Model& m, LayerHalo* lh)
{
    int H = 0;
    for (int b = 0; b < m.nblocks; b++) {
        const int d = m.dil[b];
        lh[2 * b] = {H, H, H + 2 * d};
        lh[2 * b + 1] = {H + 2 * d, H, H + 4 * d};
        H += 4 * d;
    }
    lh[2 * m.nblocks] = {H, H, H};
}

int plan_reads_chunk(const Model& m, const int64_t* read_off, int n_reads, int chunk, int step, int halo, ReadsPlan& P)
{
    LayerHalo lh[RD_MAX_LAYERS];
    layer_halos(m, lh);
    P.n_layers = 2 * m.nblocks + 1;
    P.per_layer = true;
    int64_t row = 0;
    P.read_win_off.assign(1, 0);
    std::vector<TileDesc> heads[RD_MAX_LAYERS];
    for (int r = 0; r < n_reads; r++) {
        const int64_t N = read_off[r + 1] - read_off[r];
        RD_REQUIRE(N >= 1, "read %d is empty", r);
        RD_REQUIRE(N < INT32_MAX, "read %d too long", r);
        const WindowGeom g = window_geom(N, chunk, step);
        const int64_t stream_row = row;
        P.read_row.push_back(stream_row);
        for (int li = 0; li < P.n_layers; li++) add_segment(P.tiles[li], P.rows[li], stream_row, read_off[r], (int)N, (int)N);
        row += N;
        for (int i = 0; i < g.nW; i++) {
            const int valid = (i < g.nW - 1) ? chunk : chunk - g.pad;
            const int h = (i == 0) ? 0 : (halo < valid ? halo : valid);
            int64_t o1 = stream_row + (int64_t)i * step;
            if (h > 0) {
                o1 = row;
                const int64_t alt = stream_row + (int64_t)i * step;
                for (int li = 0; li < P.n_layers; li++) {
                    const int len = lh[li].h_out < valid ? lh[li].h_out : valid;
                    if (len > 0)
                        add_segment(heads[li], P.rows[li], row, read_off[r] + (int64_t)i * step, len, valid, alt, lh[li].h_in, lh[li].h_res);
                }
                row += h;
            }
            P.off1.push_back(o1);
            P.off2.push_back(stream_row + (int64_t)i * step);
            P.split.push_back(h);
            P.valid.push_back(valid);
        }
        P.n_windows += g.nW;
        P.read_win_off.push_back(P.n_windows);
    }
    for (int li = 0; li < P.n_layers; li++) P.tiles[li].insert(P.tiles[li].end(), heads[li].begin(), heads[li].end());
    P.total_rows = row;
    return RD_OK;
}

int plan_reads_global(const Model& m, const int64_t* read_off, int n_reads, int chunk, int step, int halo, ReadsPlan& P, bool* streamed)
{
    const bool st = step <= chunk - halo;
    *streamed = st;
    P.n_layers = 2 * m.nblocks + 1;
    P.per_layer = false;
    int64_t row = 0;
    P.read_win_off.assign(1, 0);
    for (int r = 0; r < n_reads; r++) {
        const int64_t N = read_off[r + 1] - read_off[r];
        RD_REQUIRE(N >= 1, "read %d is empty", r);
        RD_REQUIRE(N < INT32_MAX, "read %d too long", r);
        const WindowGeom g = window_geom(N, chunk, step);
        P.read_row.push_back(row);
        if (st) {
            add_segment(P.tiles[0], P.rows[0], row, read_off[r], (int)N, (int)N);
            row += N;
        } else {
            for (int i = 0; i < g.nW; i++) {
                const int valid = (i < g.nW - 1) ? chunk : chunk - g.pad;
                if (valid > 0) add_segment(P.tiles[0], P.rows[0], row + (int64_t)i * chunk, read_off[r] + (int64_t)i * step, valid, valid);
            }
            row += (int64_t)g.nW * chunk;
        }
        P.valid.push_back(g.pad);
        P.n_windows += g.nW;
        P.read_win_off.push_back(P.n_windows);
    }
    P.total_rows = row;
    return RD_OK;
}

size_t plan_pad_tiles(ReadsPlan& P)
{
    size_t total = 0;
    for (int li = 0; li < P.n_layers; li++)
        if (P.per_layer || li == 0) {
            std::vector<TileDesc>& v = P.tiles[li];
            while (v.size() % 8) {
                TileDesc e = {};
                e.alt_in = e.alt_res = INT32_MAX;
                v.push_back(e);
            }
            total += v.size();
        }
    return total;
}

bool PlanKey::matches(const Model& m, const int64_t* read_off, int n_reads, int chunk_, int step_, int mode_, int halo_) const
{
    if (!valid || chunk != chunk_ || step != step_ || mode != mode_ || halo != halo_ || nblocks != m.nblocks || read_off[0] != 0 ||
        lens.size() != (size_t)n_reads)
        return false;
    for (int b = 0; b < m.nblocks; b++)
        if (dil[b] != m.dil[b]) return false;
    for (int r = 0; r < n_reads; r++)
        if (lens[r] != read_off[r + 1] - read_off[r]) return false;
    return true;
}

int PlanKey::rebuild(const Model& m, const int64_t* read_off, int n_reads, int chunk_, int step_, int mode_, int halo_, ReadsPlan& P, bool* streamed,
                     size_t* n_desc)
{
    invalidate();
    P = ReadsPlan();
    int rc = mode_ == 0 ? plan_reads_chunk(m, read_off, n_reads, chunk_, step_, halo_, P) : plan_reads_global(m, read_off, n_reads, chunk_, step_, halo_, P, streamed);
    if (rc) return rc;
    *n_desc = plan_pad_tiles(P);
    chunk = chunk_;
    step = step_;
    mode = mode_;
    halo = halo_;
    nblocks = m.nblocks;
    for (int b = 0; b < RD_MAX_BLOCKS; b++) dil[b] = b < m.nblocks ? m.dil[b] : 0;
    lens.resize(n_reads);
    for (int r = 0; r < n_reads; r++) lens[r] = read_off[r + 1] - read_off[r];
    return RD_OK;
}

size_t plan_fill_lists(const ReadsPlan& P, const TileDesc* d_base, TileDesc* h_dst, TileLists& lists)
{
    size_t off = 0;
    for (int li = 0; li < RD_MAX_LAYERS; li++) {
        lists.d[li] = nullptr;
        lists.n[li] = 0;
        lists.rows[li] = 0;
    }
    for (int li = 0; li < P.n_layers; li++) {
        if (P.per_layer || li == 0) {
            const std::vector<TileDesc>& v = P.tiles[li];
            if (!v.empty()) memcpy(h_dst + off, v.data(), v.size() * sizeof(TileDesc));
            lists.d[li] = d_base + off;
            lists.n[li] = (int)(v.size() / 4);
            lists.rows[li] = P.rows[li];
            off += v.size();
        } else {
            lists.d[li] = lists.d[0];
            lists.n[li] = lists.n[0];
            lists.rows[li] = lists.rows[0];
        }
    }
    return off;
}

int pinned_reserve(void** p, size_t* cap, size_t bytes)
{
    if (bytes <= *cap) return RD_OK;
    if (*p) (void)hipHostFree(*p);
    *p = nullptr;
    *cap = 0;
    size_t want = align_up(bytes + bytes / 8, 1 << 16);
    RD_HIP(hipHostMalloc(p, want, hipHostMallocDefault));
    *cap = want;
    return RD_OK;
}

}
```

Before: 27.13 million.

## Pack short window-head segments into 4-row granules within 32-row conv sub-tiles

```diff
diff --git a/include/radian_hip.h b/include/radian_hip.h
--- a/include/radian_hip.h
+++ b/include/radian_hip.h
@@ -30,6 +30,7 @@
 int rd_destroy(rd_ctx* ctx);
 int rd_sync(rd_ctx* ctx);
 int rd_set_precision(rd_ctx* ctx, int mode);
+int rd_set_head_pack(rd_ctx* ctx, int on);
 
 typedef struct rd_weights_header {
     uint32_t magic;
diff --git a/radian_amd/_lib.py b/radian_amd/_lib.py
--- a/radian_amd/_lib.py
+++ b/radian_amd/_lib.py
@@ -25,6 +25,7 @@
     "rd_destroy": (c_i, [c_vp]),
     "rd_sync": (c_i, [c_vp]),
     "rd_set_precision": (c_i, [c_vp, c_i]),
+    "rd_set_head_pack": (c_i, [c_vp, c_i]),
     "rd_load_weights": (c_i, [c_vp, c_vp, c_sz]),
     "rd_load_lm": (c_i, [c_vp, c_vp, c_i]),
     "rd_load_lm_absent": (c_i, [c_vp, c_i]),
diff --git a/radian_amd/backend.py b/radian_amd/backend.py
--- a/radian_amd/backend.py
+++ b/radian_amd/backend.py
@@ -1,4 +1,5 @@
 import ctypes
+import os
 
 import numpy as np
 
@@ -226,6 +227,8 @@
         self._h = h
         self.device_id = device_id
         self.lm_k = None
+        if os.environ.get("RD_HEAD_PACK", "1").strip() == "0":
+            self.set_head_pack(False)
         self._tickets = {}
 
     def _check(self, rc):
@@ -256,6 +259,9 @@
     def set_precision(self, mode):
         code = {"fp32": 0, "f16x3": 1, "bf16x3": 2}[mode] if isinstance(mode, str) else int(mode)
         self._check(self._L.rd_set_precision(self._h, code))
+
+    def set_head_pack(self, on):
+        self._check(self._L.rd_set_head_pack(self._h, 1 if on else 0))
 
     def set_conv_shape(self, shape):
         self._check(self._L.rd_set_conv_shape(self._h, int(shape)))
diff --git a/radian_amd/csrc/api.hip b/radian_amd/csrc/api.hip
--- a/radian_amd/csrc/api.hip
+++ b/radian_amd/csrc/api.hip
@@ -370,11 +370,11 @@
         pc = new PlanCache();
         ctx->plan_cache[mode] = pc;
     }
-    const int halo = rd_model_halo(ctx);
-    if (!(pc->d_tiles.p && pc->key.matches(ctx->model, read_off, n_reads, chunk, step, mode, halo))) {
+    const int halo = rd_model_halo(ctx), pack = rd_head_pack_mode(ctx);
+    if (!(pc->d_tiles.p && pc->key.matches(ctx->model, read_off, n_reads, chunk, step, mode, halo, pack))) {
         RD_REQUIRE(read_off[0] == 0, "read_off[0] must be 0");
         size_t total = 0;
-        int rc = pc->key.rebuild(ctx->model, read_off, n_reads, chunk, step, mode, halo, pc->plan, &pc->streamed, &total);
+        int rc = pc->key.rebuild(ctx->model, read_off, n_reads, chunk, step, mode, halo, pc->plan, &pc->streamed, &total, pack);
         if (rc) return rc;
         if (pc->d_tiles.reserve(total * sizeof(TileDesc) + 16)) return RD_ERR_NOMEM;
         if ((rc = rd_sync_lanes(ctx))) return rc;
diff --git a/radian_amd/csrc/common.h b/radian_amd/csrc/common.h
--- a/radian_amd/csrc/common.h
+++ b/radian_amd/csrc/common.h
@@ -100,9 +100,13 @@
 constexpr int RD_MAX_LAYERS = 2 * 16 + 1;
 struct TileLists {
     const TileDesc* d[RD_MAX_LAYERS];
+    const TileDesc* g[RD_MAX_LAYERS];
     int n[RD_MAX_LAYERS];
     int64_t rows[RD_MAX_LAYERS];
 };
+
+enum { RD_PACK_NONE = 0, RD_PACK_FUSED = 1, RD_PACK_ALL = 2 };
+inline bool plan_layer_packed(int pack, int li, int n_layers) { return pack != RD_PACK_NONE && li >= (pack == RD_PACK_ALL ? 1 : 2) && li < n_layers - 1; }
 
 struct KernelTimer {
     bool enabled = false;
@@ -129,6 +133,7 @@
     int decode_math = 1;
     int conv_fuse = 1;
     int conv_shape = 0;
+    int head_pack = 1;
     int logits_f16 = 0;
     hipStream_t stream = nullptr;
     hipStream_t stream_hi = nullptr;
@@ -170,6 +175,7 @@
 int rd_forward_dev(rd_ctx* ctx, const float* d_windows, int nW, int T, float* d_probs, int lane = 0);
 int rd_forward_tiles_dev(rd_ctx* ctx, const float* d_signal, const TileLists& tiles, int64_t total_rows, void* d_probs, int lane = 0,
                          int probs_f16 = 0 );
+int rd_head_pack_mode(const rd_ctx* ctx);
 int rd_lane_get(rd_ctx* ctx, int lane, FwdLane** out);
 constexpr int RD_XCDS = 8;
 int rd_part_set(rd_ctx* ctx, int cus_per_xcd);
diff --git a/radian_amd/csrc/context.hip b/radian_amd/csrc/context.hip
--- a/radian_amd/csrc/context.hip
+++ b/radian_amd/csrc/context.hip
@@ -217,6 +217,14 @@
     return RD_OK;
 }
 
+extern "C" int rd_set_head_pack(rd_ctx* ctx, int on)
+{
+    RD_REQUIRE(ctx, "rd_set_head_pack: null context");
+    RD_REQUIRE(on == 0 || on == 1, "rd_set_head_pack: %d (1 = window heads packed into 4-row granules, 0 = 32-row sub-tiles of their own)", on);
+    ctx->head_pack = on;
+    return RD_OK;
+}
+
 extern "C" int rd_set_decode_partition(rd_ctx* ctx, int cus_per_xcd)
 {
     RD_REQUIRE(ctx, "rd_set_decode_partition: null context");
diff --git a/radian_amd/csrc/forward.hip b/radian_amd/csrc/forward.hip
--- a/radian_amd/csrc/forward.hip
+++ b/radian_amd/csrc/forward.hip
@@ -44,6 +44,7 @@
     int zero_row;
     float* sink;
     const TileDesc* tiles;
+    const TileDesc* gran;
     int dil;
     const float* w_in;
     const float* b_in;
@@ -159,9 +160,10 @@
 }
 
 constexpr int FIN_DMAX = 2;
-template <int NT, int TAPS, int EPI, int WM = 2, bool FIN = false>
+template <int NT, int TAPS, int EPI, int WM = 2, bool FIN = false, bool PACK = false>
 __global__ __launch_bounds__(128 * WM, WM == 2 ? 2 : 1) void tcn_gemm_kernel(ConvArgs a)
 {
+    static_assert(!PACK || (!FIN && WM == 2 && TAPS == 3 && EPI != EPI_HEAD), "PACK: the 128-row conv launches but the fused one");
     static_assert(!FIN || (EPI == EPI_RES_MATCH && WM == 2 && TAPS == 3 && NT == 4), "FIN: block 0's second conv, product shape");
     constexpr int BM = 64 * WM;
     constexpr int NWAVE = 2 * WM;
@@ -195,13 +197,29 @@
     const int d_len = sst.seg_len > sst.t0 ? sst.in_len : 0;
     const int lane_slot = (dma_ps ^ ((dma_r >> 2) & 3)) * 4;
     int arow[TAPS][2];
-#pragma unroll
-    for (int tap = 0; tap < TAPS; tap++)
+    if (PACK && sst.pad_ != 0) {
 #pragma unroll
         for (int pc = 0; pc < 2; pc++) {
-            const int t = d_t0 + pc * 16 + dma_r - (TAPS - 1 - tap) * a.dil;
-            arow[tap][pc] = (t >= 0 && t < d_len) ? (int)((t < d_ain ? d_seg : d_alt) + t) : a.zero_row;
-        }
+            const int row = pc * 16 + dma_r;
+            const TileDesc* __restrict__ g = a.gran + (sst.pad_ - 1) + (row >> 2);
+            const int64_t g_seg = g->seg_row, g_alt = g->alt_row;
+            const int g_t = g->t0 + (row & 3), g_ain = g->alt_in;
+            const int g_len = g->seg_len > g->t0 ? g->in_len : 0;
+#pragma unroll
+            for (int tap = 0; tap < TAPS; tap++) {
+                const int t = g_t - (TAPS - 1 - tap) * a.dil;
+                arow[tap][pc] = (t >= 0 && t < g_len) ? (int)((t < g_ain ? g_seg : g_alt) + t) : a.zero_row;
+            }
+        }
+    } else {
+#pragma unroll
+        for (int tap = 0; tap < TAPS; tap++)
+#pragma unroll
+            for (int pc = 0; pc < 2; pc++) {
+                const int t = d_t0 + pc * 16 + dma_r - (TAPS - 1 - tap) * a.dil;
+                arow[tap][pc] = (t >= 0 && t < d_len) ? (int)((t < d_ain ? d_seg : d_alt) + t) : a.zero_row;
+            }
+    }
     const char* lanebase = (const char*)(a.in + lane_slot);
     const unsigned lane_off = lane * 16;
 
@@ -382,7 +400,21 @@
             float* __restrict__ outw = a.out + (size_t)sd.seg_row * RD_C;
             const float* __restrict__ resw = a.resid + (size_t)sd.seg_row * RD_C;
             const float* __restrict__ resalt = a.resid + (size_t)sd.alt_row * RD_C;
-            const bool interior = sd.t0 + 32 <= T;
+            const bool packed = PACK && sd.pad_ != 0;
+            const bool interior = !packed && sd.t0 + 32 <= T;
+            auto store_group = [&](int k, float*& g_out, const float*& g_res, const float*& g_ralt, int64_t& src_row, int& t0, int& len, int& alt_res) {
+                g_out = outw, g_res = resw, g_ralt = resalt, src_row = sd.src_row;
+                t0 = sd.t0 + k * 4, len = T, alt_res = sd.alt_res;
+                if constexpr (PACK) {
+                    if (packed) {
+                        const uint64_t ga = (uint64_t)(a.gran + __builtin_amdgcn_readfirstlane(sd.pad_ - 1 + k));
+                        const __attribute__((address_space(4))) TileDesc* g = (const __attribute__((address_space(4))) TileDesc*)ga;
+                        const int64_t g_seg = g->seg_row, g_alt = g->alt_row;
+                        g_out = a.out + (size_t)g_seg * RD_C, g_res = a.resid + (size_t)g_seg * RD_C, g_ralt = a.resid + (size_t)g_alt * RD_C;
+                        src_row = g->src_row, t0 = g->t0, len = g->seg_len, alt_res = g->alt_res;
+                    }
+                }
+            };
             auto to_patch = [&](int np) {
 #pragma unroll
                 for (int j = 0; j < 2; j++) {
@@ -440,22 +472,34 @@
                     int tt[4];
 #pragma unroll
                     for (int i = 0; i < 4; i++) {
-                        const int t = sd.t0 + (ih + i) * 4 + rrow;
+                        float* g_out;
+                        const float *g_res, *g_ralt;
+                        int64_t g_src;
+                        int g_t0, g_len, g_ares;
+                        store_group(ih + i, g_out, g_res, g_ralt, g_src, g_t0, g_len, g_ares);
+                        const int t = g_t0 + rrow;
                         tt[i] = t;
                         if constexpr (EPI == EPI_RES_IDENT) {
-                            const int tc = (interior || t < T) ? t : T - 1;
-                            rv[i] = *(const float4*)((tc < sd.alt_res ? resw : resalt) + (size_t)tc * RD_C + ch);
+                            const int tlast = packed && g_len == 0 ? 0 : g_len - 1;
+                            const int tc = (interior || t < g_len) ? t : tlast;
+                            rv[i] = *(const float4*)((tc < g_ares ? g_res : g_ralt) + (size_t)tc * RD_C + ch);
                         }
                     }
 #pragma unroll
                     for (int i = 0; i < 4; i++) {
                         float4 v = *(const float4*)(ts + ((ih + i) * 4 + rrow) * TSTR + c4);
+                        float* outw;
+                        const float *g_res, *g_ralt;
+                        int64_t g_src;
+                        int g_t0, T, g_ares;
+                        store_group(ih + i, outw, g_res, g_ralt, g_src, g_t0, T, g_ares);
                         const int t = tt[i];
                         const bool inb = interior || t < T;
                         if constexpr (EPI == EPI_RES_IDENT) {
                             v.x += rv[i].x; v.y += rv[i].y; v.z += rv[i].z; v.w += rv[i].w;
                         } else if constexpr (EPI == EPI_RES_MATCH) {
-                            const float xv = a.x[(size_t)sd.src_row + (inb ? t : T - 1)];
+                            const int tlast = packed && T == 0 ? 0 : T - 1;
+                            const float xv = a.x[(size_t)g_src + (inb ? t : tlast)];
                             v.x = (bm4.x + xv * wm4.x) + v.x; v.y = (bm4.y + xv * wm4.y) + v.y;
                             v.z = (bm4.z + xv * wm4.z) + v.z; v.w = (bm4.w + xv * wm4.w) + v.w;
                             v.x = v.x > 0.f ? v.x : 0.f; v.y = v.y > 0.f ? v.y : 0.f;
@@ -1207,7 +1251,7 @@
            ctx->model.dil[0] <= FIN_DMAX;
 }
 
-int launch_layer(rd_ctx* ctx, hipStream_t st, int b, int kind , const TileDesc* tiles, int n,
+int launch_layer(rd_ctx* ctx, hipStream_t st, int b, int kind , const TileDesc* tiles, const TileDesc* gran, int n,
                 double rows, int zero_row, const float* d_signal, float* Xin, float* Xout, float* MID, float* d_probs, int probs_f16)
 {
     if (n <= 0) return RD_OK;
@@ -1219,6 +1263,10 @@
     int rc;
     ZeroRows zr = {};
     const bool fin = kind == 2 && b == 0 && fuse_first_conv(ctx);
+    if (gran && (split || bf3 || ctx->conv_shape != 0 || fin || (kind != 1 && kind != 2))) {
+        rd_set_error("internal: a tile list with packed heads at a launch that does not take one");
+        return RD_ERR_STATE;
+    }
     if (kind == 0 || fin) {
         const size_t row_bytes = (size_t)RD_C * (bf3 ? 6 : 4);
         zr.n16 = (int)(row_bytes / 16);
@@ -1322,6 +1370,7 @@
     a.sink = m.sink;
     a.dil = m.dil[b];
     a.tiles = tiles;
+    a.gran = gran;
     a.wpk = m.w_conv[wi];
     a.bias = m.b_conv[wi];
     SplitArgs sa = {};
@@ -1355,6 +1404,7 @@
     if (kind == 1) {
         if (split) hipLaunchKernelGGL((tcn_gemm_split_kernel<4, 3, EPI_RELU>), dim3(n), dim3(256), 0, st, sa);
         else if (ctx->conv_shape == 1) hipLaunchKernelGGL((tcn_gemm_kernel<4, 3, EPI_RELU, 4>), dim3(n / 2), dim3(512), 0, st, a);
+        else if (gran) hipLaunchKernelGGL((tcn_gemm_kernel<4, 3, EPI_RELU, 2, false, true>), dim3(n), dim3(256), 0, st, a);
         else hipLaunchKernelGGL((tcn_gemm_kernel<4, 3, EPI_RELU>), dim3(n), dim3(256), 0, st, a);
     } else if (b == 0) {
         if (fin) {
@@ -1366,16 +1416,24 @@
         if (split) hipLaunchKernelGGL((tcn_gemm_split_kernel<4, 3, EPI_RES_MATCH>), dim3(n), dim3(256), 0, st, sa);
         else if (ctx->conv_shape == 1) hipLaunchKernelGGL((tcn_gemm_kernel<4, 3, EPI_RES_MATCH, 4>), dim3(n / 2), dim3(512), 0, st, a);
         else if (fin) hipLaunchKernelGGL((tcn_gemm_kernel<4, 3, EPI_RES_MATCH, 2, true>), dim3(n), dim3(256), 0, st, a);
+        else if (gran) hipLaunchKernelGGL((tcn_gemm_kernel<4, 3, EPI_RES_MATCH, 2, false, true>), dim3(n), dim3(256), 0, st, a);
         else hipLaunchKernelGGL((tcn_gemm_kernel<4, 3, EPI_RES_MATCH>), dim3(n), dim3(256), 0, st, a);
     } else {
         if (split) hipLaunchKernelGGL((tcn_gemm_split_kernel<4, 3, EPI_RES_IDENT>), dim3(n), dim3(256), 0, st, sa);
         else if (ctx->conv_shape == 1) hipLaunchKernelGGL((tcn_gemm_kernel<4, 3, EPI_RES_IDENT, 4>), dim3(n / 2), dim3(512), 0, st, a);
+        else if (gran) hipLaunchKernelGGL((tcn_gemm_kernel<4, 3, EPI_RES_IDENT, 2, false, true>), dim3(n), dim3(256), 0, st, a);
         else hipLaunchKernelGGL((tcn_gemm_kernel<4, 3, EPI_RES_IDENT>), dim3(n), dim3(256), 0, st, a);
     }
     RD_HIP(hipGetLastError());
     return timer_end(st, ctx->timer_conv, 2.0 * rows * RD_C * RD_C * RD_K, (kind == 2 && b > 0 ? 3.0 : 2.0) * rows * RD_C * 4.0, kind == 1 ? 0 : b == 0 ? 2 : 1);
 }
 
+}
+
+int rd_head_pack_mode(const rd_ctx* ctx)
+{
+    if (!ctx->head_pack || ctx->precision != 0 || ctx->conv_shape != 0) return RD_PACK_NONE;
+    return fuse_first_conv(ctx) ? RD_PACK_FUSED : RD_PACK_ALL;
 }
 
 int rd_split3_dev(rd_ctx* ctx, const float* d_in, size_t n, uint16_t* d_out)
@@ -1500,7 +1558,7 @@
     for (int li = 0; li < nl; li++) {
         const int b = li == nl - 1 ? m.nblocks : li / 2;
         const int kind = li == nl - 1 ? 3 : (li == 0 ? 0 : (li & 1 ? 2 : 1));
-        if ((rc = launch_layer(ctx, L->st, b, kind, tl.d[li], tl.n[li], (double)tl.rows[li], zero_row, d_signal, Xin, Xout, MID, (float*)d_probs, probs_f16))) return rc;
+        if ((rc = launch_layer(ctx, L->st, b, kind, tl.d[li], tl.g[li], tl.n[li], (double)tl.rows[li], zero_row, d_signal, Xin, Xout, MID, (float*)d_probs, probs_f16))) return rc;
         if (kind == 2) {
             float* t = Xin;
             Xin = Xout;
@@ -1542,6 +1600,7 @@
     const int nl = 2 * ctx->model.nblocks + 1;
     for (int li = 0; li < RD_MAX_LAYERS; li++) {
         out->d[li] = li < nl ? ctx->ws_tiles.as<TileDesc>() : nullptr;
+        out->g[li] = nullptr;
         out->n[li] = li < nl ? (int)n : 0;
         out->rows[li] = li < nl ? (int64_t)nW * T : 0;
     }
diff --git a/radian_amd/csrc/pipe_reads.hip b/radian_amd/csrc/pipe_reads.hip
--- a/radian_amd/csrc/pipe_reads.hip
+++ b/radian_amd/csrc/pipe_reads.hip
@@ -485,9 +485,9 @@
 
 int lane_plan_build(rd_ctx* ctx, RLane& R, const int64_t* read_off, int n_reads, int chunk, int step, int mode, bool* miss, size_t* n_desc)
 {
-    const int halo = rd_model_halo(ctx);
-    *miss = !R.key.matches(ctx->model, read_off, n_reads, chunk, step, mode, halo);
-    int rc = *miss ? R.key.rebuild(ctx->model, read_off, n_reads, chunk, step, mode, halo, R.plan, &R.streamed, &R.n_desc) : RD_OK;
+    const int halo = rd_model_halo(ctx), pack = rd_head_pack_mode(ctx);
+    *miss = !R.key.matches(ctx->model, read_off, n_reads, chunk, step, mode, halo, pack);
+    int rc = *miss ? R.key.rebuild(ctx->model, read_off, n_reads, chunk, step, mode, halo, R.plan, &R.streamed, &R.n_desc, pack) : RD_OK;
     *n_desc = R.n_desc;
     return rc;
 }
@@ -500,7 +500,10 @@
         int rc_ = copy_on_stream(R.tiles.p, hs, off * sizeof(TileDesc), L->st);
         if (rc_) return rc_;
     }
-    for (int li = 0; li < RD_MAX_LAYERS; li++) std::vector<TileDesc>().swap(P.tiles[li]);
+    for (int li = 0; li < RD_MAX_LAYERS; li++) {
+        std::vector<TileDesc>().swap(P.tiles[li]);
+        std::vector<TileDesc>().swap(P.gran[li]);
+    }
     R.key.valid = true;
     return RD_OK;
 }
diff --git a/radian_amd/csrc/plan.h b/radian_amd/csrc/plan.h
--- a/radian_amd/csrc/plan.h
+++ b/radian_amd/csrc/plan.h
@@ -30,6 +30,7 @@
     int n_layers = 0;
     bool per_layer = false;
     std::vector<TileDesc> tiles[RD_MAX_LAYERS];
+    std::vector<TileDesc> gran[RD_MAX_LAYERS];
     int64_t rows[RD_MAX_LAYERS] = {0};
     std::vector<int64_t> off1, off2;
     std::vector<int32_t> split, valid;
@@ -39,19 +40,20 @@
     int n_windows = 0;
 };
 
-int plan_reads_chunk(const Model& m, const int64_t* read_off, int n_reads, int chunk, int step, int halo, ReadsPlan& P);
+int plan_reads_chunk(const Model& m, const int64_t* read_off, int n_reads, int chunk, int step, int halo, ReadsPlan& P, int pack = RD_PACK_NONE);
 int plan_reads_global(const Model& m, const int64_t* read_off, int n_reads, int chunk, int step, int halo, ReadsPlan& P, bool* streamed);
 size_t plan_pad_tiles(ReadsPlan& P);
 
 struct PlanKey {
     bool valid = false;
     int chunk = -1, step = -1, mode = -1, halo = -1, nblocks = -1;
+    int pack = -1;
     int dil[RD_MAX_BLOCKS] = {0};
     std::vector<int64_t> lens;
-    bool matches(const Model& m, const int64_t* read_off, int n_reads, int chunk_, int step_, int mode_, int halo_) const;
+    bool matches(const Model& m, const int64_t* read_off, int n_reads, int chunk_, int step_, int mode_, int halo_, int pack_ = RD_PACK_NONE) const;
     void invalidate() { valid = false; }
     int rebuild(const Model& m, const int64_t* read_off, int n_reads, int chunk_, int step_, int mode_, int halo_, ReadsPlan& P, bool* streamed,
-                size_t* n_desc);
+                size_t* n_desc, int pack_ = RD_PACK_NONE);
 };
 size_t plan_fill_lists(const ReadsPlan& P, const TileDesc* d_base, TileDesc* h_dst, TileLists& lists);
 
diff --git a/radian_amd/csrc/plan.hip b/radian_amd/csrc/plan.hip
--- a/radian_amd/csrc/plan.hip
+++ b/radian_amd/csrc/plan.hip
@@ -55,6 +55,43 @@
     rows += len;
 }
 
+void add_granules(std::vector<TileDesc>& gran, int64_t& rows, int64_t seg_row, int64_t src_row, int len, int in_len, int64_t alt_row, int alt_in, int alt_res)
+{
+    for (int t0 = 0; t0 < len; t0 += 4) {
+        TileDesc td;
+        td.seg_row = seg_row;
+        td.src_row = src_row;
+        td.alt_row = alt_row;
+        td.t0 = t0;
+        td.seg_len = len;
+        td.in_len = in_len;
+        td.alt_in = alt_in;
+        td.alt_res = alt_res;
+        td.pad_ = 0;
+        gran.push_back(td);
+    }
+    rows += len;
+}
+
+void pack_heads(std::vector<TileDesc>& list, std::vector<TileDesc>& gran)
+{
+    while (gran.size() % 8) {
+        TileDesc e = {};
+        e.alt_in = e.alt_res = INT32_MAX;
+        gran.push_back(e);
+    }
+    for (size_t g0 = 0; g0 < gran.size(); g0 += 8) {
+        TileDesc td = {};
+        td.alt_in = td.alt_res = INT32_MAX;
+        for (size_t g = g0; g < g0 + 8; g++) {
+            const int left = gran[g].seg_len - gran[g].t0;
+            td.seg_len += left < 4 ? left : 4;
+        }
+        td.pad_ = (int32_t)(g0 + 1);
+        list.push_back(td);
+    }
+}
+
 struct LayerHalo {
     int h_in, h_res, h_out;
 };
@@ -70,7 +107,7 @@
     lh[2 * m.nblocks] = {H, H, H};
 }
 
-int plan_reads_chunk(const Model& m, const int64_t* read_off, int n_reads, int chunk, int step, int halo, ReadsPlan& P)
+int plan_reads_chunk(const Model& m, const int64_t* read_off, int n_reads, int chunk, int step, int halo, ReadsPlan& P, int pack)
 {
     LayerHalo lh[RD_MAX_LAYERS];
     layer_halos(m, lh);
@@ -97,7 +134,10 @@
                 const int64_t alt = stream_row + (int64_t)i * step;
                 for (int li = 0; li < P.n_layers; li++) {
                     const int len = lh[li].h_out < valid ? lh[li].h_out : valid;
-                    if (len > 0)
+                    if (len <= 0) continue;
+                    if (plan_layer_packed(pack, li, P.n_layers))
+                        add_granules(P.gran[li], P.rows[li], row, read_off[r] + (int64_t)i * step, len, valid, alt, lh[li].h_in, lh[li].h_res);
+                    else
                         add_segment(heads[li], P.rows[li], row, read_off[r] + (int64_t)i * step, len, valid, alt, lh[li].h_in, lh[li].h_res);
                 }
                 row += h;
@@ -110,7 +150,10 @@
         P.n_windows += g.nW;
         P.read_win_off.push_back(P.n_windows);
     }
-    for (int li = 0; li < P.n_layers; li++) P.tiles[li].insert(P.tiles[li].end(), heads[li].begin(), heads[li].end());
+    for (int li = 0; li < P.n_layers; li++) {
+        P.tiles[li].insert(P.tiles[li].end(), heads[li].begin(), heads[li].end());
+        pack_heads(P.tiles[li], P.gran[li]);
+    }
     P.total_rows = row;
     return RD_OK;
 }
@@ -158,14 +201,14 @@
                 e.alt_in = e.alt_res = INT32_MAX;
                 v.push_back(e);
             }
-            total += v.size();
+            total += v.size() + P.gran[li].size();
         }
     return total;
 }
 
-bool PlanKey::matches(const Model& m, const int64_t* read_off, int n_reads, int chunk_, int step_, int mode_, int halo_) const
-{
-    if (!valid || chunk != chunk_ || step != step_ || mode != mode_ || halo != halo_ || nblocks != m.nblocks || read_off[0] != 0 ||
+bool PlanKey::matches(const Model& m, const int64_t* read_off, int n_reads, int chunk_, int step_, int mode_, int halo_, int pack_) const
+{
+    if (!valid || pack != (mode_ == 0 ? pack_ : RD_PACK_NONE) || chunk != chunk_ || step != step_ || mode != mode_ || halo != halo_ || nblocks != m.nblocks || read_off[0] != 0 ||
         lens.size() != (size_t)n_reads)
         return false;
     for (int b = 0; b < m.nblocks; b++)
@@ -176,17 +219,19 @@
 }
 
 int PlanKey::rebuild(const Model& m, const int64_t* read_off, int n_reads, int chunk_, int step_, int mode_, int halo_, ReadsPlan& P, bool* streamed,
-                     size_t* n_desc)
+                     size_t* n_desc, int pack_)
 {
     invalidate();
     P = ReadsPlan();
-    int rc = mode_ == 0 ? plan_reads_chunk(m, read_off, n_reads, chunk_, step_, halo_, P) : plan_reads_global(m, read_off, n_reads, chunk_, step_, halo_, P, streamed);
+    if (mode_ != 0) pack_ = RD_PACK_NONE;
+    int rc = mode_ == 0 ? plan_reads_chunk(m, read_off, n_reads, chunk_, step_, halo_, P, pack_) : plan_reads_global(m, read_off, n_reads, chunk_, step_, halo_, P, streamed);
     if (rc) return rc;
     *n_desc = plan_pad_tiles(P);
     chunk = chunk_;
     step = step_;
     mode = mode_;
     halo = halo_;
+    pack = pack_;
     nblocks = m.nblocks;
     for (int b = 0; b < RD_MAX_BLOCKS; b++) dil[b] = b < m.nblocks ? m.dil[b] : 0;
     lens.resize(n_reads);
@@ -199,6 +244,7 @@
     size_t off = 0;
     for (int li = 0; li < RD_MAX_LAYERS; li++) {
         lists.d[li] = nullptr;
+        lists.g[li] = nullptr;
         lists.n[li] = 0;
         lists.rows[li] = 0;
     }
@@ -210,6 +256,12 @@
             lists.n[li] = (int)(v.size() / 4);
             lists.rows[li] = P.rows[li];
             off += v.size();
+            const std::vector<TileDesc>& g = P.gran[li];
+            if (!g.empty()) {
+                memcpy(h_dst + off, g.data(), g.size() * sizeof(TileDesc));
+                lists.g[li] = d_base + off;
+                off += g.size();
+            }
         } else {
             lists.d[li] = lists.d[0];
             lists.n[li] = lists.n[0];
```

Measured after the change: 27.31 million, median of 6. No clear change (+0.6%).
